# tohtsky/myFM

Hardware: AMD Instinct MI355X
Metric: Gibbs iterations/sec (rank=32) (higher is better)
Workload: dtype f64

## Files before the change

### include/myfm_hip.h

```cpp
#ifndef MYFM_HIP_H_
#define MYFM_HIP_H_

#include <stdint.h>

#ifdef __cplusplus
extern "C" {
#endif

#define MFM_OK 0
#define MFM_ERR_INVALID 1
#define MFM_ERR_RUNTIME 2
#define MFM_ERR_DEVICE 3

#define MFM_TASK_REGRESSION 0
#define MFM_TASK_CLASSIFICATION 1
#define MFM_TASK_ORDERED 2

typedef struct mfm_ctx mfm_ctx;
typedef struct mfm_design mfm_design;
typedef struct mfm_store mfm_store;

const char *mfm_version(void);
int mfm_device_count(void);
const char *mfm_global_error(void);

int mfm_create(int device, mfm_ctx **out);
void mfm_destroy(mfm_ctx *ctx);
const char *mfm_last_error(const mfm_ctx *ctx);
int mfm_get_device(const mfm_ctx *ctx);
int mfm_set_stream(mfm_ctx *ctx, void *hip_stream);
int mfm_synchronize(mfm_ctx *ctx);

int mfm_set_allreduce(mfm_ctx *ctx, int (*fn)(void *user, void *dev_buf, int64_t count), void *user);
int mfm_set_shard(mfm_ctx *ctx, int32_t rank, int32_t world);
int mfm_comm_unique_id(void *out128);
int mfm_comm_init(mfm_ctx *ctx, const void *id128, int32_t rank, int32_t world);
int mfm_comm_stats(const mfm_ctx *ctx, int64_t *calls, int64_t *doubles);
int mfm_comm_info(const mfm_ctx *ctx, int32_t *n_ranks, char *path, int64_t path_cap);
int mfm_peer_info(mfm_ctx *ctx, int32_t *pending, void **sum_buf, void **flag_buf, int64_t *sum_bytes, int64_t *flag_bytes);
int mfm_peer_set(mfm_ctx *ctx, int32_t world, int32_t rank, void *const *sum_bufs, void *const *flag_bufs);
int mfm_peer_model_info(mfm_ctx *ctx, void **w_buf, void **V_buf);
int mfm_peer_set_model(mfm_ctx *ctx, int32_t world, int32_t rank, void *const *w_bufs, void *const *V_bufs);
int mfm_peer_export(mfm_ctx *ctx, void *handles256);
int mfm_peer_import(mfm_ctx *ctx, int32_t world, int32_t rank, const void *all_handles);
int mfm_peer_drop(mfm_ctx *ctx);
int mfm_set_main_levels(mfm_ctx *ctx, const int32_t *level, int64_t D0);
int mfm_set_row_offset(mfm_ctx *ctx, int64_t first_global_row);

int mfm_set_main(mfm_ctx *ctx, int64_t N, int64_t D0, const int64_t *indptr, const int32_t *indices,
                 const double *data, const double *y);
int mfm_add_block(mfm_ctx *ctx, int64_t B, int64_t Db, const int64_t *indptr, const int32_t *indices,
                  const double *data, const int64_t *original_to_block);
int mfm_set_groups(mfm_ctx *ctx, const int32_t *group_index, int64_t D, int32_t G);
int mfm_set_residual_policy(mfm_ctx *ctx, int32_t recomputable);
int mfm_finalize(mfm_ctx *ctx, int32_t rank);

int64_t mfm_dim_all(const mfm_ctx *ctx);
int mfm_plan_info(const mfm_ctx *ctx, int64_t *n_levels_main, int64_t *n_launches_per_sweep);
int mfm_plan_flags(const mfm_ctx *ctx);
#define MFM_RES_INFO_FIELDS 16
int mfm_res_info(const mfm_ctx *ctx, int64_t *out, int n_out, char *why, int why_len);
#define MFM_CELL_INFO_FIELDS 74
int mfm_cell_info(const mfm_ctx *ctx, int64_t *out, int n_out, char *why, int why_len);
#define MFM_CHAIN_STREAM_INFO_FIELDS 30
int mfm_chain_stream_info(const mfm_ctx *ctx, int64_t *out, int max_records, int *n_records);

int mfm_set_state(mfm_ctx *ctx, double w0, const double *w, const double *V);
int mfm_get_state(mfm_ctx *ctx, double *w0, double *w, double *V);
int mfm_set_w0(mfm_ctx *ctx, double w0);
int mfm_zero_w(mfm_ctx *ctx);
int mfm_get_e(mfm_ctx *ctx, double *e);
int mfm_get_q(mfm_ctx *ctx, double *q);
int mfm_set_e(mfm_ctx *ctx, const double *e);

int mfm_reduce_e(mfm_ctx *ctx, double *sum_e, double *sum_e2);
int mfm_shift_e(mfm_ctx *ctx, double delta);
int mfm_group_stats_w(mfm_ctx *ctx, const double *mu_w, double *sum, double *ssd);
int mfm_group_stats_V(mfm_ctx *ctx, const double *mu_V, double *sum, double *ssd);
int mfm_hyper_stats(mfm_ctx *ctx, int32_t need_e, const double *mu_w, const double *mu_V, double *sum_e, double *sum_e2,
                    double *sum_w, double *ssd_w, double *sum_V, double *ssd_V);
int mfm_sweep_w(mfm_ctx *ctx, double alpha, const double *lambda_w, const double *mu_w, const double *z);
int mfm_sweep_V(mfm_ctx *ctx, int32_t f_begin, int32_t f_end, double alpha, const double *lambda_V,
                const double *mu_V, const double *z);
int mfm_sweep_wV(mfm_ctx *ctx, double alpha, double e_shift, const double *lambda_w, const double *mu_w, const double *zw,
                 int32_t f_begin, int32_t f_end, const double *lambda_V, const double *mu_V, const double *zv);

typedef struct mfm_hyper_prior {
  double alpha_0, beta_0, gamma_0, mu_0, reg_0, n_total;
  int32_t fit_w0, reserved;
} mfm_hyper_prior;
int mfm_regression_iteration_ready(mfm_ctx *ctx);
int mfm_regression_iteration(mfm_ctx *ctx, const mfm_hyper_prior *prior, const double *n_in_group, double *alpha, double *w0,
                             double *lambda_w, double *mu_w, double *lambda_V, double *mu_V);
int mfm_update_e_regression(mfm_ctx *ctx);
int mfm_update_e_classification(mfm_ctx *ctx, uint64_t seed, uint64_t draw_index);
int mfm_score_train(mfm_ctx *ctx);

int mfm_oprobit_add_group(mfm_ctx *ctx, int32_t n_class, const int64_t *rows, int64_t n_rows, int32_t *group);
int mfm_oprobit_eval(mfm_ctx *ctx, int32_t group, const double *gamma, double *ll, double *dgamma, double *H);
int mfm_oprobit_sample_z(mfm_ctx *ctx, int32_t group, const double *gamma, uint64_t seed, uint64_t draw_index);

#define MFM_RNG_NORMALS 0
#define MFM_RNG_GAMMA 1
#define MFM_RNG_LATENT 2
typedef struct mfm_rng_op {
  int32_t kind;
  int32_t dest;
  int64_t count;
  int64_t offset;
  double shape;
} mfm_rng_op;
int mfm_rng_prepare(int64_t n_features, int32_t rank, int32_t n_groups);
int mfm_rng_seed_mt19937(mfm_ctx *ctx, const uint32_t *state624, int32_t position);
int mfm_rng_set_program(mfm_ctx *ctx, const mfm_rng_op *ops, int32_t n_ops);
int mfm_rng_prefetch(mfm_ctx *ctx);
int mfm_rng_acquire(mfm_ctx *ctx, double *hyper_variates, int64_t n_hyper_variates);
int mfm_rng_get_z(mfm_ctx *ctx, double *zw, double *zv);

int mfm_update_e_classification_exact(mfm_ctx *ctx, int32_t *status);
int mfm_set_latent_order(mfm_ctx *ctx, const int64_t *rows, int64_t n);
int mfm_oprobit_sample_z_exact(mfm_ctx *ctx, int32_t group, const double *gamma, int32_t *status);
int mfm_latent_stats(mfm_ctx *ctx, int64_t *out8);
int mfm_rng_host_read(mfm_ctx *ctx, uint64_t offset, int64_t n, uint32_t *out);
int mfm_rng_host_advance(mfm_ctx *ctx, uint64_t words);

int mfm_timing_enable(mfm_ctx *ctx, int on);
int mfm_timing_select(mfm_ctx *ctx, int32_t kernel_class);
int mfm_timing_reset(mfm_ctx *ctx);
int mfm_timing_n_classes(void);
const char *mfm_timing_class_name(int cls);
int mfm_timing_get(mfm_ctx *ctx, int cls, double *ms_total, int64_t *launches, double *alg_bytes_total);

int mfm_design_create(int device, int64_t N, int64_t D0, const int64_t *indptr, const int32_t *indices,
                      const double *data, mfm_design **out);
int mfm_design_add_block(mfm_design *d, int64_t B, int64_t Db, const int64_t *indptr, const int32_t *indices,
                         const double *data, const int64_t *original_to_block);
void mfm_design_destroy(mfm_design *d);
const char *mfm_design_last_error(const mfm_design *d);
int64_t mfm_design_dim_all(const mfm_design *d);
int64_t mfm_design_n_rows(const mfm_design *d);
int mfm_design_predict(mfm_design *d, int32_t rank, int32_t n_samples, const double *w0s, const double *ws,
                       const double *Vs, int32_t mode, int32_t n_cut, const double *cutpoints, double *out);

int mfm_store_create(int device, int64_t D, int32_t rank, mfm_store **out);
void mfm_store_destroy(mfm_store *st);
const char *mfm_store_last_error(const mfm_store *st);
int32_t mfm_store_size(const mfm_store *st);
int mfm_store_reserve(mfm_store *st, int32_t n_samples);
int mfm_store_push_ctx(mfm_store *st, mfm_ctx *ctx);
int mfm_store_push_host(mfm_store *st, double w0, const double *w, const double *V);
int mfm_store_get(mfm_store *st, int32_t idx, double *w0, double *w, double *V);
int mfm_design_predict_store(mfm_design *d, mfm_store *st, int32_t first, int32_t count, int32_t mode, int32_t n_cut,
                             const double *cutpoints, double *out);

int mfm_design_summary_store(mfm_design *d, mfm_store *st, int32_t first, int32_t count, int32_t mode, int32_t n_q,
                             const double *probs, const double *precisions, const double *z, int64_t tile_rows,
                             int32_t chunk_samples, double *out_mean, double *out_std, double *out_q);
int mfm_design_summary(mfm_design *d, int32_t rank, int32_t n_samples, const double *w0s, const double *ws, const double *Vs,
                       int32_t mode, int32_t n_q, const double *probs, const double *precisions, const double *z,
                       int64_t tile_rows, int32_t chunk_samples, double *out_mean, double *out_std, double *out_q);
int mfm_design_summary_oprobit_store(mfm_design *d, mfm_store *st, int32_t first, int32_t count, int32_t expected, int32_t n_cut,
                                     const double *cutpoints, int32_t n_q, const double *probs, int64_t tile_rows,
                                     int32_t chunk_samples, double *out_mean, double *out_std, double *out_q);
int mfm_design_summary_oprobit(mfm_design *d, int32_t rank, int32_t n_samples, const double *w0s, const double *ws, const double *Vs,
                               int32_t expected, int32_t n_cut, const double *cutpoints, int32_t n_q, const double *probs,
                               int64_t tile_rows, int32_t chunk_samples, double *out_mean, double *out_std, double *out_q);

int mfm_design_logdens_store(mfm_design *d, mfm_store *st, int32_t first, int32_t count, int32_t task, const double *y,
                             const double *precisions, int32_t n_cut, const double *cutpoints, int64_t tile_rows,
                             int32_t chunk_samples, double *out_lpd, double *out_mean, double *out_var, double *out_pit,
                             double *out_ll);
int mfm_design_logdens(mfm_design *d, int32_t rank, int32_t n_samples, const double *w0s, const double *ws, const double *Vs,
                       int32_t task, const double *y, const double *precisions, int32_t n_cut, const double *cutpoints,
                       int64_t tile_rows, int32_t chunk_samples, double *out_lpd, double *out_mean, double *out_var,
                       double *out_pit, double *out_ll);
int mfm_logdens_value(int32_t task, double y, double score, double log_norm, double sqrt_alpha, int32_t n_cut,
                      const double *cutpoints_row, double *out);

int mfm_design_loo_store(mfm_design *d, mfm_store *st, int32_t first, int32_t count, int32_t task, const double *y,
                         const double *precisions, int32_t n_cut, const double *cutpoints, int64_t tile_rows,
                         int32_t chunk_samples, int32_t tail_len, double *out_elpd, double *out_k, double *out_lpd,
                         double *out_pit, double *out_lw);
int mfm_design_loo(mfm_design *d, int32_t rank, int32_t n_samples, const double *w0s, const double *ws, const double *Vs,
                   int32_t task, const double *y, const double *precisions, int32_t n_cut, const double *cutpoints,
                   int64_t tile_rows, int32_t chunk_samples, int32_t tail_len, double *out_elpd, double *out_k,
                   double *out_lpd, double *out_pit, double *out_lw);
int mfm_psis_row(int32_t S, int32_t tail_len, const double *log_lik, double *out_elpd, double *out_k, double *out_lw);

int mfm_design_ess_store(mfm_design *d, mfm_store *st, int32_t first, int32_t count, int32_t kind, int32_t mode_or_task,
                         const double *y, const double *precisions, int32_t n_cut, const double *cutpoints, int64_t tile_rows,
                         int32_t chunk_samples, double *out0, double *out1, double *out2, double *out3);
int mfm_design_ess(mfm_design *d, int32_t rank, int32_t n_samples, const double *w0s, const double *ws, const double *Vs,
                   int32_t kind, int32_t mode_or_task, const double *y, const double *precisions, int32_t n_cut,
                   const double *cutpoints, int64_t tile_rows, int32_t chunk_samples, double *out0, double *out1, double *out2,
                   double *out3);
int mfm_ess_row(int32_t S, const double *x, double *out_ess, double *out_rhat);
int mfm_design_ess_chains_store(mfm_design *d, mfm_store *st, int32_t first, int32_t count, int32_t n_chains, int32_t kind,
                                int32_t mode_or_task, const double *y, const double *precisions, int32_t n_cut,
                                const double *cutpoints, int64_t tile_rows, int32_t chunk_samples, double *out0, double *out1,
                                double *out2, double *out3);
int mfm_design_ess_chains(mfm_design *d, int32_t rank, int32_t n_samples, const double *w0s, const double *ws, const double *Vs,
                          int32_t n_chains, int32_t kind, int32_t mode_or_task, const double *y, const double *precisions,
                          int32_t n_cut, const double *cutpoints, int64_t tile_rows, int32_t chunk_samples, double *out0,
                          double *out1, double *out2, double *out3);
int mfm_ess_row_chains(int32_t S, int32_t n_chains, const double *x, double *out_ess, double *out_rhat);
int mfm_ess_check_chains(int32_t n_samples, int32_t n_chains);
int32_t mfm_ess_max_chains(void);
int mfm_rank_z_table(int32_t S, double *out);

int mfm_design_crps_store(mfm_design *d, mfm_store *st, int32_t first, int32_t count, int32_t task, const double *y,
                          const double *precisions, int32_t n_cut, const double *cutpoints, int64_t tile_rows,
                          int32_t chunk_samples, double *out_crps, double *out_accuracy, double *out_spread);
int mfm_design_crps(mfm_design *d, int32_t rank, int32_t n_samples, const double *w0s, const double *ws, const double *Vs,
                    int32_t task, const double *y, const double *precisions, int32_t n_cut, const double *cutpoints,
// ... 171 lines not shown
```

### myfm_amd/_build.py

```python
import os
import subprocess
import sys
import sysconfig

HERE = os.path.dirname(os.path.abspath(__file__))
ROOT = os.path.dirname(HERE)
CSRC = os.path.join(HERE, "csrc")
INCLUDE = os.path.join(ROOT, "include")
HIP_LIB = os.path.join(HERE, "libmyfm_hip.so")
EXT_SUFFIX = sysconfig.get_config_var("EXT_SUFFIX") or ".so"
PYMOD = os.path.join(HERE, "_myfm" + EXT_SUFFIX)

HIP_UNITS = {
    "mfm_hip.hip": ["mfm_env.hpp", "mfm_common.hpp", "mfm_wave.hpp", "mfm_policies.hpp", "mfm_kernels.hpp", "mfm_mf_kernels.hpp", "mfm_res.hpp", "mfm_res_entry.hpp", "mfm_res_plan.hpp",
                    "mfm_plan.hpp", "mfm_block_kernels.hpp", "mfm_erfcx.hpp", "mfm_tasks.hpp", "mfm_tn.hpp", "mfm_philox.hpp", "mfm_predict.hpp", "mfm_samples.hpp", "mfm_dist.hpp", "mfm_contrib.hpp", "mfm_logdens.hpp", "mfm_psis.hpp", "mfm_ess.hpp", "mfm_crps.hpp", "mfm_loo_pred.hpp", "mfm_normal_quantile.hpp", "mfm_rng.hpp", "mfm_mtjump.hpp", "mfm_cell.hpp",
                    "mfm_chain_api.hpp", "mfm_rng_state.hpp", "mfm_latent_api.hpp", "mfm_latent_host.hpp", "mfm_comm.hpp", "mfm_vbmoments.hpp", "mfm_vb_sums.hpp"],
    "mfm_latent.hip": ["mfm_env.hpp", "mfm_common.hpp", "mfm_rng_state.hpp", "mfm_latent_api.hpp"],
    "mfm_cell.hip": ["mfm_env.hpp", "mfm_common.hpp", "mfm_wave.hpp", "mfm_cell.hpp"],
    "mfm_chain.hip": ["mfm_env.hpp", "mfm_common.hpp", "mfm_wave.hpp", "mfm_policies.hpp", "mfm_chain_api.hpp", "mfm_chain_plan.hpp", "mfm_chain_stream.hpp"],
    "mfm_vb.hip": ["mfm_env.hpp", "mfm_common.hpp", "mfm_erfcx.hpp", "mfm_vb.hpp", "mfm_comm.hpp"],
    "mfm_pairs.hip": ["mfm_env.hpp", "mfm_common.hpp", "mfm_pairs.hpp", "mfm_pairs_rank.hpp", "mfm_pairs_samples.hpp", "mfm_pairs_sim.hpp", "mfm_pairs_ucb.hpp", "mfm_pairs_vb.hpp", "mfm_vb_sums.hpp", "mfm_samples.hpp"],
    "mfm_foldin.hip": ["mfm_env.hpp", "mfm_common.hpp", "mfm_foldin.hpp", "mfm_foldin_handle.hpp", "mfm_philox.hpp", "mfm_samples.hpp"],
    "mfm_foldin_gibbs.hip": ["mfm_env.hpp", "mfm_common.hpp", "mfm_foldin.hpp", "mfm_foldin_gibbs.hpp", "mfm_foldin_gibbs_plan.hpp",
                             "mfm_foldin_handle.hpp", "mfm_tn.hpp", "mfm_philox.hpp", "mfm_samples.hpp"],
}
OBJ_DIR = os.path.join(CSRC, "_obj")
PYMOD_HEADERS = ["mfm_env.hpp", "mfm_hostnormals.hpp", "mfm_mtjump.hpp", "mfm_normal_quantile.hpp"]


def _newer(target, deps):
    if not os.path.exists(target):
        return True
    t = os.path.getmtime(target)
    return any(os.path.exists(d) and os.path.getmtime(d) > t for d in deps)


def _hipcc():
    for c in ("/opt/rocm/bin/hipcc", "hipcc"):
        if os.path.exists(c) or c == "hipcc":
            return c


def build_hip(force=False, verbose=False):
    os.makedirs(OBJ_DIR, exist_ok=True)
    flags = ["--offload-arch=gfx950", "-O3", "-std=c++17", "-fPIC", "-ffp-contract=off", "-I" + INCLUDE, "-I" + CSRC] + \
        os.environ.get("MYFM_AMD_HIPCC_FLAGS", "").split()
    jobs, objs = [], []
    for src, hdrs in HIP_UNITS.items():
        obj = os.path.join(OBJ_DIR, os.path.splitext(src)[0] + ".o")
        objs.append(obj)
        deps = [os.path.join(CSRC, src)] + [os.path.join(CSRC, h) for h in hdrs] + [os.path.join(INCLUDE, "myfm_hip.h")]
        if force or _newer(obj, deps):
            cmd = [_hipcc()] + flags + ["-c", os.path.join(CSRC, src), "-o", obj]
            if verbose:
                print(" ".join(cmd))
            jobs.append((cmd, subprocess.Popen(cmd)))
    failed = [(cmd, pr.returncode) for cmd, pr in jobs if pr.wait() != 0]
    if failed:
        raise subprocess.CalledProcessError(failed[0][1], " ".join(failed[0][0]))
    if jobs or not os.path.exists(HIP_LIB) or _newer(HIP_LIB, objs):
        cmd = [_hipcc(), "--offload-arch=gfx950", "-shared", "-fPIC"] + objs + ["-o", HIP_LIB]
        if verbose:
            print(" ".join(cmd))
        subprocess.check_call(cmd)
    return HIP_LIB


def build_pymod(force=False, verbose=False):
    import pybind11

    src = os.path.join(CSRC, "_myfm.cpp")
    deps = [src, os.path.join(INCLUDE, "myfm_hip.h")] + [os.path.join(CSRC, h) for h in PYMOD_HEADERS]
    if not (force or _newer(PYMOD, deps)):
        return PYMOD
    cmd = ["g++", "-O2", "-std=c++17", "-shared", "-fPIC", "-fvisibility=hidden", "-I" + pybind11.get_include(),
           "-I" + sysconfig.get_paths()["include"], "-I" + INCLUDE, src, "-o", PYMOD, "-L" + HERE, "-lmyfm_hip",
           "-Wl,-rpath,$ORIGIN"]
    if verbose:
        print(" ".join(cmd))
    subprocess.check_call(cmd)
    return PYMOD


def build_all(force=False, verbose=False):
    build_hip(force, verbose)
    build_pymod(force, verbose)


if __name__ == "__main__":
    build_all(force="--force" in sys.argv, verbose=True)


def preload_hip_runtime():
    import ctypes
    import importlib.util

    if os.environ.get("MYFM_AMD_SYSTEM_HIP"):
        return None
    try:
        spec = importlib.util.find_spec("torch")
    except Exception:
        spec = None
    if spec is None or not spec.submodule_search_locations:
        return None
    lib = os.path.join(list(spec.submodule_search_locations)[0], "lib", "libamdhip64.so")
    if not os.path.exists(lib):
        return None
    try:
        return ctypes.CDLL(lib, mode=ctypes.RTLD_GLOBAL)
    except OSError:
        return None
```

### myfm_amd/_capi.py

```python
import ctypes as C
import os

import numpy as np
import scipy.sparse as sps

_HERE = os.path.dirname(os.path.abspath(__file__))
LIB_PATH = os.path.join(_HERE, "libmyfm_hip.so")

MFM_OK, MFM_ERR_INVALID, MFM_ERR_RUNTIME, MFM_ERR_DEVICE = 0, 1, 2, 3
TASK_REGRESSION, TASK_CLASSIFICATION, TASK_ORDERED = 0, 1, 2

SYMBOLS = [
    "mfm_version", "mfm_device_count", "mfm_global_error", "mfm_create", "mfm_destroy", "mfm_last_error",
    "mfm_set_stream", "mfm_synchronize", "mfm_set_main", "mfm_add_block", "mfm_set_groups", "mfm_finalize",
    "mfm_peer_info", "mfm_peer_set", "mfm_peer_model_info", "mfm_peer_set_model", "mfm_peer_export", "mfm_peer_import", "mfm_peer_drop", "mfm_set_residual_policy", "mfm_dim_all", "mfm_plan_info", "mfm_plan_flags", "mfm_res_info", "mfm_cell_info", "mfm_chain_stream_info", "mfm_set_state", "mfm_get_state", "mfm_set_w0", "mfm_zero_w", "mfm_get_e",
    "mfm_get_q", "mfm_set_e", "mfm_reduce_e", "mfm_shift_e", "mfm_group_stats_w", "mfm_group_stats_V",
    "mfm_sweep_w", "mfm_sweep_V", "mfm_sweep_wV", "mfm_update_e_regression", "mfm_update_e_classification", "mfm_score_train",
    "mfm_oprobit_add_group", "mfm_oprobit_eval", "mfm_oprobit_sample_z", "mfm_hyper_stats", "mfm_timing_enable", "mfm_timing_select", "mfm_timing_reset",
    "mfm_timing_n_classes", "mfm_timing_class_name", "mfm_timing_get", "mfm_design_create", "mfm_design_add_block",
    "mfm_design_destroy", "mfm_design_last_error", "mfm_design_dim_all", "mfm_design_predict",
    "mfm_host_column_levels", "mfm_rng_prepare", "mfm_rng_seed_mt19937", "mfm_rng_set_program", "mfm_rng_prefetch", "mfm_rng_acquire",
    "mfm_rng_get_z", "mfm_design_score_ctx", "mfm_design_n_rows", "mfm_set_allreduce", "mfm_set_row_offset", "mfm_set_main_levels",
    "mfm_test_erfcx", "mfm_test_truncated_normal", "mfm_get_device", "mfm_set_shard", "mfm_comm_unique_id", "mfm_comm_init",
    "mfm_comm_stats", "mfm_comm_info", "mfm_store_create", "mfm_store_destroy", "mfm_store_last_error", "mfm_store_size", "mfm_store_push_ctx",
    "mfm_store_push_host", "mfm_store_get", "mfm_design_predict_store", "mfm_store_reserve", "mfm_cs_plan_selftest", "mfm_cs_plan_probe",
    "mfm_regression_iteration_ready", "mfm_regression_iteration",
    "mfm_update_e_classification_exact", "mfm_oprobit_sample_z_exact", "mfm_latent_stats", "mfm_rng_host_read", "mfm_rng_host_advance", "mfm_set_latent_order",
    "mfm_vb_create", "mfm_vb_add_block", "mfm_vb_finalize", "mfm_vb_destroy", "mfm_vb_last_error", "mfm_vb_plan_info", "mfm_vb_set_state", "mfm_vb_get_state",
    "mfm_vb_set_w0", "mfm_vb_update_e", "mfm_vb_shift_e", "mfm_vb_get_e", "mfm_vb_get_cache", "mfm_vb_zero_w", "mfm_vb_sweep_w",
    "mfm_vb_sweep_V", "mfm_vb_group_stats", "mfm_vb_synchronize", "mfm_vb_truncated_normal",
    "mfm_vb_set_stream", "mfm_vb_set_allreduce", "mfm_vb_set_shard", "mfm_vb_comm_init", "mfm_vb_comm_stats", "mfm_vb_set_levels",
    "mfm_vb_design_levels",
    "mfm_pairs_create", "mfm_pairs_destroy", "mfm_pairs_last_error", "mfm_pairs_set_exclude", "mfm_pairs_set_scratch_bound",
    "mfm_pairs_scores_store", "mfm_pairs_topk_store", "mfm_pairs_scores", "mfm_pairs_topk", "mfm_pairs_add_block",
    "mfm_pairs_set_cutpoints", "mfm_pairs_moments_store", "mfm_pairs_moments", "mfm_pairs_topk_ucb_store", "mfm_pairs_topk_ucb",
    "mfm_pairs_set_targets", "mfm_pairs_rank_store", "mfm_pairs_rank",
    "mfm_pairs_topk_samples_store", "mfm_pairs_topk_samples", "mfm_pairs_topk_prob_store", "mfm_pairs_topk_prob",
    "mfm_pairs_create_sim", "mfm_pairs_sim_store", "mfm_pairs_sim", "mfm_pairs_topk_sim_store", "mfm_pairs_topk_sim",
    "mfm_foldin_create", "mfm_foldin_destroy", "mfm_foldin_last_error", "mfm_foldin_set_scratch_bound", "mfm_foldin_max_rank",
    "mfm_foldin_solve_store", "mfm_foldin_solve", "mfm_foldin_gibbs_solve_store", "mfm_foldin_gibbs_solve",
    "mfm_design_summary_store", "mfm_design_summary", "mfm_design_summary_oprobit_store", "mfm_design_summary_oprobit",
    "mfm_design_logdens_store", "mfm_design_logdens", "mfm_logdens_value",
    "mfm_design_loo_store", "mfm_design_loo", "mfm_psis_row",
    "mfm_design_ess_store", "mfm_design_ess", "mfm_ess_row", "mfm_rank_z_table",
    "mfm_design_ess_chains_store", "mfm_design_ess_chains", "mfm_ess_row_chains", "mfm_ess_check_chains", "mfm_ess_max_chains",
    "mfm_design_crps_store", "mfm_design_crps", "mfm_crps_row",
    "mfm_design_loo_summary_store", "mfm_design_loo_summary", "mfm_design_loo_crps_store", "mfm_design_loo_crps",
    "mfm_loo_summary_row", "mfm_loo_crps_row",
    "mfm_design_contrib_store", "mfm_design_contrib", "mfm_contrib_row",
    "mfm_design_moments_vb", "mfm_pairs_moments_vb", "mfm_pairs_topk_bound_vb",
]

SIM_METRICS = {"cosine": 0, "dot": 1}
PAIRS_VOTE_MAX = 32768

CHAIN_STREAM_INFO = ("block", "n_cols", "n_steps", "Cg", "Lw", "NB", "RD", "n_slots", "max_hot_col", "max_enter", "max_exit", "max_cold_sr",
                     "max_enter_sr", "max_exit_sr", "n_cols_no_hot")
CHAIN_STREAM_INFO_TAIL = ("lds_bytes", "n_cold", "n_hot", "launches_w", "launches_V")
CHAIN_STREAM_INFO_FIELDS = len(CHAIN_STREAM_INFO) + 10 + len(CHAIN_STREAM_INFO_TAIL)


def chain_stream_record(rec):
    n = len(CHAIN_STREAM_INFO)
    d = dict(zip(CHAIN_STREAM_INFO, (int(v) for v in rec[:n])))
    d["hot_rounds"] = [int(v) for v in rec[n:n + 10]]
    d.update(zip(CHAIN_STREAM_INFO_TAIL, (int(v) for v in rec[n + 10:])))
    return d


_lib = None


def lib():
    global _lib
    if _lib is not None:
        return _lib
    if not os.path.exists(LIB_PATH):
        raise ImportError(
            "%s is missing: build it with `python -c 'import __graft_entry__ as g; g.build()'` "
            "(hipcc --offload-arch=gfx950). There is no CPU fallback." % LIB_PATH
        )
    from ._build import preload_hip_runtime

    preload_hip_runtime()
    L = C.CDLL(LIB_PATH)
    vp, i64, i32, dbl, P = C.c_void_p, C.c_int64, C.c_int32, C.c_double, C.c_void_p
    u64 = C.c_uint64
    L.mfm_version.restype = C.c_char_p
    L.mfm_global_error.restype = C.c_char_p
    L.mfm_create.argtypes = [C.c_int, C.POINTER(vp)]
    L.mfm_destroy.argtypes = [vp]
    L.mfm_destroy.restype = None
    L.mfm_last_error.restype = C.c_char_p
    L.mfm_last_error.argtypes = [vp]
    L.mfm_set_stream.argtypes = [vp, vp]
    L.mfm_synchronize.argtypes = [vp]
    L.mfm_set_main.argtypes = [vp, i64, i64, P, P, P, P]
    L.mfm_add_block.argtypes = [vp, i64, i64, P, P, P, P]
    L.mfm_set_groups.argtypes = [vp, P, i64, i32]
    L.mfm_finalize.argtypes = [vp, i32]
    L.mfm_peer_info.argtypes = [vp, P, P, P, P, P]
    L.mfm_peer_set.argtypes = [vp, i32, i32, P, P]
    L.mfm_peer_model_info.argtypes = [vp, P, P]
    L.mfm_peer_set_model.argtypes = [vp, i32, i32, P, P]
    L.mfm_peer_export.argtypes = [vp, P]
    L.mfm_peer_import.argtypes = [vp, i32, i32, P]
    L.mfm_peer_drop.argtypes = [vp]
    L.mfm_regression_iteration_ready.argtypes = [vp]
    L.mfm_regression_iteration.argtypes = [vp, P, P, P, P, P, P, P, P]
    L.mfm_set_residual_policy.argtypes = [vp, i32]
    L.mfm_dim_all.restype = i64
    L.mfm_dim_all.argtypes = [vp]
    L.mfm_plan_info.argtypes = [vp, C.POINTER(i64), C.POINTER(i64)]
    L.mfm_plan_flags.argtypes = [vp]
    L.mfm_res_info.argtypes = [vp, P, C.c_int, C.c_char_p, C.c_int]
    L.mfm_cell_info.argtypes = [vp, P, C.c_int, C.c_char_p, C.c_int]
    L.mfm_chain_stream_info.argtypes = [vp, P, C.c_int, C.POINTER(C.c_int)]
    L.mfm_cs_plan_probe.argtypes = [i64, i32, P, P, P, i32, i32, i32, i32, P, P, C.POINTER(i32), C.POINTER(dbl)]
    L.mfm_set_state.argtypes = [vp, dbl, P, P]
    L.mfm_get_state.argtypes = [vp, C.POINTER(dbl), P, P]
    L.mfm_set_w0.argtypes = [vp, dbl]
    L.mfm_zero_w.argtypes = [vp]
    L.mfm_get_e.argtypes = [vp, P]
    L.mfm_get_q.argtypes = [vp, P]
    L.mfm_set_e.argtypes = [vp, P]
    L.mfm_reduce_e.argtypes = [vp, C.POINTER(dbl), C.POINTER(dbl)]
    L.mfm_shift_e.argtypes = [vp, dbl]
    L.mfm_group_stats_w.argtypes = [vp, P, P, P]
    L.mfm_group_stats_V.argtypes = [vp, P, P, P]
    L.mfm_hyper_stats.argtypes = [vp, C.c_int32, P, P, P, P, P, P, P, P]
    L.mfm_sweep_w.argtypes = [vp, dbl, P, P, P]
    L.mfm_sweep_V.argtypes = [vp, i32, i32, dbl, P, P, P]
    L.mfm_sweep_wV.argtypes = [vp, dbl, dbl, P, P, P, i32, i32, P, P, P]
    L.mfm_update_e_regression.argtypes = [vp]
    L.mfm_update_e_classification.argtypes = [vp, u64, u64]
    L.mfm_score_train.argtypes = [vp]
    L.mfm_oprobit_add_group.argtypes = [vp, i32, P, i64, C.POINTER(i32)]
    L.mfm_oprobit_eval.argtypes = [vp, i32, P, C.POINTER(dbl), P, P]
    L.mfm_oprobit_sample_z.argtypes = [vp, i32, P, u64, u64]
    L.mfm_timing_enable.argtypes = [vp, C.c_int]
    L.mfm_timing_select.argtypes = [vp, C.c_int32]
    L.mfm_timing_reset.argtypes = [vp]
    L.mfm_timing_class_name.restype = C.c_char_p
    L.mfm_timing_class_name.argtypes = [C.c_int]
    L.mfm_timing_get.argtypes = [vp, C.c_int, C.POINTER(dbl), C.POINTER(i64), C.POINTER(dbl)]
    L.mfm_design_create.argtypes = [C.c_int, i64, i64, P, P, P, C.POINTER(vp)]
    L.mfm_design_add_block.argtypes = [vp, i64, i64, P, P, P, P]
    L.mfm_design_destroy.argtypes = [vp]
    L.mfm_design_destroy.restype = None
    L.mfm_design_last_error.restype = C.c_char_p
    L.mfm_design_last_error.argtypes = [vp]
    L.mfm_design_dim_all.restype = i64
    L.mfm_design_dim_all.argtypes = [vp]
    L.mfm_design_predict.argtypes = [vp, i32, i32, P, P, P, i32, i32, P, P]
    L.mfm_host_column_levels.argtypes = [i64, i64, P, P, P, C.POINTER(i32)]
    L.mfm_rng_prepare.argtypes = [i64, i32, i32]
    L.mfm_rng_seed_mt19937.argtypes = [vp, P, i32]
    L.mfm_rng_set_program.argtypes = [vp, P, i32]
    L.mfm_rng_prefetch.argtypes = [vp]
    L.mfm_rng_acquire.argtypes = [vp, P, i64]
    L.mfm_rng_get_z.argtypes = [vp, P, P]
    L.mfm_update_e_classification_exact.argtypes = [vp, C.POINTER(i32)]
    L.mfm_oprobit_sample_z_exact.argtypes = [vp, i32, P, C.POINTER(i32)]
    L.mfm_latent_stats.argtypes = [vp, P]
    L.mfm_set_latent_order.argtypes = [vp, P, i64]
    L.mfm_rng_host_read.argtypes = [vp, u64, i64, P]
    L.mfm_rng_host_advance.argtypes = [vp, u64]
    L.mfm_design_score_ctx.argtypes = [vp, vp, P]
    L.mfm_design_n_rows.restype = i64
    L.mfm_design_n_rows.argtypes = [vp]
    L.mfm_set_allreduce.argtypes = [vp, vp, vp]
    L.mfm_set_row_offset.argtypes = [vp, i64]
    L.mfm_set_main_levels.argtypes = [vp, P, i64]
    L.mfm_get_device.argtypes = [vp]
    L.mfm_set_shard.argtypes = [vp, i32, i32]
    L.mfm_comm_unique_id.argtypes = [P]
    L.mfm_comm_init.argtypes = [vp, P, i32, i32]
    L.mfm_comm_stats.argtypes = [vp, C.POINTER(i64), C.POINTER(i64)]
    L.mfm_comm_info.argtypes = [vp, C.POINTER(i32), C.c_char_p, i64]
    L.mfm_store_create.argtypes = [C.c_int, i64, i32, C.POINTER(vp)]
    L.mfm_store_destroy.argtypes = [vp]
    L.mfm_store_destroy.restype = None
    L.mfm_store_last_error.restype = C.c_char_p
    L.mfm_store_last_error.argtypes = [vp]
    L.mfm_store_size.argtypes = [vp]
    L.mfm_store_reserve.argtypes = [vp, i32]
    L.mfm_store_push_ctx.argtypes = [vp, vp]
    L.mfm_store_push_host.argtypes = [vp, dbl, P, P]
    L.mfm_store_get.argtypes = [vp, i32, C.POINTER(dbl), P, P]
    L.mfm_design_predict_store.argtypes = [vp, vp, i32, i32, i32, i32, P, P]
    L.mfm_design_summary_store.argtypes = [vp, vp, i32, i32, i32, i32, P, P, P, i64, i32, P, P, P]
    L.mfm_design_summary.argtypes = [vp, i32, i32, P, P, P, i32, i32, P, P, P, i64, i32, P, P, P]
    L.mfm_design_summary_oprobit_store.argtypes = [vp, vp, i32, i32, i32, i32, P, i32, P, i64, i32, P, P, P]
    L.mfm_design_summary_oprobit.argtypes = [vp, i32, i32, P, P, P, i32, i32, P, i32, P, i64, i32, P, P, P]
    L.mfm_design_logdens_store.argtypes = [vp, vp, i32, i32, i32, P, P, i32, P, i64, i32, P, P, P, P, P]
    L.mfm_design_logdens.argtypes = [vp, i32, i32, P, P, P, i32, P, P, i32, P, i64, i32, P, P, P, P, P]
    L.mfm_logdens_value.argtypes = [i32, dbl, dbl, dbl, dbl, i32, P, P]
    L.mfm_design_loo_store.argtypes = [vp, vp, i32, i32, i32, P, P, i32, P, i64, i32, i32, P, P, P, P, P]
    L.mfm_design_loo.argtypes = [vp, i32, i32, P, P, P, i32, P, P, i32, P, i64, i32, i32, P, P, P, P, P]
    L.mfm_psis_row.argtypes = [i32, i32, P, P, P, P]
    L.mfm_design_ess_store.argtypes = [vp, vp, i32, i32, i32, i32, P, P, i32, P, i64, i32, P, P, P, P]
    L.mfm_design_ess.argtypes = [vp, i32, i32, P, P, P, i32, i32, P, P, i32, P, i64, i32, P, P, P, P]
    L.mfm_ess_row.argtypes = [i32, P, P, P]
    L.mfm_design_ess_chains_store.argtypes = [vp, vp, i32, i32, i32, i32, i32, P, P, i32, P, i64, i32, P, P, P, P]
    L.mfm_design_ess_chains.argtypes = [vp, i32, i32, P, P, P, i32, i32, i32, P, P, i32, P, i64, i32, P, P, P, P]
    L.mfm_ess_row_chains.argtypes = [i32, i32, P, P, P]
    L.mfm_ess_check_chains.argtypes = [i32, i32]
    L.mfm_ess_max_chains.argtypes = []
    L.mfm_rank_z_table.argtypes = [i32, P]
    L.mfm_design_crps_store.argtypes = [vp, vp, i32, i32, i32, P, P, i32, P, i64, i32, P, P, P]
    L.mfm_design_crps.argtypes = [vp, i32, i32, P, P, P, i32, P, P, i32, P, i64, i32, P, P, P]
    L.mfm_crps_row.argtypes = [i32, i32, dbl, P, P, i32, P, P]
    L.mfm_design_loo_summary_store.argtypes = [vp, vp, i32, i32, i32, P, P, i32, P, i64, i32, i32, i32, P, P, P, P, P, P, P]
    L.mfm_design_loo_summary.argtypes = [vp, i32, i32, P, P, P, i32, P, P, i32, P, i64, i32, i32, i32, P, P, P, P, P, P, P]
    L.mfm_design_contrib_store.argtypes = [vp, vp, i32, i32, i32, P, i64, i64, i32, P, P, P, P, P]
    L.mfm_design_contrib.argtypes = [vp, i32, i32, P, P, P, i32, P, i64, i64, i32, P, P, P, P, P]
    L.mfm_contrib_row.argtypes = [i32, P, P, i64, i32, i32, P, P, i32, P, i64, P, P]
    L.mfm_design_loo_crps_store.argtypes = [vp, vp, i32, i32, i32, P, P, i32, P, i64, i32, i32, P, P, P, P]
    L.mfm_design_loo_crps.argtypes = [vp, i32, i32, P, P, P, i32, P, P, i32, P, i64, i32, i32, P, P, P, P]
    L.mfm_loo_summary_row.argtypes = [i32, P, P, P, i32, P, P, P, P, P, P]
    L.mfm_loo_crps_row.argtypes = [i32, i32, dbl, P, P, P, i32, P, P]
    L.mfm_pairs_create.argtypes = [C.c_int, i64, i64, P, P, P, i64, P, P, P, C.POINTER(vp)]
    L.mfm_pairs_create_sim.argtypes = L.mfm_pairs_create.argtypes
    L.mfm_pairs_sim_store.argtypes = [vp, vp, i32, i32, i32, P, P]
    L.mfm_pairs_sim.argtypes = [vp, i32, i32, P, P, P, i32, P, P]
    L.mfm_pairs_topk_sim_store.argtypes = [vp, vp, i32, i32, i32, i32, C.c_double, P, P, P, P]
    L.mfm_pairs_topk_sim.argtypes = [vp, i32, i32, P, P, P, i32, i32, C.c_double, P, P, P, P]
    L.mfm_pairs_destroy.argtypes = [vp]
    L.mfm_pairs_destroy.restype = None
    L.mfm_pairs_last_error.restype = C.c_char_p
    L.mfm_pairs_last_error.argtypes = [vp]
    L.mfm_pairs_set_exclude.argtypes = [vp, P, P]
    L.mfm_pairs_set_scratch_bound.argtypes = [vp, i64]
    L.mfm_pairs_add_block.argtypes = [vp, i32, i64, i64, i64, P, P, P, P]
    L.mfm_pairs_set_cutpoints.argtypes = [vp, i32, i32, P]
    L.mfm_pairs_scores_store.argtypes = [vp, vp, i32, i32, i32, P]
    L.mfm_pairs_topk_store.argtypes = [vp, vp, i32, i32, i32, i32, P, P]
    L.mfm_pairs_scores.argtypes = [vp, i32, i32, P, P, P, i32, P]
    L.mfm_pairs_topk.argtypes = [vp, i32, i32, P, P, P, i32, i32, P, P]
    L.mfm_pairs_moments_store.argtypes = [vp, vp, i32, i32, i32, P, P]
    L.mfm_pairs_moments.argtypes = [vp, i32, i32, P, P, P, i32, P, P]
    L.mfm_pairs_topk_ucb_store.argtypes = [vp, vp, i32, i32, i32, i32, C.c_double, P, P, P, P]
    L.mfm_pairs_topk_ucb.argtypes = [vp, i32, i32, P, P, P, i32, i32, C.c_double, P, P, P, P]
    L.mfm_pairs_set_targets.argtypes = [vp, P, P]
    L.mfm_design_moments_vb.argtypes = [vp, i32, dbl, dbl, P, P, P, P, dbl, i32, i64, P, P, P]
    L.mfm_pairs_moments_vb.argtypes = [vp, i32, dbl, dbl, P, P, P, P, dbl, P, P]
    L.mfm_pairs_topk_bound_vb.argtypes = [vp, i32, dbl, dbl, P, P, P, P, dbl, i32, dbl, P, P, P, P]
    L.mfm_pairs_rank_store.argtypes = [vp, vp, i32, i32, i32, P, P]
    L.mfm_pairs_rank.argtypes = [vp, i32, i32, P, P, P, i32, P, P]
    L.mfm_pairs_topk_samples_store.argtypes = [vp, vp, i32, i32, i32, i32, P, P, P]
    L.mfm_pairs_topk_samples.argtypes = [vp, i32, i32, P, P, P, i32, i32, P, P, P]
    L.mfm_pairs_topk_prob_store.argtypes = [vp, vp, i32, i32, i32, i32, i32, P, P]
    L.mfm_pairs_topk_prob.argtypes = [vp, i32, i32, P, P, P, i32, i32, i32, P, P]
    L.mfm_foldin_create.argtypes = [C.c_int, i64, i64, P, P, P, P, i64, P, i32, C.POINTER(vp)]
    L.mfm_foldin_destroy.argtypes = [vp]
    L.mfm_foldin_destroy.restype = None
    L.mfm_foldin_last_error.restype = C.c_char_p
    L.mfm_foldin_last_error.argtypes = [vp]
    L.mfm_foldin_set_scratch_bound.argtypes = [vp, i64]
    L.mfm_foldin_max_rank.argtypes = []
    L.mfm_foldin_solve_store.argtypes = [vp, vp, i32, i32, P, P, P, i32, u64, P, P]
    L.mfm_foldin_solve.argtypes = [vp, i32, i32, P, P, P, P, P, P, i32, u64, P, P]
    L.mfm_foldin_gibbs_solve_store.argtypes = [vp, vp, i32, i32, i32, i32, P, P, P, i32, i32, i32, u64, P, P]
    L.mfm_foldin_gibbs_solve.argtypes = [vp, i32, i32, P, P, P, i32, i32, P, P, P, i32, i32, i32, u64, P, P]
    L.mfm_test_erfcx.argtypes = [C.c_int, P, i64, P]
    L.mfm_test_truncated_normal.argtypes = [C.c_int, i32, dbl, dbl, u64, u64, i64, P]
    _lib = L
    return L
# ... 124 lines not shown

    def set_e(self, e):
        e = _f64(e)
        self._ck(lib().mfm_set_e(self.h, _p(e)))

    def reduce_e(self):
        a, b = C.c_double(), C.c_double()
        self._ck(lib().mfm_reduce_e(self.h, C.byref(a), C.byref(b)))
        return a.value, b.value

    def shift_e(self, delta):
        self._ck(lib().mfm_shift_e(self.h, float(delta)))

    def group_stats_w(self, mu_w):
        mu_w = _f64(mu_w)
        s, ss = np.empty(self.G), np.empty(self.G)
        self._ck(lib().mfm_group_stats_w(self.h, _p(mu_w), _p(s), _p(ss)))
        return s, ss

    def group_stats_V(self, mu_V):
        mu = _f64(np.asarray(mu_V).T)
        s, ss = np.empty((self.K, self.G)), np.empty((self.K, self.G))
        self._ck(lib().mfm_group_stats_V(self.h, _p(mu), _p(s), _p(ss)))
        return s.T.copy(), ss.T.copy()

    def sweep_w(self, alpha, lambda_w, mu_w, z):
        lambda_w, mu_w = _f64(lambda_w), _f64(mu_w)
        if z is not None:
            z = _f64(z)
            assert z.shape[0] == self.D
        self._ck(lib().mfm_sweep_w(self.h, float(alpha), _p(lambda_w), _p(mu_w), _p(z)))

    def sweep_V(self, f_begin, f_end, alpha, lambda_V, mu_V, z):
        lam, mu = _f64(np.asarray(lambda_V).T), _f64(np.asarray(mu_V).T)
        if z is not None:
            z = _f64(z)
            assert z.size == (f_end - f_begin) * self.D
        self._ck(lib().mfm_sweep_V(self.h, f_begin, f_end, float(alpha), _p(lam), _p(mu), _p(z)))

    def sweep_wV(self, alpha, e_shift, lambda_w, mu_w, zw, f_begin, f_end, lambda_V, mu_V, zv):
        lambda_w, mu_w = _f64(lambda_w), _f64(mu_w)
        lam, mu = _f64(np.asarray(lambda_V).T), _f64(np.asarray(mu_V).T)
        if zw is not None:
            zw, zv = _f64(zw), _f64(zv)
            assert zw.shape[0] == self.D and zv.size == (f_end - f_begin) * self.D
        self._ck(lib().mfm_sweep_wV(self.h, float(alpha), float(e_shift), _p(lambda_w), _p(mu_w), _p(zw), f_begin, f_end,
                                    _p(lam), _p(mu), _p(zv)))

    def update_e_regression(self):
        self._ck(lib().mfm_update_e_regression(self.h))

    def update_e_classification(self, seed, draw_index):
        self._ck(lib().mfm_update_e_classification(self.h, seed, draw_index))

    def score_train(self):
        self._ck(lib().mfm_score_train(self.h))

    def oprobit_add_group(self, n_class, rows=None):
        g = C.c_int32()
        if rows is None:
            self._ck(lib().mfm_oprobit_add_group(self.h, n_class, None, 0, C.byref(g)))
        else:
            rows = np.ascontiguousarray(rows, dtype=np.int64)
            self._ck(lib().mfm_oprobit_add_group(self.h, n_class, _p(rows), rows.shape[0], C.byref(g)))
        return g.value

    def oprobit_eval(self, group, gamma, want_h=True):
        gamma = _f64(gamma)
        m = gamma.shape[0]
        ll = C.c_double()
        dg = np.empty(m)
        H = np.empty((m, m)) if want_h else None
        self._ck(lib().mfm_oprobit_eval(self.h, group, _p(gamma), C.byref(ll), _p(dg), _p(H)))
        return ll.value, dg, H

    def oprobit_sample_z(self, group, gamma, seed, draw_index):
        gamma = _f64(gamma)
        self._ck(lib().mfm_oprobit_sample_z(self.h, group, _p(gamma), seed, draw_index))

    def synchronize(self):
        self._ck(lib().mfm_synchronize(self.h))

    RNG_OP = np.dtype([("kind", np.int32), ("dest", np.int32), ("count", np.int64), ("offset", np.int64), ("shape", np.float64)])

    def rng_seed_mt19937(self, state624, position):
        st = np.ascontiguousarray(state624, dtype=np.uint32)
        assert st.shape[0] == 624
        self._ck(lib().mfm_rng_seed_mt19937(self.h, _p(st), int(position)))

    def rng_set_program(self, ops):
        arr = np.array([tuple(o) for o in ops], dtype=self.RNG_OP)
        self._n_hv = int(sum(o[2] for o in ops if o[1] == 0))
        self._ck(lib().mfm_rng_set_program(self.h, _p(arr), len(ops)))

    def rng_prefetch(self):
        self._ck(lib().mfm_rng_prefetch(self.h))

    def rng_acquire(self):
        hv = np.empty(max(self._n_hv, 1))
        self._ck(lib().mfm_rng_acquire(self.h, _p(hv), self._n_hv))
        return hv[: self._n_hv]

    def rng_get_z(self):
        zw, zv = np.empty(self.D), np.empty((max(self.K, 1), self.D))
        self._ck(lib().mfm_rng_get_z(self.h, _p(zw), _p(zv)))
        return zw, zv[: self.K]

    def update_e_classification_exact(self):
        st = C.c_int32()
        self._ck(lib().mfm_update_e_classification_exact(self.h, C.byref(st)))
        return st.value

    def oprobit_sample_z_exact(self, group, gamma):
        gamma = _f64(gamma)
        st = C.c_int32()
        self._ck(lib().mfm_oprobit_sample_z_exact(self.h, group, _p(gamma), C.byref(st)))
        return st.value

    def latent_stats(self):
        out = np.zeros(8, dtype=np.int64)
        self._ck(lib().mfm_latent_stats(self.h, _p(out)))
        return dict(zip(("status", "chunks", "subs", "lq", "quads", "walkers", "attempts"), (int(v) for v in out)))

    def rng_host_read(self, offset, n):
        out = np.empty(max(int(n), 1), dtype=np.uint32)
        self._ck(lib().mfm_rng_host_read(self.h, int(offset), int(n), _p(out)))
        return out[: int(n)]

    def rng_host_advance(self, words):
        self._ck(lib().mfm_rng_host_advance(self.h, int(words)))

    def set_residual_policy(self, recomputable):
        self._ck(lib().mfm_set_residual_policy(self.h, 1 if recomputable else 0))

    def plan_flags(self):
        f = lib().mfm_plan_flags(self.h)
        return {"qfree": bool(f & 1), "unit": bool(f & 2), "ell": bool(f & 4), "sharded": bool(f & 8), "soa": bool(f & 16),
                "fused_next": bool(f & 32), "sharded_fused": bool(f & 64), "mf": bool(f & 128), "resident": bool(f & 256), "cell": bool(f & 512), "streamed_chain": bool(f & 1024), "resident_overflow": bool(f & 2048)}

    RES_INFO = ("ready", "G", "RV", "RL", "RX", "umax", "n_items", "item_bits", "n_runs", "max_wg_users", "max_slice_items",
                "e_where", "n_rows", "s2_in_sweep_b", "lds_bytes", "entry_bytes")
    E_WHERE = ("rows", "slots", "slots_with_sums", "cell", "dropped")

    def res_info(self):
        out = np.zeros(len(self.RES_INFO), dtype=np.int64)
        why = C.create_string_buffer(256)
        self._ck(lib().mfm_res_info(self.h, _p(out), out.shape[0], why, len(why)))
        d = dict(zip(self.RES_INFO, (int(v) for v in out)))
        d["ready"] = bool(d["ready"])
        d["e_where"] = self.E_WHERE[d["e_where"]]
        d["why"] = why.value.decode()
        return d

    CELL_INFO = ("ready", "G", "umax", "item32", "n_streams", "n_fields", "N", "Npad", "max_steps", "chunk_max", "chunk_min",
                 "chunks_empty", "split_mask", "score_fb")
    CELL_STREAM_TYPE = ("U", "I", "C")
    CELL_MAX_STREAMS, CELL_MAX_FIELDS = 4, 16
    CELL_INFO_FIELDS = len(CELL_INFO) + 3 * CELL_MAX_STREAMS + 3 * CELL_MAX_FIELDS

    def cell_info(self):
        out = np.zeros(self.CELL_INFO_FIELDS, dtype=np.int64)
        why = C.create_string_buffer(256)
        self._ck(lib().mfm_cell_info(self.h, _p(out), out.shape[0], why, len(why)))
        n = len(self.CELL_INFO)
        nf = n + 3 * self.CELL_MAX_STREAMS
        d = dict(zip(self.CELL_INFO, (int(v) for v in out[:n])))
        d["ready"], d["item32"] = bool(d["ready"]), bool(d["item32"])
        d["streams"] = [(self.CELL_STREAM_TYPE[int(out[n + 3 * s])], int(out[n + 3 * s + 1]), int(out[n + 3 * s + 2]))
                        for s in range(d["n_streams"])]
        d["fields"] = [tuple(int(x) for x in out[nf + 3 * k:nf + 3 * k + 3]) for k in range(d["n_fields"])]
        d["why"] = why.value.decode()
        return d

    def chain_stream_info(self):
        n = C.c_int(0)
        self._ck(lib().mfm_chain_stream_info(self.h, None, 0, C.byref(n)))
        out = np.zeros((max(n.value, 1), CHAIN_STREAM_INFO_FIELDS), dtype=np.int64)
        self._ck(lib().mfm_chain_stream_info(self.h, _p(out), n.value, C.byref(n)))
        return [chain_stream_record(out[i]) for i in range(n.value)]

    def plan_info(self):
        a, b = C.c_int64(), C.c_int64()
        lib().mfm_plan_info(self.h, C.byref(a), C.byref(b))
        return a.value, b.value

    def timing_enable(self, on=True):
        self._ck(lib().mfm_timing_enable(self.h, int(on)))

    def timing_reset(self):
        self._ck(lib().mfm_timing_reset(self.h))

    def timing(self):
        L = lib()
        out = {}
        for c in range(L.mfm_timing_n_classes()):
            ms, n, by = C.c_double(), C.c_int64(), C.c_double()
            self._ck(L.mfm_timing_get(self.h, c, C.byref(ms), C.byref(n), C.byref(by)))
            if n.value:
                out[L.mfm_timing_class_name(c).decode()] = (ms.value, n.value, by.value)
        return out


class Design:

    def __init__(self, X, blocks=(), device=0):
        L = lib()
        h = C.c_void_p()
        X, ip, ix, dv = csr_parts(X)
        rc = L.mfm_design_create(device, X.shape[0], X.shape[1], _p(ip), _p(ix), _p(dv), C.byref(h))
        if rc:
            _raise(rc, L.mfm_global_error())
        self.h = h
        self.N = X.shape[0]
        for mp, B in blocks:
            B, bp, bx, bv = csr_parts(B)
            mp = np.ascontiguousarray(mp, dtype=np.int64)
            if mp.shape[0] != self.N:
                self.close()
                raise ValueError("Relation blocks have inconsistent mapper size with case_size")
            rc = L.mfm_design_add_block(h, B.shape[0], B.shape[1], _p(bp), _p(bx), _p(bv), _p(mp))
            if rc:
                msg = L.mfm_design_last_error(h)
                self.close()
                _raise(rc, msg)
        self.D = L.mfm_design_dim_all(h)

    def close(self):
        if getattr(self, "h", None):
            lib().mfm_design_destroy(self.h)
            self.h = None

    def __del__(self):
        try:
            self.close()
        except Exception:
            pass

    def score_ctx(self, ctx):
        out = np.empty(self.N)
        self._ck(lib().mfm_design_score_ctx(self.h, ctx.h, _p(out)))
        return out

    def _ck(self, rc):
        if rc:
            _raise(rc, lib().mfm_design_last_error(self.h))

    def moments_vb(self, model, extra_var=0.0, want_prob=False, tile_rows=0):
        K, head, keep = _pack_vb_model(model)
        mean, std, prob = np.empty(self.N), np.empty(self.N), np.empty(self.N if want_prob else 0)
        self._ck(lib().mfm_design_moments_vb(self.h, K, *head, float(extra_var), int(bool(want_prob)), int(tile_rows), _p(mean), _p(std),
                                             _p(prob) if want_prob else None))
        return (mean, std, prob) if want_prob else (mean, std)

    def _predict(self, src, mode, cutpoints):
        n_cut, cp = 0, None
        if mode == 2:
            cp = _f64(np.stack([np.asarray(c, dtype=np.float64) for c in cutpoints]))
            n_cut = cp.shape[1]
        out = np.empty((self.N, n_cut + 1) if mode == 2 else self.N)
        self._ck(src.call("mfm_design_predict", self.h, mode, n_cut, _p(cp), _p(out)))
        return out

    def _summary(self, src, mode, quantiles, precisions, tile_rows, chunk_samples):
        probs, prec, z, mean, std, q = _summary_args(self.N, quantiles, precisions)
        self._ck(src.call("mfm_design_summary", self.h, mode, len(probs), _p(probs), _p(prec), _p(z), int(tile_rows),
                          int(chunk_samples), _p(mean), _p(std), _p(q)))
        return mean, std, q

    def _summary_oprobit(self, src, cutpoints, expected, quantiles, tile_rows, chunk_samples):
        cp, n_cut, probs, mean, std, q = _summary_oprobit_args(self.N, cutpoints, expected, quantiles)
        self._ck(src.call("mfm_design_summary_oprobit", self.h, int(bool(expected)), n_cut, _p(cp), len(probs), _p(probs),
                          int(tile_rows), int(chunk_samples), _p(mean), _p(std), _p(q)))
        return mean, std, q

    def _log_density_args(self, y, precisions, cutpoints):
        y = _f64(y).reshape(-1)
        if y.shape[0] != self.N:
            raise ValueError("y must hold one value per design row")
        prec = None if precisions is None else _f64(precisions).reshape(-1)
        cp, n_cut = None, 0
        if cutpoints is not None:
            cp = _f64(cutpoints)
            if cp.ndim != 2:
                raise ValueError("cutpoints must be a 2-D array, one row of n_cut cutpoints per sample")
            n_cut = cp.shape[1]
        return y, prec, n_cut, cp

    def _log_density(self, src, task, y, precisions, cutpoints, pointwise, tile_rows, chunk_samples):
        y, prec, n_cut, cp = self._log_density_args(y, precisions, cutpoints)
        lpd, mean, var = np.empty(self.N), np.empty(self.N), np.empty(self.N)
        pit = np.empty(self.N) if task == TASK_REGRESSION else None
        ll = np.empty((src.S, self.N)) if pointwise else None
        self._ck(src.call("mfm_design_logdens", self.h, int(task), _p(y), _p(prec), n_cut, _p(cp), int(tile_rows), int(chunk_samples),
                          _p(lpd), _p(mean), _p(var), _p(pit), _p(ll)))
        return lpd, mean, var, pit, ll

    def log_density(self, samples, task, y, precisions=None, cutpoints=None, pointwise=False, tile_rows=0, chunk_samples=0):
        return self._log_density(_host(samples), task, y, precisions, cutpoints, pointwise, tile_rows, chunk_samples)

    def _loo(self, src, task, y, precisions, cutpoints, log_weights, r_eff, tile_rows, chunk_samples):
        y, prec, n_cut, cp = self._log_density_args(y, precisions, cutpoints)
        elpd, k, lpd = np.empty(self.N), np.empty(self.N), np.empty(self.N)
        pit = np.empty(self.N) if task == TASK_REGRESSION else None
        lw = np.empty((src.S, self.N)) if log_weights else None
        self._ck(src.call("mfm_design_loo", self.h, int(task), _p(y), _p(prec), n_cut, _p(cp), int(tile_rows), int(chunk_samples),
                          psis_tail_len(src.S, r_eff), _p(elpd), _p(k), _p(lpd), _p(pit), _p(lw)))
# ... 544 lines not shown
```

### myfm_amd/csrc/mfm_hip.hip

```cpp
#include <algorithm>
#include <cerrno>
#include <chrono>
#include <cmath>
#include <cstdio>
#include <cstring>
#include <map>
#include <memory>
#include <mutex>
#include <string>
#include <thread>
#include <type_traits>
#include <vector>

#include <fcntl.h>
#include <sys/file.h>
#include <sys/stat.h>
#include <unistd.h>

#include <hipcub/hipcub.hpp>

#include "mfm_common.hpp"
#include "mfm_kernels.hpp"
#include "mfm_plan.hpp"
#include "mfm_res_plan.hpp"
// ... 1410 lines not shown
  MFM_HIP_CHECK(hipStreamSynchronize(c->stream));
  c->res.peers_set = true;
  c->res_state = ResState::Live;
  MFM_CATCH(ctx)
}

int mfm_peer_set_model(mfm_ctx *ctx, int32_t world, int32_t rank, void *const *w_bufs, void *const *V_bufs) {
  MFM_TRY(ctx)
  ctx->need_final();
  mfm_ctx *c = ctx;
  if (!c->resident_V() || !c->res.peers_set) throw Error(MFM_ERR_RUNTIME, "mfm_peer_set_model: mfm_peer_set comes first");
  if (world != c->res.xworld || rank != c->res.xrank) throw Error(MFM_ERR_INVALID, "mfm_peer_set_model: world / rank differ from the communicator's");
  for (int r = 0; r < world; r++) {
    if (!w_bufs[r] || (c->K > 0 && !V_bufs[r])) throw Error(MFM_ERR_INVALID, "mfm_peer_set_model: null buffer");
    c->res.peer_w[r] = (double *)w_bufs[r];
    c->res.peer_V[r] = (double *)V_bufs[r];
  }
  if (c->res.peer_w[rank] != c->w.p || c->res.peer_V[rank] != c->V.p)
    throw Error(MFM_ERR_INVALID, "mfm_peer_set_model: this rank's own entry must be its own w / V (mfm_peer_model_info)");
  MFM_HIP_CHECK(hipStreamSynchronize(c->stream));
  c->res.peers_model = true;
  MFM_CATCH(ctx)
}

int mfm_peer_model_info(mfm_ctx *ctx, void **w_buf, void **V_buf) {
  MFM_TRY(ctx)
  ctx->need_final();
  if (w_buf) *w_buf = ctx->w.p;
  if (V_buf) *V_buf = ctx->V.p;
  MFM_CATCH(ctx)
}

int mfm_peer_export(mfm_ctx *ctx, void *handles256) {
  MFM_TRY(ctx)
  ctx->need_final();
  if (ctx->res_state != ResState::AwaitingPeers) throw Error(MFM_ERR_RUNTIME, "mfm_peer_export: no row-sharded persistent sweep waiting for its peers");
  static_assert(sizeof(hipIpcMemHandle_t) == 64, "IPC handle size");
  hipIpcMemHandle_t h[4];
  std::memset(h, 0, sizeof h);
  MFM_HIP_CHECK(hipIpcGetMemHandle(&h[0], ctx->res.xsum.p));
  MFM_HIP_CHECK(hipIpcGetMemHandle(&h[1], ctx->res.xflag.p));
  MFM_HIP_CHECK(hipIpcGetMemHandle(&h[2], ctx->w.p));
  if (ctx->K > 0) MFM_HIP_CHECK(hipIpcGetMemHandle(&h[3], ctx->V.p));
  std::memcpy(handles256, h, sizeof h);
  MFM_CATCH(ctx)
}

int mfm_peer_import(mfm_ctx *ctx, int32_t world, int32_t rank, const void *all_handles) {
  MFM_TRY(ctx)
  ctx->need_final();
  mfm_ctx *c = ctx;
  if (c->res_state != ResState::AwaitingPeers) throw Error(MFM_ERR_RUNTIME, "mfm_peer_import: no row-sharded persistent sweep waiting for its peers");
  if (world != c->res.xworld || rank != c->res.xrank) throw Error(MFM_ERR_INVALID, "mfm_peer_import: world / rank differ from the communicator's");
  void *sums[RES_MAX_PEERS], *flags[RES_MAX_PEERS], *ws[RES_MAX_PEERS], *Vs[RES_MAX_PEERS];
  for (int r = 0; r < world; r++) {
    if (r == rank) {
      sums[r] = c->res.xsum.p;
      flags[r] = c->res.xflag.p;
      ws[r] = c->w.p;
      Vs[r] = c->V.p;
      continue;
    }
    hipIpcMemHandle_t h[4];
    std::memcpy(h, (const char *)all_handles + (size_t)r * 256, sizeof h);
    MFM_HIP_CHECK(hipIpcOpenMemHandle(&sums[r], h[0], hipIpcMemLazyEnablePeerAccess));
    c->res.peer_mapped.push_back(sums[r]);
    MFM_HIP_CHECK(hipIpcOpenMemHandle(&flags[r], h[1], hipIpcMemLazyEnablePeerAccess));
    c->res.peer_mapped.push_back(flags[r]);
    MFM_HIP_CHECK(hipIpcOpenMemHandle(&ws[r], h[2], hipIpcMemLazyEnablePeerAccess));
    c->res.peer_mapped.push_back(ws[r]);
    Vs[r] = nullptr;
    if (c->K > 0) {
      MFM_HIP_CHECK(hipIpcOpenMemHandle(&Vs[r], h[3], hipIpcMemLazyEnablePeerAccess));
      c->res.peer_mapped.push_back(Vs[r]);
    }
  }
  int rc = mfm_peer_set(ctx, world, rank, sums, flags);
  if (rc != MFM_OK) return rc;
  if (env_int("MYFM_PEER_MODEL", 0) != 0) {
    rc = mfm_peer_set_model(ctx, world, rank, ws, Vs);
    if (rc != MFM_OK) return rc;
  }
  MFM_CATCH(ctx)
}

int mfm_peer_drop(mfm_ctx *ctx) {
  MFM_TRY(ctx)
  ctx->need_final();
  MFM_HIP_CHECK(hipStreamSynchronize(ctx->stream));
  materialize_e(ctx);
  ctx->drop_resident();
  MFM_CATCH(ctx)
}

int mfm_set_residual_policy(mfm_ctx *ctx, int32_t recomputable) {
  if (!ctx) return MFM_ERR_INVALID;
  ctx->e_recomputable = recomputable != 0;
  return MFM_OK;
}

int64_t mfm_dim_all(const mfm_ctx *ctx) { return ctx->D; }

int mfm_plan_info(const mfm_ctx *ctx, int64_t *n_levels_main, int64_t *n_launches_per_sweep) {
  if (ctx->v_path == VPath::Deferred) {
    if (n_levels_main) *n_levels_main = 2;
    if (n_launches_per_sweep) *n_launches_per_sweep = 1;
    return MFM_OK;
  }
  if (n_levels_main) *n_levels_main = (int64_t)ctx->plan_V.n_levels;
  if (n_launches_per_sweep) {
    int64_t n = ctx->plan_V.launches;
    for (auto &B : ctx->blocks) n += B->plan_V.launches + 3;
    *n_launches_per_sweep = n;
  }
  return MFM_OK;
}

int mfm_plan_flags(const mfm_ctx *ctx) {
  bool streamed = false;
  for (auto &B : ctx->blocks)
    for (const Step &st : B->plan_V.steps) streamed = streamed || (st.is_chain && st.chain.form == ChainForm::Stream);
  int form = 0;
  switch (ctx->v_path) {
    case VPath::QFree: form = 1; break;
    case VPath::Split: form = 16; break;
    case VPath::SplitFused: form = 16 | 32; break;
    case VPath::TwoField: form = 16 | 32 | 128; break;
    case VPath::ShardedSplit: form = 64; break;
    case VPath::ShardedTwoField: form = 64 | 128; break;
    case VPath::Deferred:
    case VPath::Generic:
    case VPath::Cell:
      break;
  }
  return (streamed ? 1024 : 0) | (ctx->resident_V() && ctx->res.RX > 0 ? 2048 : 0) | form | (ctx->X.unit ? 2 : 0) | (ctx->X.ell_width >= 0 ? 4 : 0) |
         (ctx->comm.active() ? 8 : 0) | (ctx->resident_V() ? 256 : 0) | (ctx->cell.ready ? 512 : 0);
}

int mfm_res_info(const mfm_ctx *ctx, int64_t *out, int n_out, char *why, int why_len) {
  if (!ctx || n_out < 0 || (n_out > 0 && !out) || why_len < 0 || (why_len > 0 && !why)) return MFM_ERR_INVALID;
  const ResPlan &rp = ctx->res;
  const int64_t v[MFM_RES_INFO_FIELDS] = {ctx->resident_V() ? 1 : 0, rp.G,       rp.RV,     rp.RL,           rp.RX,
                                          rp.umax,          rp.n_items, rp.item_bits, rp.n_runs,    rp.max_wg_users,
                                          rp.max_slice_items, (int64_t)ctx->e_where, rp.n_rows, rp.s2b, (int64_t)rp.lds_bytes,
                                          rp.ent_bytes};
  for (int i = 0; i < n_out; i++) out[i] = i < MFM_RES_INFO_FIELDS ? v[i] : 0;
  if (why_len > 0) {
    std::strncpy(why, ctx->resident_V() ? "" : rp.why.c_str(), (size_t)why_len - 1);
    why[why_len - 1] = 0;
  }
  return MFM_OK;
}

int mfm_cell_info(const mfm_ctx *ctx, int64_t *out, int n_out, char *why, int why_len) {
  if (!ctx || n_out < 0 || (n_out > 0 && !out) || why_len < 0 || (why_len > 0 && !why)) return MFM_ERR_INVALID;
  const CellPlan &cp = ctx->cell;
  int64_t v[MFM_CELL_INFO_FIELDS] = {0};
  const int m = (int)cp.fields.size(), ns = (int)cp.streams.size();
  int64_t split = 0;
  const bool typed = ns > 0 && cp.sU == 0;
  for (int k = 0; k < m && typed; k++)
    if (cp.split_pass(k == 0 ? m - 1 : k - 1, k, k == 0)) split |= (int64_t)1 << k;
  const int64_t head[14] = {cp.ready ? 1 : 0, cp.G,         cp.umax,      cp.item32 ? 1 : 0, ns,    m, cp.N, cp.Npad, cp.max_steps,
                            cp.chunk_max,     cp.chunk_min, cp.chunks_empty, split,          cp.ready ? cp.score_fb() : 0};
  for (int i = 0; i < 14; i++) v[i] = head[i];
  for (int i = 0; i < ns && i < CELL_MAX_STREAMS; i++) {
    v[14 + 3 * i] = cp.streams[i].type;
    v[15 + 3 * i] = cp.streams[i].slot;
    v[16 + 3 * i] = cp.streams[i].card;
  }
  for (int k = 0; k < m && k < CELL_MAX_FIELDS; k++) {
    v[14 + 3 * CELL_MAX_STREAMS + 3 * k] = cp.fields[k].stream;
    v[15 + 3 * CELL_MAX_STREAMS + 3 * k] = cp.fields[k].kind;
    v[16 + 3 * CELL_MAX_STREAMS + 3 * k] = cp.fields[k].n;
  }
  for (int i = 0; i < n_out; i++) out[i] = i < MFM_CELL_INFO_FIELDS ? v[i] : 0;
  if (why_len > 0) {
    std::strncpy(why, cp.ready ? "" : cp.why.c_str(), (size_t)why_len - 1);
    why[why_len - 1] = 0;
  }
  return MFM_OK;
}

int mfm_chain_stream_info(const mfm_ctx *ctx, int64_t *out, int max_records, int *n_records) {
  static_assert(MFM_CHAIN_STREAM_INFO_FIELDS == CS_INFO_FIELDS, "include/myfm_hip.h documents cs_info_record's fields");
  if (!ctx || max_records < 0 || (max_records > 0 && !out)) return MFM_ERR_INVALID;
  int n = 0;
  for (size_t b = 0; b < ctx->blocks.size(); b++) {
    std::vector<const CsStream *> of_w;
    for (const Step &st : ctx->blocks[b]->plan_W.steps)
      if (st.is_chain && st.chain.form == ChainForm::Stream) of_w.push_back(st.chain.stream.get());
    size_t k = 0;
    for (const Step &st : ctx->blocks[b]->plan_V.steps) {
      if (!st.is_chain || st.chain.form != ChainForm::Stream) continue;
      if (n < max_records) {
        int64_t *rec = out + (size_t)n * MFM_CHAIN_STREAM_INFO_FIELDS;
        cs_info_record(cs_stream_info(*st.chain.stream), rec);
        rec[0] = (int64_t)b;
        rec[28] = k < of_w.size() ? cs_stream_launches(*of_w[k], false) : 0;
        rec[29] = cs_stream_launches(*st.chain.stream, true);
      }
      n++;
      k++;
    }
  }
  if (n_records) *n_records = n;
  return MFM_OK;
}

int mfm_set_state(mfm_ctx *ctx, double w0, const double *w, const double *V) {
  MFM_TRY(ctx)
  ctx->need_final();
  ctx->w0 = w0;
  ctx->ring.upload(ctx->w.p, w, (size_t)ctx->D * sizeof(double), ctx->stream);
  if (ctx->K) ctx->ring.upload(ctx->V.p, V, (size_t)ctx->D * ctx->K * sizeof(double), ctx->stream);
  MFM_CATCH(ctx)
}

int mfm_get_state(mfm_ctx *ctx, double *w0, double *w, double *V) {
  MFM_TRY(ctx)
  ctx->need_final();
  *w0 = ctx->w0;
  if (ctx->D)
    MFM_HIP_CHECK(hipMemcpyAsync(w, ctx->w.p, (size_t)ctx->D * sizeof(double), hipMemcpyDeviceToHost, ctx->stream));
  if (ctx->K && ctx->D)
    MFM_HIP_CHECK(
        hipMemcpyAsync(V, ctx->V.p, (size_t)ctx->D * ctx->K * sizeof(double), hipMemcpyDeviceToHost, ctx->stream));
  ctx->sync_and_check();
  MFM_CATCH(ctx)
}

int mfm_set_w0(mfm_ctx *ctx, double w0) {
  MFM_TRY(ctx)
  if (w0 != ctx->w0) ensure_e(ctx);
  ctx->w0 = w0;
  MFM_CATCH(ctx)
}

int mfm_zero_w(mfm_ctx *ctx) {
  MFM_TRY(ctx)
  ctx->need_final();
  if (ctx->D) MFM_HIP_CHECK(hipMemsetAsync(ctx->w.p, 0, (size_t)ctx->D * sizeof(double), ctx->stream));
  MFM_CATCH(ctx)
}

static int get_eq(mfm_ctx *ctx, double *dst, int which) {
  MFM_TRY(ctx)
  ctx->need_final();
  materialize_e(ctx);
  if (ctx->N) {
    hipLaunchKernelGGL(k_get_eq, dim3(cdiv(ctx->N, WG)), dim3(WG), 0, ctx->stream, ctx->eq_rows(), ctx->scratch_n.p, ctx->N,
                       which);
    MFM_HIP_CHECK(
        hipMemcpyAsync(dst, ctx->scratch_n.p, (size_t)ctx->N * sizeof(double), hipMemcpyDeviceToHost, ctx->stream));
    MFM_HIP_CHECK(hipStreamSynchronize(ctx->stream));
  }
  MFM_CATCH(ctx)
}
int mfm_get_e(mfm_ctx *ctx, double *e) { return get_eq(ctx, e, 0); }
int mfm_get_q(mfm_ctx *ctx, double *q) {
  if (ctx->finalized && ctx->q_stale_factor >= 0) {
    try {
      ctx->use_device();
      for (auto &B : ctx->blocks)
        if (ctx->cell.ready) block_rowcache(ctx->stream, ctx->timing, *B, ctx->V.p + (size_t)ctx->q_stale_factor * ctx->D + B->col_off, true);
      launch_qbuild(ctx, ctx->V.p + (size_t)ctx->q_stale_factor * ctx->D);
      ctx->q_stale_factor = -1;
    } catch (const std::exception &ex) {
      ctx->err = ex.what();
      return MFM_ERR_RUNTIME;
    }
  }
  return get_eq(ctx, q, 1);
}
int mfm_set_e(mfm_ctx *ctx, const double *e) {
  MFM_TRY(ctx)
  ctx->need_final();
  if (ctx->e_where == EWhere::Dropped) ctx->e_where = EWhere::Rows;
  ctx->e_is_residual = false;
  materialize_e(ctx);
  if (ctx->N) {
    MFM_HIP_CHECK(hipStreamSynchronize(ctx->stream));
    MFM_HIP_CHECK(hipMemcpy(ctx->scratch_n.p, e, (size_t)ctx->N * sizeof(double), hipMemcpyHostToDevice));
    hipLaunchKernelGGL(k_set_eq, dim3(cdiv(ctx->N, WG)), dim3(WG), 0, ctx->stream, ctx->eq_rows(), ctx->scratch_n.p, ctx->N, 0);
    MFM_HIP_CHECK(hipStreamSynchronize(ctx->stream));
  }
  MFM_CATCH(ctx)
}

int mfm_reduce_e(mfm_ctx *ctx, double *sum_e, double *sum_e2) {
  MFM_TRY(ctx)
  ctx->need_final();
  materialize_e(ctx);
  hipStream_t s = ctx->stream;
  {
    TimedLaunch t(ctx->timing, s, KC_REDUCE_E, 8.0 * ctx->N);
    hipLaunchKernelGGL(k_reduce_e_partial, dim3(REDUCE_BLOCKS), dim3(WG), 0, s, ctx->eq_rows(), ctx->N, ctx->red_partial.p);
    hipLaunchKernelGGL(k_reduce_final, dim3(1), dim3(WG), 0, s, ctx->red_partial.p, REDUCE_BLOCKS, ctx->red_out.p);
  }
  ctx->comm.allreduce(ctx->red_out.p, 2);
  double2 *h = ctx->readback(2);
  MFM_HIP_CHECK(hipMemcpyAsync(h, ctx->red_out.p, sizeof(double2), hipMemcpyDeviceToHost, s));
  MFM_HIP_CHECK(hipMemcpyAsync(h + 1, ctx->ls.error.p, sizeof(int), hipMemcpyDeviceToHost, s));
  MFM_HIP_CHECK(hipStreamSynchronize(s));
  ctx->check_coresident(*(const int *)(h + 1));
  *sum_e = h[0].x;
// ... 802 lines not shown
```

### myfm_amd/csrc/mfm_res.hpp

```cpp
#pragma once
#include <algorithm>
#include <cstdlib>
#include <cstring>
#include <atomic>
#include <string>
#include <thread>
#include <type_traits>
#include <vector>

#include "mfm_common.hpp"
#include "mfm_mf_kernels.hpp"
#include "mfm_res_entry.hpp"

namespace mfm {

#ifndef MFM_RES_CH
#define MFM_RES_CH 4
#endif
constexpr int RES_MAX_PEERS = 8;

struct ResArgs {
  double2 *eq;
  const double *e_in;
  double *e_slots;
  const int32_t *perm;
  const uint32_t *uidw;
  const uint32_t *headw;
  const int32_t *run_item;
  const int32_t *first_run;
  const int32_t *wg_run_ptr;
  const int32_t *wg_nruns;
  const int32_t *wg_user_ptr;
  const int2 *user_desc;
  const int32_t *wg_item_ptr;
  const int32_t *ent_ptr;
  const uint32_t *entries;
  const int32_t *scols;
  const int2 *item_desc;
  double *partials;
  double *dv;
  double *V;
  int64_t D;
  int f_begin, f_end;
  int linear;
  int n_sw;
  double *w;
  const double *zw;
  const double *lam_w, *mu_w;
  double e_shift;
  const double *z;
  const double *lam, *mu;
  const int32_t *group;
  int n_groups;
  double alpha;
  const double *scal;
  int n_items, umax;
  unsigned long long *bar;
  int n_wg;
  int *error;
  unsigned long long *prof;
  int xworld, xrank;
  unsigned long long xepoch0;
  double *xsum[RES_MAX_PEERS];
  unsigned long long *xflag[RES_MAX_PEERS];
  unsigned long long *xarrive;
  int xmodel;
  double *xw[RES_MAX_PEERS], *xV[RES_MAX_PEERS];
  int ngx;
  int no_store;
  int xch_break;
  int ent4;
  const double *s2_lin;
};

__device__ __forceinline__ void res_store2(double *p, double a, double b) {
  __hip_atomic_store(p, a, __ATOMIC_RELAXED, __HIP_MEMORY_SCOPE_AGENT);
  __hip_atomic_store(p + 1, b, __ATOMIC_RELAXED, __HIP_MEMORY_SCOPE_AGENT);
}

enum { RES_BAR_START = 0, RES_BAR_TOP = 16, RES_BAR_XCNT = 32, RES_BAR_GEN = 160, RES_BAR_CENSUS = 288, RES_BAR_WORDS = 416 };
struct ResBar {
  int xcc;
  unsigned long long n_x, nx;
};

__device__ __forceinline__ bool res_spin(const ResArgs &a, const unsigned long long *w, unsigned long long target, bool &dead) {
  unsigned spins = 0;
  while (__hip_atomic_load(w, __ATOMIC_RELAXED, __HIP_MEMORY_SCOPE_AGENT) < target) {
#ifndef MFM_RES_NO_SLEEP
    __builtin_amdgcn_s_sleep(1);
#endif
    if ((++spins & 1023u) == 0u) {
      if (spins > (1u << 22) || __hip_atomic_load(a.error, __ATOMIC_RELAXED, __HIP_MEMORY_SCOPE_AGENT) != 0) {
        __hip_atomic_store(a.error, 1, __ATOMIC_RELAXED, __HIP_MEMORY_SCOPE_AGENT);
        dead = true;
        return false;
      }
    }
  }
  return true;
}

__device__ __forceinline__ bool res_spin_sys(const ResArgs &a, const unsigned long long *w, unsigned long long target, bool &dead) {
  unsigned spins = 0;
  while (__hip_atomic_load(w, __ATOMIC_RELAXED, __HIP_MEMORY_SCOPE_SYSTEM) < target) {
    __builtin_amdgcn_s_sleep(2);
    if ((++spins & 1023u) == 0u) {
      const int seen = __hip_atomic_load(a.error, __ATOMIC_RELAXED, __HIP_MEMORY_SCOPE_AGENT);
      if (spins > (1u << 23) || seen != 0) {
        if (seen == 0) __hip_atomic_store(a.error, 2, __ATOMIC_RELAXED, __HIP_MEMORY_SCOPE_AGENT);
        dead = true;
        return false;
      }
    }
  }
  return true;
}

__device__ __forceinline__ void res_bar_init(const ResArgs &a, ResBar &rb, bool &dead) {
  unsigned x;
  asm volatile("s_getreg_b32 %0, hwreg(HW_REG_XCC_ID, 0, 4)" : "=s"(x));
  rb.xcc = (int)(x & 7u);
  __hip_atomic_fetch_add(a.bar + RES_BAR_CENSUS + 16 * rb.xcc, 1ull, __ATOMIC_RELAXED, __HIP_MEMORY_SCOPE_AGENT);
  asm volatile("s_waitcnt vmcnt(0)" ::: "memory");
  __hip_atomic_fetch_add(a.bar + RES_BAR_START, 1ull, __ATOMIC_RELAXED, __HIP_MEMORY_SCOPE_AGENT);
  rb.n_x = 1;
  rb.nx = 1;
  if (!res_spin(a, a.bar + RES_BAR_START, (unsigned long long)a.n_wg, dead)) return;
  rb.nx = 0;
  for (int i = 0; i < 8; i++) {
    const unsigned long long c = __hip_atomic_load(a.bar + RES_BAR_CENSUS + 16 * i, __ATOMIC_RELAXED, __HIP_MEMORY_SCOPE_AGENT);
    rb.nx += c > 0 ? 1 : 0;
    if (i == rb.xcc) rb.n_x = c;
  }
}

__device__ __forceinline__ void res_grid_barrier(const ResArgs &a, const ResBar &rb, unsigned long long k, int tid, bool &dead) {
  asm volatile("s_waitcnt vmcnt(0)" ::: "memory");
  __syncthreads();
  if (tid == 0 && !dead) {
    const unsigned long long old =
        __hip_atomic_fetch_add(a.bar + RES_BAR_XCNT + 16 * rb.xcc, 1ull, __ATOMIC_RELAXED, __HIP_MEMORY_SCOPE_AGENT);
    if (old + 1 == k * rb.n_x) {
      __builtin_amdgcn_fence(__ATOMIC_RELEASE, "agent");
      asm volatile("s_waitcnt vmcnt(0)" ::: "memory");
      __hip_atomic_fetch_add(a.bar + RES_BAR_TOP, 1ull, __ATOMIC_RELAXED, __HIP_MEMORY_SCOPE_AGENT);
      if (res_spin(a, a.bar + RES_BAR_TOP, k * rb.nx, dead))
        __hip_atomic_store(a.bar + RES_BAR_GEN + 16 * rb.xcc, k, __ATOMIC_RELAXED, __HIP_MEMORY_SCOPE_AGENT);
    } else {
      res_spin(a, a.bar + RES_BAR_GEN + 16 * rb.xcc, k, dead);
    }
    __builtin_amdgcn_fence(__ATOMIC_ACQUIRE, "agent");
  }
  __syncthreads();
}

constexpr int res_dv_shift(bool s2b) { return s2b ? 5 : 4; }
typedef double res_d16_t __attribute__((ext_vector_type(16)));
typedef unsigned res_u4_t __attribute__((ext_vector_type(4)));
typedef double res_d2u_t __attribute__((ext_vector_type(2), aligned(8)));
__device__ __forceinline__ double res_cc0(double x) { return x; }
__device__ __forceinline__ double res_cc1(double) { return 0.0; }
__device__ __forceinline__ double res_cc0(res_d2u_t x) { return x[0]; }
__device__ __forceinline__ double res_cc1(res_d2u_t x) { return x[1]; }

#define RES_UID(lo, hi, bb, k) \
  ((k) < 3 ? (int)(((lo) >> (10 * (k))) & 0x3ffu) : (int)(((lo) >> 30) | ((((hi) >> (8 * (bb))) & 0xffu) << 2)))
#define RES_UIDS(lo, hi, bb, uid)        \
  {                                      \
    const unsigned lo_ = lo;             \
    uid[0] = RES_UID(lo_, hi, bb, 0);    \
    uid[1] = RES_UID(lo_, hi, bb, 1);    \
    uid[2] = RES_UID(lo_, hi, bb, 2);    \
    uid[3] = RES_UID(lo_, hi, bb, 3);    \
  }
#define RES_USER_WORDS(p_, row_, off_, uw_, ux_)                                                      \
  _Pragma("unroll") for (int w_ = 0; w_ < 4; w_++) uw_[w_] = (p_)[((row_) + w_) * NT + (off_)];       \
  ux_ = (p_)[((row_) + 4) * NT + (off_)]
#define RES_GROUP_WORDS(a_, ngt_, j_, uw_, ux_, hb_)                                           \
  RES_USER_WORDS((a_).uidw, (int64_t)g * (5 * (ngt_)) + 5 * (j_), tid, uw_, ux_);              \
  hb_ = (a_).headw[((int64_t)g * (ngt_) + (j_)) * NT + tid]

template <int NT, int NGV, int NGL, bool XCH = false, bool OVF = false, bool S2B = false>
__global__ __launch_bounds__(NT) void k_mf_resident(ResArgs a) {
  extern __shared__ __attribute__((aligned(16))) char res_smem[];
  constexpr int NW = NT / WAVE, NG = NGV + NGL, R = 16 * NG, RL = 16 * NGL;
  constexpr int B = 4;
  const int g = (int)blockIdx.x, tid = threadIdx.x, lane = tid & 63;
  const int wv = __builtin_amdgcn_readfirstlane(tid >> 6);
  const int U = a.umax;
  const double alpha_k = a.scal ? a.scal[0] : a.alpha, e_shift_k = a.scal ? a.scal[2] : a.e_shift;
  const int ngx = OVF ? a.ngx : 0, NGt = NG + ngx, Rt = 16 * NGt;
  d2_t *utab = (d2_t *)res_smem;
  double *elds = (double *)(utab + U);
  double *acc1 = elds + (size_t)RL * NT;
  double *acc2 = acc1 + NW * U;
  double *acc3 = acc2 + NW * U;
  d2_t *wcarry = (d2_t *)(acc2 + (S2B ? 2 : 1) * NW * U);
  int *wflag = (int *)(wcarry + NW);
  const int32_t *perm_g = a.perm + (int64_t)g * Rt * NT;
  const int u0 = a.wg_user_ptr[g], nu = a.wg_user_ptr[g + 1] - u0;
  const int rb0 = a.wg_run_ptr[g];
  const int pad_item = a.n_items;
  constexpr int DSH = res_dv_shift(S2B);
  const unsigned rb0b = 4u * (unsigned)rb0, padb = (unsigned)pad_item << DSH;
  const char *run_item_b = (const char *)a.run_item, *dv_b = (const char *)a.dv;
  double *acc1w = acc1 + wv * U, *acc2w = acc2 + wv * U, *acc3w = acc3 + wv * U;
  bool dead = false;
  unsigned long long nbar = 0;
  ResBar rbar;
  rbar.xcc = 0;
  rbar.n_x = rbar.nx = 1;
#define RES_STAMP0(k) \
  if (a.prof && tid == 0) a.prof[(int64_t)g * a.n_sw * 64 + 56 + (k)] = __builtin_amdgcn_s_memrealtime()
  RES_STAMP0(0);
  if (tid == 0) res_bar_init(a, rbar, dead);
  RES_STAMP0(1);
  const int wv_hi = wv >> 2;
#define RES_PRIO(j)                  \
  if ((((j) & 1) ^ wv_hi) != 0)      \
    __builtin_amdgcn_s_setprio(1);   \
  else                               \
    __builtin_amdgcn_s_setprio(0)
  const int trash_run = a.wg_run_ptr[g] + a.wg_nruns[g];
#define RES_STAMP(k)                                                                                      \
  if (a.prof && tid == 0) a.prof[((int64_t)g * a.n_sw + (f - f_first)) * 64 + (k)] = __builtin_amdgcn_s_memrealtime()

  const bool s2_tab = S2B && a.s2_lin != nullptr;
  for (int i = tid; i < (S2B && !s2_tab ? 3 : 2) * NW * U; i += NT) acc1[i] = 0.0;
  if (s2_tab)
    for (int i = tid; i < NW * U; i += NT) acc3[i] = a.s2_lin[(int64_t)g * (NW * U) + i];
  for (int i = tid; i < U; i += NT) utab[i] = d2_t{0.0, 0.0};

  res_u4_t uw[NG];
  unsigned ux[NG];
  unsigned hbv[NG], nbv[NG];
#pragma unroll
  for (int j = 0; j < NG; j++) {
    RES_GROUP_WORDS(a, NGt, j, uw[j], ux[j], hbv[j]);
    nbv[j] = hbv[j] | (j == 0 ? 1u : 0u);
  }
  const unsigned nbx0 = OVF && ngx > 0 ? a.headw[((int64_t)g * NGt + NG) * NT + tid] : 0u;
  double *eog = OVF ? a.e_slots + ((int64_t)g * Rt + 16 * NG) * NT + tid : nullptr;
  const uint32_t *uidw_x = a.uidw + ((int64_t)g * (5 * NGt) + 5 * NG) * NT + tid;
  const uint32_t *headw_x = a.headw + ((int64_t)g * NGt + NG) * NT + tid;
  const int run0 = a.first_run[g * NT + tid];
  const bool head0 = (hbv[0] & 1u) != 0u;
#define RES_NIB(j, q) ((((nbv[j]) | ((j) + 1 < NG ? nbv[(j) + 1 < NG ? (j) + 1 : (j)] << 16 : nbx0 << 16)) >> (4 * (q))) & 15u)
#define RES_ON_NIB(q) RES_NIB(j, q)
#define RES_ON_HEADS hbv[j]
#define RES_ON_UIDS(bb, uid) RES_UIDS(uw[j][bb], ux[j], bb, uid)
#define RES_ON_LD(bb, k) (j < NGV ? ev[j < NGV ? j : 0][4 * (bb) + k] : elds[(16 * (j - NGV) + 4 * (bb) + k) * NT + tid])
#define RES_ON_ST(bb, k, x)                \
  if (j < NGV)                             \
    ev[j < NGV ? j : 0][4 * (bb) + k] = x; \
  else                                     \
    elds[(16 * (j - NGV) + 4 * (bb) + k) * NT + tid] = x
#define RES_OV_NIB(q) ((nbw >> (4 * (q))) & 15u)
#define RES_OV_HEADS hb_c
#define RES_OV_UIDS(bb, uid) RES_UIDS(uwx[bb], uxx, bb, uid)
#define RES_OV_LD(bb, k) eo[4 * (bb) + k]
#define RES_OV_ST(bb, k, x) eo[4 * (bb) + k] = x
#define RES_OVERFLOW_GROUPS(STEP, gA, gB)                                                   \
  if (OVF) {                                                                                \
    unsigned hb_c = nbx0;                                                                   \
    for (int jx = 0; jx < ngx; jx++) {                                                      \
      res_u4_t uwx;                                                                         \
      unsigned uxx;                                                                         \
      RES_USER_WORDS(uidw_x, 5 * jx, 0, uwx, uxx);                                          \
      const unsigned hb_n = jx + 1 < ngx ? headw_x[(jx + 1) * NT] : 0u;                     \
      const unsigned nbw = hb_c | (hb_n << 16);                                             \
      res_d16_t eo;                                                                         \
      _Pragma("unroll") for (int i = 0; i < 16; i++) eo[i] = eog[(16 * jx + i) * NT];       \
      _Pragma("unroll 1") for (int bp = 0; bp < 2; bp++) {                                  \
        STEP(RES_OV, 2 * bp, itA, itB, gA, gB);                                             \
        STEP(RES_OV, 2 * bp + 1, itB, itA, gB, gA);                                         \
      }                                                                                     \
      _Pragma("unroll") for (int i = 0; i < 16; i++) eog[(16 * jx + i) * NT] = eo[i];       \
      hb_c = hb_n;                                                                          \
    }                                                                                       \
  }
#define RES_PRIME(T, OFF, gA)                                                                                         \
  {                                                                                                                   \
    int it0[B];                                                                                                       \
    const unsigned n0 = RES_NIB(0, 0), n1 = RES_NIB(0, 1);                                                            \
    _Pragma("unroll") for (int k = 0; k < B; k++) {                                                                   \
      rcb += ((n0 >> k) & 1u) << 2;                                                                                   \
      it0[k] = *(const int *)(run_item_b + ((n0 >> k) & 1u ? rcb : rb0b));                                            \
    }                                                                                                                 \
    _Pragma("unroll") for (int k = 0; k < B; k++) {                                                                   \
      rcb += ((n1 >> k) & 1u) << 2;                                                                                   \
      itA[k] = *(const int *)(run_item_b + ((n1 >> k) & 1u ? rcb : rb0b));                                            \
    }                                                                                                                 \
    _Pragma("unroll") for (int k = 0; k < B; k++)                                                                     \
      gA[k] = *(const T *)(dv_b + (OFF) + ((n0 >> k) & 1u ? (unsigned)it0[k] << DSH : padb));                         \
  }

#define RES_OPAQUE()                                                                            \
  _Pragma("unroll") for (int j_ = 0; j_ < NG; j_++) {                                           \
    asm volatile("" : "+v"(uw[j_]), "+v"(ux[j_]), "+v"(hbv[j_]), "+v"(nbv[j_]));                \
  }
  res_d16_t ev[NGV > 0 ? NGV : 1];
#pragma unroll
  for (int j = 0; j < NG; j++) {
#pragma unroll 1
    for (int bb = 0; bb < 4; bb++) {
      int row[B];
#pragma unroll
      for (int k = 0; k < B; k++) row[k] = a.e_in ? 0 : perm_g[(16 * j + 4 * bb + k) * NT + tid];
#pragma unroll
      for (int k = 0; k < B; k++) {
        const double x = (a.e_in ? a.e_in[((int64_t)g * Rt + 16 * j + 4 * bb + k) * NT + tid] : a.eq[row[k] < 0 ? 0 : row[k]].x) + e_shift_k;
        RES_ON_ST(bb, k, x);
      }
    }
  }
  if (OVF) {
    for (int jx = 0; jx < ngx; jx++) {
#pragma unroll 4
      for (int i = 0; i < 16; i++) {
        const int64_t sl = 16 * (NG + jx) + i;
        const int row = a.e_in ? 0 : perm_g[sl * NT + tid];
        const double x = (a.e_in ? a.e_in[((int64_t)g * Rt + sl) * NT + tid] : a.eq[row < 0 ? 0 : row].x) + e_shift_k;
        eog[(16 * jx + i) * NT] = x;
      }
    }
  }
  __syncthreads();
  if (S2B && !s2_tab) {
    const uint32_t *uidw_p = a.uidw + (int64_t)g * (5 * NGt) * NT + tid;
    const uint32_t *headw_p = a.headw + (int64_t)g * NGt * NT + tid;
    int run = run0 - 1;
    double c = 0.0;
#pragma unroll 1
    for (int jp = 0; jp < NGt; jp++) {
      const unsigned nb = headw_p[jp * NT] | (jp == 0 ? 1u : 0u);
      const unsigned uxp = uidw_p[(5 * jp + 4) * NT];
#pragma unroll 1
      for (int bb = 0; bb < 4; bb++) {
        const unsigned lo_ = uidw_p[(5 * jp + bb) * NT];
#pragma unroll 1
        for (int k = 0; k < B; k++) {
          if ((nb >> (4 * bb + k)) & 1u) {
            run++;
            c = a.dv[((int64_t)a.run_item[run] << (DSH - 3)) + 1];
          }
          const int uid = RES_UID(lo_, uxp, bb, k);
          __hip_atomic_fetch_add(&acc3w[uid], c * c, __ATOMIC_RELAXED, __HIP_MEMORY_SCOPE_WORKGROUP);
        }
      }
    }
    __syncthreads();
  }

  RES_STAMP0(2);
  const int f_first = a.f_begin - a.linear;
  for (int f = f_first; f < a.f_end; f++) {
    const bool lin = f < a.f_begin;
    double *Vf = lin ? a.w : a.V + (int64_t)f * a.D;
    const double *zf = lin ? a.zw : a.z + (int64_t)(f - a.f_begin) * a.D;
    const double *lamf = lin ? a.lam_w : a.lam + (int64_t)f * a.n_groups;
    const double *muf = lin ? a.mu_w : a.mu + (int64_t)f * a.n_groups;
    int uj = 0;
    double uold = 0.0, uz = 0.0, ulam = 0.0, umu = 0.0;
    if (tid < nu) {
      const int2 d = a.user_desc[u0 + tid];
      uj = d.x;
      uold = Vf[uj];
      uz = zf[uj];
      ulam = lamf[d.y];
      umu = muf[d.y];
    }
    RES_STAMP(0);
    {
      RES_OPAQUE();
      asm volatile(";; res sweep A");
      unsigned rcb = 4u * (unsigned)(run0 - 1);
      int itA[B];
      d2_t ddA[B];
      RES_PRIME(d2_t, 0, ddA);
      d2_t ddc = d2_t{0.0, 0.0};
      int itB[B];
      d2_t ddB[B];
#define RES_STEP_A(F, bb, iti, ito, ddi, ddo)                                                                              \
  {                                                                                                                        \
    const unsigned n4 = F##_NIB(bb), n4a = F##_NIB((bb) + 1), n4b = F##_NIB((bb) + 2);                                     \
    _Pragma("unroll") for (int k = 0; k < B; k++) {                                                                        \
      rcb += ((n4b >> k) & 1u) << 2;                                                                                       \
      ito[k] = *(const int *)(run_item_b + ((n4b >> k) & 1u ? rcb : rb0b));                                                \
    }                                                                                                                      \
    _Pragma("unroll") for (int k = 0; k < B; k++)                                                                          \
      ddo[k] = *(const d2_t *)(dv_b + ((n4a >> k) & 1u ? (unsigned)iti[k] << DSH : padb));                                 \
    int uid[B];                                                                                                            \
    F##_UIDS(bb, uid);                                                                                                     \
    double up[B], ex[B];                                                                                                   \
    _Pragma("unroll") for (int k = 0; k < B; k++) {                                                                        \
      up[k] = utab[uid[k]][0];                                                                                             \
      ex[k] = F##_LD(bb, k);                                                                                               \
    }                                                                                                                      \
    _Pragma("unroll") for (int k = 0; k < B; k++) {                                                                        \
      const bool need = ((n4 >> k) & 1u) != 0u;                                                                            \
      ddc[0] = need ? ddi[k][0] : ddc[0];                                                                                  \
      ddc[1] = need ? ddi[k][1] : ddc[1];                                                                                  \
      const double er = ex[k] + up[k] * ddc[0];                                                                            \
      F##_ST(bb, k, er);                                                                                                   \
      const double c = ddc[1];                                                                                             \
      __hip_atomic_fetch_add(&acc1w[uid[k]], (-er) * c, __ATOMIC_RELAXED, __HIP_MEMORY_SCOPE_WORKGROUP);                   \
      if (!S2B) __hip_atomic_fetch_add(&acc2w[uid[k]], c * c, __ATOMIC_RELAXED, __HIP_MEMORY_SCOPE_WORKGROUP);             \
    }                                                                                                                      \
  }
#pragma unroll
      for (int j = 0; j < NG; j++) {
        RES_PRIO(j);
#pragma unroll
        for (int bp = 0; bp < 2; bp++) {
          RES_STEP_A(RES_ON, 2 * bp, itA, itB, ddA, ddB);
          RES_STEP_A(RES_ON, 2 * bp + 1, itB, itA, ddB, ddA);
        }
      }
      asm volatile(";; res sweep end");
      RES_OVERFLOW_GROUPS(RES_STEP_A, ddA, ddB);
#undef RES_STEP_A
    }
    __syncthreads();
    RES_STAMP(1);
    if (tid < nu) {
      double S1 = 0.0, S2 = 0.0;
#pragma unroll
      for (int w = 0; w < NW; w++) {
        double *accS = S2B ? acc3 : acc2;
        S1 += acc1[w * U + tid];
        S2 += accS[w * U + tid];
        acc1[w * U + tid] = 0.0;
        accS[w * U + tid] = 0.0;
      }
      const double fresh = PMainV::draw(S1, S2, uold, alpha_k, ulam, umu, uz);
      Vf[uj] = fresh;
      if (XCH && a.xmodel) {
        for (int r = 0; r < a.xworld; r++)
          if (r != a.xrank)
            __hip_atomic_store((lin ? a.xw[r] : a.xV[r] + (int64_t)f * a.D) + uj, fresh, __ATOMIC_RELAXED, __HIP_MEMORY_SCOPE_SYSTEM);
      }
      utab[tid] = d2_t{lin ? 1.0 : fresh, fresh - uold};
    }
    __syncthreads();
    RES_STAMP(2);
    {
      typedef typename std::conditional<S2B, res_d2u_t, double>::type cc_t;
#define RES_CC0(x) res_cc0(x)
#define RES_CC1(x) res_cc1(x)
      bool have_head = false;
      double f1 = 0.0, f2 = 0.0, s1 = 0.0, s2 = 0.0;
      d2_t *part2 = (d2_t *)a.partials;
      char *part_b = (char *)a.partials - 16;
      const unsigned trashb = 16u * (unsigned)(trash_run + 1);
      {
        RES_OPAQUE();
        asm volatile(";; res sweep B");
        unsigned rcb = 4u * (unsigned)(run0 - 1);
        unsigned rcCb = 16u * (unsigned)(run0 - 1);
        int itA[B];
        cc_t ccA[B];
        RES_PRIME(cc_t, 8, ccA);
        double ccc = 0.0, cqc = 0.0;
        int itB[B];
        cc_t ccB[B];
#define RES_PARTIAL_STORE() *(d2_t *)(part_b + (head && have_head ? rcCb : trashb)) = d2_t{s1, s2}
#define RES_STEP_B(F, bb, iti, ito, cci, cco)                                                                              \
  {                                                                                                                        \
    const unsigned n4 = F##_NIB(bb), n4a = F##_NIB((bb) + 1), n4b = F##_NIB((bb) + 2);                                     \
    const unsigned h4 = (F##_HEADS >> (4 * (bb))) & 15u;                                                                   \
    _Pragma("unroll") for (int k = 0; k < B; k++) {                                                                        \
      rcb += ((n4b >> k) & 1u) << 2;                                                                                       \
      ito[k] = *(const int *)(run_item_b + ((n4b >> k) & 1u ? rcb : rb0b));                                                \
    }                                                                                                                      \
    _Pragma("unroll") for (int k = 0; k < B; k++)                                                                          \
      cco[k] = *(const cc_t *)(dv_b + 8 + ((n4a >> k) & 1u ? (unsigned)iti[k] << DSH : padb));                             \
    int uid[B];                                                                                                            \
    F##_UIDS(bb, uid);                                                                                                     \
    d2_t ut[B];                                                                                                            \
    double ex[B];                                                                                                          \
    _Pragma("unroll") for (int k = 0; k < B; k++) {                                                                        \
      ut[k] = utab[uid[k]];                                                                                                \
      ex[k] = F##_LD(bb, k);                                                                                               \
    }                                                                                                                      \
    _Pragma("unroll") for (int k = 0; k < B; k++) {                                                                        \
      const bool need = ((n4 >> k) & 1u) != 0u;                                                                            \
      const bool head = ((h4 >> k) & 1u) != 0u;                                                                            \
      ccc = need ? RES_CC0(cci[k]) : ccc;                                                                                  \
      if (S2B) {                                                                                                           \
        cqc = need ? RES_CC1(cci[k]) : cqc;                                                                                \
        __hip_atomic_fetch_add(&acc3w[uid[k]], cqc, __ATOMIC_RELAXED, __HIP_MEMORY_SCOPE_WORKGROUP);                       \
      }                                                                                                                    \
      rcCb += need ? 16u : 0u;                                                         \
                        \
      RES_PARTIAL_STORE();                                                                                                 \
      f1 = head && !have_head ? s1 : f1;                                                                                   \
      f2 = head && !have_head ? s2 : f2;                                                                                   \
      have_head = have_head || head;                                                                                       \
      const double er = ex[k] + ccc * ut[k][1];                                                                            \
      F##_ST(bb, k, er);                                                                                                   \
      s1 = (head ? 0.0 : s1) + (-er) * ut[k][0];                                                                           \
      s2 = (head ? 0.0 : s2) + ut[k][0] * ut[k][0];                                                                        \
    }                                                                                                                      \
  }
#pragma unroll
        for (int j = 0; j < NG; j++) {
          RES_PRIO(j);
#pragma unroll 1
          for (int bp = 0; bp < 2; bp++) {
            RES_STEP_B(RES_ON, 2 * bp, itA, itB, ccA, ccB);
            RES_STEP_B(RES_ON, 2 * bp + 1, itB, itA, ccB, ccA);
          }
          if (a.prof && lane == 0 && (wv == 4 || wv == 7))
            a.prof[((int64_t)g * a.n_sw + (f - f_first)) * 64 + 16 + (wv == 4 ? 0 : 20) + j] = __builtin_amdgcn_s_memrealtime();
        }
        asm volatile(";; res sweep end");
        RES_OVERFLOW_GROUPS(RES_STEP_B, ccA, ccB);
#undef RES_STEP_B
#undef RES_CC0
#undef RES_CC1
#undef RES_PARTIAL_STORE
      }
      if (a.prof && lane == 0)
        a.prof[((int64_t)g * a.n_sw + (f - f_first)) * 64 + 8 + wv] = __builtin_amdgcn_s_memrealtime();
      double v1 = s1, v2 = s2;
      int fl = have_head ? 1 : 0;
      wave_segscan2(v1, v2, fl);
      if (lane == 63) {
        wcarry[wv] = d2_t{v1, v2};
        wflag[wv] = fl;
      }
      double x1 = dpp_f64<0x138, 0xf>(v1), x2 = dpp_f64<0x138, 0xf>(v2);
      int xf = dpp_i32<0x138, 0xf>(fl, 0);
      if (lane == 0) {
        x1 = 0.0;
        x2 = 0.0;
        xf = 0;
      }
      lds_barrier();
      if (have_head && tid > 0) {
        if (!xf) {
          double c1 = 0.0, c2 = 0.0;
          for (int w = 0; w < wv; w++) {
            const d2_t cw = wcarry[w];
            const bool fw = wflag[w] != 0;
            c1 = (fw ? 0.0 : c1) + cw[0];
            c2 = (fw ? 0.0 : c2) + cw[1];
          }
          x1 = c1 + x1;
          x2 = c2 + x2;
        }
        const int closing = head0 ? run0 - 1 : run0;
        part2[closing] = d2_t{x1 + f1, x2 + f2};
      }
    }
    RES_STAMP(3);
    constexpr int CH = MFM_RES_CH;
    const int c0 = a.ent_ptr[g] >> 6, c1 = a.ent_ptr[g + 1] >> 6;
    const int per = (c1 - c0 + NW - 1) / NW;
    const int wb = c0 + wv * per, we = wb + per < c1 ? wb + per : c1;
    const int i0 = a.wg_item_ptr[g], ni = a.wg_item_ptr[g + 1] - i0;
    const bool more = f + 1 < a.f_end;
    int ij = 0;
    double iold = 0.0, iz = 0.0, ivn = 0.0, ivq = 0.0, ilam = 0.0, imu = 0.0;
    if (tid < ni) {
      const int2 d = a.item_desc[i0 + tid];
      ij = d.x;
      iold = Vf[ij];
      iz = zf[ij];
      ivn = more ? a.V[(int64_t)(f + 1) * a.D + ij] : 0.0;
      if (S2B) ivq = f + 2 < a.f_end ? a.V[(int64_t)(f + 2) * a.D + ij] : 0.0;
      ilam = lamf[d.y];
      imu = muf[d.y];
    }
    const bool ent4 = a.ent4 != 0;
#define RES_ENTRIES(c_)                                                                                                    \
  if (ent4) {                                                                                                              \
    _Pragma("unroll") for (int k = 0; k < CH; k++)                                                                         \
      en[k] = make_int2((int)a.entries[(int64_t)((c_) + k < we ? (c_) + k : (c_)) * WAVE + lane], 0);                      \
  } else {                                                                                                                 \
    _Pragma("unroll") for (int k = 0; k < CH; k++)                                                                         \
      en[k] = ((const int2 *)a.entries)[(int64_t)((c_) + k < we ? (c_) + k : (c_)) * WAVE + lane];                         \
  }
#define RES_ENT_RUN(e_) (ent4 ? res_entry_run((uint32_t)(e_).x) : (e_).x)
#define RES_ENT_ITEM(e_) (ent4 ? res_entry_item((uint32_t)(e_).x) : (e_).y)
    int2 en[CH];
#pragma unroll
    for (int k = 0; k < CH; k++) en[k] = make_int2(0, 0);
    if (wb < we) {
      RES_ENTRIES(wb);
    }
    res_grid_barrier(a, rbar, ++nbar, tid, dead);
    RES_STAMP(4);
    {
      const d2_t *part2 = (const d2_t *)a.partials;
      for (int cb = wb; cb < we; cb += CH) {
        d2_t sv[CH];
#pragma unroll
        for (int k = 0; k < CH; k++) sv[k] = part2[RES_ENT_RUN(en[k])];
        int il[CH];
#pragma unroll
        for (int k = 0; k < CH; k++) il[k] = RES_ENT_ITEM(en[k]);
        if (cb + CH < we) {
          RES_ENTRIES(cb + CH);
        }
#pragma unroll
        for (int k = 0; k < CH; k++) {
          if (cb + k >= we) break;
          __hip_atomic_fetch_add(&acc1[wv * U + il[k]], sv[k][0], __ATOMIC_RELAXED, __HIP_MEMORY_SCOPE_WORKGROUP);
          __hip_atomic_fetch_add(&acc2[wv * U + il[k]], sv[k][1], __ATOMIC_RELAXED, __HIP_MEMORY_SCOPE_WORKGROUP);
        }
      }
      __syncthreads();
      double S1 = 0.0, S2 = 0.0;
      if (tid < ni) {
#pragma unroll
        for (int w = 0; w < NW; w++) {
          S1 += acc1[w * U + tid];
          S2 += acc2[w * U + tid];
          acc1[w * U + tid] = 0.0;
          acc2[w * U + tid] = 0.0;
        }
      }
      if (XCH) {
        const unsigned long long E = a.xepoch0 + (unsigned long long)(f - f_first) + 1ull;
        const int64_t stride = 2 * ((int64_t)a.n_items + 1), par = (int64_t)(E & 1ull);
        if (tid < ni) {
          const int64_t off = ((int64_t)a.xrank * 2 + par) * stride + 2 * (int64_t)(i0 + tid);
          for (int r = 0; r < a.xworld; r++) {
            __hip_atomic_store(a.xsum[r] + off, S1, __ATOMIC_RELAXED, __HIP_MEMORY_SCOPE_SYSTEM);
            __hip_atomic_store(a.xsum[r] + off + 1, S2, __ATOMIC_RELAXED, __HIP_MEMORY_SCOPE_SYSTEM);
          }
        }
        asm volatile("s_waitcnt vmcnt(0)" ::: "memory");
        __syncthreads();
        if (tid == 0 && !dead) {
          const unsigned long long old = __hip_atomic_fetch_add(a.xarrive, 1ull, __ATOMIC_RELAXED, __HIP_MEMORY_SCOPE_AGENT);
          if (old + 1 == (unsigned long long)a.n_wg * E) {
            for (int r = 0; r < a.xworld && !a.xch_break; r++)
              __hip_atomic_store(a.xflag[r] + 16 * a.xrank, E, __ATOMIC_RELEASE, __HIP_MEMORY_SCOPE_SYSTEM);
          }
          for (int r = 0; r < a.xworld && !dead; r++) res_spin_sys(a, a.xflag[a.xrank] + 16 * r, E, dead);
        }
        __syncthreads();
        if (tid < ni) {
          S1 = S2 = 0.0;
          for (int r = 0; r < a.xworld; r++) {
            const int64_t off = ((int64_t)r * 2 + par) * stride + 2 * (int64_t)(i0 + tid);
            S1 += __hip_atomic_load(a.xsum[a.xrank] + off, __ATOMIC_RELAXED, __HIP_MEMORY_SCOPE_SYSTEM);
            S2 += __hip_atomic_load(a.xsum[a.xrank] + off + 1, __ATOMIC_RELAXED, __HIP_MEMORY_SCOPE_SYSTEM);
          }
        }
      }
      if (tid < ni) {
        const double fresh = PMainV::draw(S1, S2, iold, alpha_k, ilam, imu, iz);
        Vf[ij] = fresh;
        res_store2(a.dv + ((int64_t)(i0 + tid) << (DSH - 3)), fresh - iold, ivn);
        if (S2B) __hip_atomic_store(a.dv + 4 * (int64_t)(i0 + tid) + 2, ivq * ivq, __ATOMIC_RELAXED, __HIP_MEMORY_SCOPE_AGENT);
      }
    }
    RES_STAMP(5);
    res_grid_barrier(a, rbar, ++nbar, tid, dead);
    RES_STAMP(6);
  }
#undef RES_STAMP
#undef RES_ENTRIES
#undef RES_ENT_RUN
#undef RES_ENT_ITEM
  RES_STAMP0(3);
  if (!a.no_store) {
    int run_last = run0;
#pragma unroll
    for (int j = 0; j < NG; j++) {
#pragma unroll 1
      for (int bb = 0; bb < 4; bb++) {
        const unsigned h4 = (hbv[j] >> (4 * bb)) & 15u;
        int row[B], it[B];
#pragma unroll
        for (int k = 0; k < B; k++) {
          if (16 * j + 4 * bb + k > 0) run_last += (int)((h4 >> k) & 1u);
          it[k] = a.run_item[run_last];
          row[k] = perm_g[(16 * j + 4 * bb + k) * NT + tid];
        }
        int uid[B];
        RES_ON_UIDS(bb, uid);
#pragma unroll
        for (int k = 0; k < B; k++) {
          const double dl = a.dv[(int64_t)it[k] << (DSH - 3)];
          const double ex = RES_ON_LD(bb, k);
          const double ef = ex + utab[uid[k]][0] * dl;
          if (a.e_slots)
            a.e_slots[((int64_t)g * Rt + 16 * j + 4 * bb + k) * NT + tid] = ef;
          else if (row[k] >= 0)
            a.eq[row[k]].x = ef;
        }
      }
    }
    if (OVF) {
      for (int jx = 0; jx < ngx; jx++) {
        res_u4_t uwx;
        unsigned uxx;
        RES_USER_WORDS(uidw_x, 5 * jx, 0, uwx, uxx);
        const unsigned hbx = headw_x[jx * NT];
#pragma unroll 1
        for (int bb = 0; bb < 4; bb++) {
          const unsigned h4 = (hbx >> (4 * bb)) & 15u;
          int it[B], uid[B];
#pragma unroll
          for (int k = 0; k < B; k++) {
            run_last += (int)((h4 >> k) & 1u);
            it[k] = a.run_item[run_last];
          }
          RES_OV_UIDS(bb, uid);
#pragma unroll
          for (int k = 0; k < B; k++) {
            const double dl = a.dv[(int64_t)it[k] << (DSH - 3)];
            double *ep = eog + (16 * jx + 4 * bb + k) * NT;
            *ep = *ep + utab[uid[k]][0] * dl;
          }
        }
      }
    }
  }
#undef RES_PRIO
#undef RES_NIB
#undef RES_ON_NIB
#undef RES_ON_HEADS
#undef RES_ON_UIDS
#undef RES_ON_LD
#undef RES_ON_ST
#undef RES_OV_NIB
#undef RES_OV_HEADS
#undef RES_OV_UIDS
#undef RES_OV_LD
#undef RES_OV_ST
#undef RES_OVERFLOW_GROUPS
#undef RES_PRIME
#undef RES_OPAQUE
  asm volatile("s_waitcnt vmcnt(0)" ::: "memory");
  RES_STAMP0(4);
#undef RES_STAMP0
}

__global__ void k_res_init_dv(const double *__restrict__ theta, const int32_t *__restrict__ scols, int n_items,
                              double *__restrict__ dv, unsigned long long *__restrict__ bar, int wd,
                              const double *__restrict__ theta2) {
  const int i = blockIdx.x * blockDim.x + threadIdx.x;
  if (blockIdx.x == 0)
    for (int k = threadIdx.x; k < RES_BAR_WORDS; k += blockDim.x) bar[k] = 0ull;
  if (i > n_items) return;
  const bool pad = i == n_items;
  dv[wd * i] = 0.0;
  dv[wd * i + 1] = pad ? 0.0 : theta ? theta[scols[i]] : 1.0;
  if (wd == 4) {
    const double c2 = !pad && theta2 ? theta2[scols[i]] : 0.0;
    dv[wd * i + 2] = c2 * c2;
    dv[wd * i + 3] = 0.0;
  }
}

__global__ __launch_bounds__(512) void k_res_s2_lin(const uint32_t *__restrict__ uidw, const uint32_t *__restrict__ headw,
                                                    const int32_t *__restrict__ run_item, const int32_t *__restrict__ first_run,
                                                    int NGt, int umax, int n_items, double *__restrict__ s2_lin) {
  extern __shared__ unsigned res_s2_cnt[];
  constexpr int NT = 512, NW = NT / WAVE;
  const int g = (int)blockIdx.x, tid = threadIdx.x, wv = tid >> 6;
  for (int i = tid; i < NW * umax; i += NT) res_s2_cnt[i] = 0u;
  __syncthreads();
  const uint32_t *uidw_p = uidw + (int64_t)g * (5 * NGt) * NT + tid;
  const uint32_t *headw_p = headw + (int64_t)g * NGt * NT + tid;
  int run = first_run[g * NT + tid] - 1;
  bool real = false;
  for (int jp = 0; jp < NGt; jp++) {
    const unsigned nb = headw_p[jp * NT] | (jp == 0 ? 1u : 0u);
    const unsigned uxp = uidw_p[(5 * jp + 4) * NT];
    for (int bb = 0; bb < 4; bb++) {
      const unsigned lo_ = uidw_p[(5 * jp + bb) * NT];
      for (int k = 0; k < 4; k++) {
        if ((nb >> (4 * bb + k)) & 1u) {
          run++;
          real = run_item[run] < n_items;
        }
        if (real) atomicAdd(&res_s2_cnt[wv * umax + RES_UID(lo_, uxp, bb, k)], 1u);
      }
    }
  }
  __syncthreads();
  for (int i = tid; i < NW * umax; i += NT) s2_lin[(int64_t)g * (NW * umax) + i] = (double)res_s2_cnt[i];
}

__global__ void k_res_unpermute(const double *__restrict__ e_slots, const int32_t *__restrict__ perm, int64_t n_slots,
                                double2 *__restrict__ eq) {
  const int64_t i = (int64_t)blockIdx.x * blockDim.x + threadIdx.x;
  if (i >= n_slots) return;
  const int32_t row = perm[i];
  if (row >= 0) eq[row].x = e_slots[i];
}

struct ResScoreArgs {
  const uint32_t *uidw, *headw;
  const int32_t *first_run, *run_feat, *wg_user_ptr, *wg_fill;
  const int2 *user_desc;
  int umax, KS;
  const double *Vt, *w;
  double w0;
  const double *w0p;
  const double *y_slots;
  double *e_slots;
  double2 *sums;
  unsigned long long *prof;
};

template <int NT, int NG, int KPT>
__global__ __launch_bounds__(NT) void k_res_score(ResScoreArgs a) {
  extern __shared__ __attribute__((aligned(16))) char res_smem[];
  constexpr int R = 16 * NG, NW = NT / WAVE;
  constexpr int US = 2 * KPT + 2;
  const int g = blockIdx.x, tid = threadIdx.x, lane = tid & 63, wv = tid >> 6;
  const int KP = a.KS >> 1;
  const double w0_k = a.w0p ? *a.w0p : a.w0;
  double *uV = (double *)res_smem;
  double *uW = uV + (size_t)a.umax * US;
  double2 *wsum = (double2 *)(uW + ((a.umax + 1) & ~1));
  if (a.prof && tid == 0) a.prof[4 * g] = __builtin_amdgcn_s_memrealtime();
  int *ucol = (int *)(wsum + NW);
  const int u0 = a.wg_user_ptr[g], nu = a.wg_user_ptr[g + 1] - u0;
  for (int ul = tid; ul < a.umax; ul += NT) {
    const int ju = ul < nu ? a.user_desc[u0 + ul].x : -1;
    ucol[ul] = ju;
    uW[ul] = ju >= 0 ? a.w[ju] : 0.0;
  }
  __syncthreads();
#pragma unroll 4
  for (int i = tid; i < a.umax * KPT; i += NT) {
    const int ul = i / KPT, pr = i - ul * KPT;
    const int ju = ucol[ul];
    double2 v = make_double2(0.0, 0.0);
    if (ju >= 0 && pr < KP) v = ((const double2 *)(a.Vt + (int64_t)ju * a.KS))[pr];
    ((double2 *)(uV + (size_t)ul * US))[pr] = v;
  }
  res_u4_t uw[NG];
  unsigned ux[NG], hbv[NG];
#pragma unroll
  for (int j = 0; j < NG; j++) {
    RES_GROUP_WORDS(a, NG, j, uw[j], ux[j], hbv[j]);
  }
  int run = a.first_run[g * NT + tid];
  const int64_t fill = a.wg_fill[g];
  __syncthreads();
  if (a.prof && tid == 0) a.prof[4 * g + 1] = __builtin_amdgcn_s_memrealtime();
  double2 vi[KPT];
  double wi = 0.0, s1 = 0.0, s2 = 0.0;
#pragma unroll
  for (int p = 0; p < KPT; p++) vi[p] = make_double2(0.0, 0.0);
  int jc[4], jn[4];
  double yn[4];
#pragma unroll
  for (int k = 0; k < 4; k++) yn[k] = a.y_slots[((int64_t)g * R + k) * NT + tid];
  {
    const unsigned h0 = hbv[0] & 15u;
    int r = run;
#pragma unroll
    for (int k = 0; k < 4; k++) {
      if (k > 0) r += (int)((h0 >> k) & 1u);
      jc[k] = a.run_feat[r];
    }
    run = r;
  }
#pragma unroll
  for (int j = 0; j < NG; j++) {
    const unsigned hb2 = hbv[j] | (j + 1 < NG ? hbv[j + 1 < NG ? j + 1 : j] << 16 : 0u);
#pragma unroll 1
    for (int bb = 0; bb < 4; bb++) {
      {
        const unsigned hn = (hb2 >> (4 * (bb + 1))) & 15u;
        int r = run;
#pragma unroll
        for (int k = 0; k < 4; k++) {
          r += (int)((hn >> k) & 1u);
          jn[k] = a.run_feat[r];
        }
        run = r;
      }
      int uid[4];
      RES_UIDS(uw[j][bb], ux[j], bb, uid);
      const unsigned h4 = (hbv[j] >> (4 * bb)) & 15u;
      double yv[4], eb[4];
#pragma unroll
      for (int k = 0; k < 4; k++) yv[k] = yn[k];
      {
        const int nb = 16 * j + 4 * bb + 4 < R ? 16 * j + 4 * bb + 4 : 0;
#pragma unroll
        for (int k = 0; k < 4; k++) yn[k] = a.y_slots[((int64_t)g * R + nb + k) * NT + tid];
      }
#pragma unroll
      for (int k = 0; k < 4; k++) {
        const int slot = 16 * j + 4 * bb + k;
        const bool head = slot == 0 || ((h4 >> k) & 1u);
        if (head) {
          const int ji = jc[k];
          wi = 0.0;
          if (ji >= 0) {
            const double2 *src = (const double2 *)(a.Vt + (int64_t)ji * a.KS);
#pragma unroll
            for (int p = 0; p < KPT; p++) vi[p] = p < KP ? src[p] : make_double2(0.0, 0.0);
            wi = a.w[ji];
          } else {
#pragma unroll
            for (int p = 0; p < KPT; p++) vi[p] = make_double2(0.0, 0.0);
          }
        }
        const double2 *vu = (const double2 *)(uV + (size_t)uid[k] * US);
        double d0 = 0.0, d1 = 0.0;
#pragma unroll
        for (int p = 0; p < KPT; p += 2) {
          const double2 x0 = vu[p], x1 = vu[p + 1];
          d0 += x0.x * vi[p].x + x0.y * vi[p].y;
          d1 += x1.x * vi[p + 1].x + x1.y * vi[p + 1].y;
        }
        const double pred = w0_k + (uW[uid[k]] + wi) + (d0 + d1);
        const bool real = (int64_t)tid * R + slot < fill;
        const double e = real ? pred - yv[k] : 0.0;
        eb[k] = e;
        s1 += e;
        s2 += e * e;
      }
#pragma unroll
      for (int k = 0; k < 4; k++) a.e_slots[((int64_t)g * R + 16 * j + 4 * bb + k) * NT + tid] = eb[k];
#pragma unroll
      for (int k = 0; k < 4; k++) jc[k] = jn[k];
    }
  }
  if (a.prof && lane == 0) a.prof[4 * g + 2] = __builtin_amdgcn_s_memrealtime();
  wave_allreduce_sum2(s1, s2);
  if (lane == 0) wsum[wv] = make_double2(s1, s2);
  __syncthreads();
  if (a.prof && tid == 0) a.prof[4 * g + 3] = __builtin_amdgcn_s_memrealtime();
  if (tid == 0) {
    double t1 = 0.0, t2 = 0.0;
    for (int w = 0; w < NW; w++) {
      t1 += wsum[w].x;
      t2 += wsum[w].y;
    }
    a.sums[g] = make_double2(t1, t2);
  }
}

#undef RES_UID
#undef RES_UIDS
#undef RES_USER_WORDS
#undef RES_GROUP_WORDS

__global__ void k_res_permute_y(const double *__restrict__ y, const int32_t *__restrict__ perm, int64_t n_slots,
                                double *__restrict__ y_slots) {
  const int64_t i = (int64_t)blockIdx.x * blockDim.x + threadIdx.x;
  if (i >= n_slots) return;
  const int32_t row = perm[i];
  y_slots[i] = row >= 0 ? y[row] : 0.0;
}

template <class F>
static inline void res_parallel_for(int n, F f) {
  const int hw = (int)std::thread::hardware_concurrency();
  const int T = std::max(1, std::min({n, 16, hw > 0 ? hw : 1}));
  if (T == 1) {
    for (int i = 0; i < n; i++) f(i);
    return;
  }
  std::atomic<int> next(0);
  auto work = [&]() {
    for (;;) {
      const int i = next.fetch_add(1);
      if (i >= n) return;
      f(i);
    }
  };
  std::vector<std::thread> pool;
  for (int t = 1; t < T; t++) pool.emplace_back(work);
  work();
  for (auto &t : pool) t.join();
}

struct ResForm {
  int rv, rl;
  bool xch, ovf, s2b;
  const void *fn;
  DeviceOnce raised;
};
static inline auto &res_forms() {
#define MFM_RES_FORM(NGV, NGL, ...) {16 * NGV, 16 * NGL, __VA_ARGS__, (const void *)k_mf_resident<512, NGV, NGL, __VA_ARGS__>, {}}
  static ResForm forms[] = {
      MFM_RES_FORM(1, 0, false, false, false), MFM_RES_FORM(2, 0, false, false, false), MFM_RES_FORM(4, 1, false, false, false),
      MFM_RES_FORM(1, 0, true, false, false),  MFM_RES_FORM(2, 0, true, false, false),  MFM_RES_FORM(4, 1, true, false, false),
      MFM_RES_FORM(4, 1, false, true, false),  MFM_RES_FORM(4, 1, false, false, true),  MFM_RES_FORM(4, 1, false, true, true)};
#undef MFM_RES_FORM
  return forms;
}
static inline ResForm *res_form(int rv, int rl, bool xch, bool ovf, bool s2b) {
  for (ResForm &f : res_forms())
    if (f.rv == rv && f.rl == rl && f.xch == xch && f.ovf == ovf && f.s2b == s2b) return &f;
  return nullptr;
}
struct ResScoreForm {
  int ng;
  const void *fn;
  DeviceOnce raised;
};
static inline auto &res_score_forms() {
#define MFM_RES_SCORE_FORM(NG) {NG, (const void *)k_res_score<512, NG, 16>, {}}
  static ResScoreForm forms[] = {MFM_RES_SCORE_FORM(1), MFM_RES_SCORE_FORM(2), MFM_RES_SCORE_FORM(5), MFM_RES_SCORE_FORM(6),
                                 MFM_RES_SCORE_FORM(7), MFM_RES_SCORE_FORM(8), MFM_RES_SCORE_FORM(9), MFM_RES_SCORE_FORM(10)};
#undef MFM_RES_SCORE_FORM
  return forms;
}
template <class Form, class Args>
static inline void res_launch(Form &f, int G, size_t lds, hipStream_t s, Args &a) {
  if (f.raised.need()) {
    MFM_HIP_CHECK(hipFuncSetAttribute(f.fn, hipFuncAttributeMaxDynamicSharedMemorySize, 160 * 1024));
    f.raised.mark();
  }
  void *args[] = {&a};
  MFM_HIP_CHECK(hipLaunchKernel(f.fn, dim3(G), dim3(512), args, lds, s));
}

struct ResPlan {
  bool ready = false;
  int G = 0, NT = 512, RV = 0, RL = 0, umax = 0, item_bits = 0, n_items = 0;
  int RX = 0;
  int R() const { return RV + RL + RX; }
  bool allow_overflow = true;
  int64_t n_rows = 0, n_runs = 0;
  size_t lds_bytes = 0;
  int s2b = 0;
  int dv_doubles() const { return 1 << (res_dv_shift(s2b != 0) - 3); }
  bool plan_lds() {
    const size_t nw = (size_t)(NT / WAVE), lim = 160 * 1024 - 512;
    lds_bytes = (size_t)RL * NT * 8 + 2 * nw * umax * 8 + (size_t)umax * 16 + nw * 16 + nw * 4 + 64;
    if (lds_bytes > lim) return false;
    s2b = res_form(RV, RL, !allow_overflow, RX > 0, true) && lds_bytes + nw * umax * 8 <= lim ? 1 : 0;
    if (s2b) lds_bytes += nw * umax * 8;
    return true;
  }
  DevBuf<int32_t> perm, first_run, wg_run_ptr, wg_nruns, wg_user_ptr, wg_item_ptr, ent_ptr, scols;
  DevBuf<uint32_t> entries;
  int ent_bytes = 8;
  void choose_entry_width(int64_t zero_run) { ent_bytes = res_entry_bytes(zero_run, !allow_overflow); }
  DevBuf<double> s2_lin;
  void fill_s2_lin(hipStream_t s) {
    s2_lin = DevBuf<double>();
    if (!s2b) return;
    const size_t nw = (size_t)(NT / WAVE);
    s2_lin.alloc((size_t)G * nw * umax);
    hipLaunchKernelGGL(k_res_s2_lin, dim3(G), dim3(NT), nw * umax * sizeof(unsigned), s, uidw.p, headw.p, run_item.p, first_run.p,
                       R() / 16, umax, n_items, s2_lin.p);
    MFM_HIP_CHECK(hipGetLastError());
    MFM_HIP_CHECK(hipStreamSynchronize(s));
  }
  DevBuf<uint32_t> uidw, headw;
  DevBuf<int32_t> run_item;
  DevBuf<int2> user_desc, item_desc;
  DevBuf<double> partials, dv, e_slots;
  DevBuf<unsigned long long> bar;
  DevBuf<int32_t> run_feat, wg_fill;
  DevBuf<double> y_slots;
  DevBuf<double2> sums;
  int max_wg_users = 0, max_slice_items = 0;
  int xworld = 1, xrank = 0;
  bool peers_set = false;
  DevBuf<double> xsum;
  DevBuf<unsigned long long> xflag, xarrive;
  double *peer_sum[RES_MAX_PEERS] = {nullptr, nullptr, nullptr, nullptr, nullptr, nullptr, nullptr, nullptr};
  unsigned long long *peer_flag[RES_MAX_PEERS] = {nullptr, nullptr, nullptr, nullptr, nullptr, nullptr, nullptr, nullptr};
  unsigned long long xepoch = 0;
  bool peers_model = false;
  double *peer_w[RES_MAX_PEERS] = {nullptr, nullptr, nullptr, nullptr, nullptr, nullptr, nullptr, nullptr};
  double *peer_V[RES_MAX_PEERS] = {nullptr, nullptr, nullptr, nullptr, nullptr, nullptr, nullptr, nullptr};
  std::vector<void *> peer_mapped;
  size_t xsum_bytes(int world) const { return (size_t)world * 2 * 2 * ((size_t)n_items + 1) * sizeof(double); }
  void alloc_exchange(int world, int rank, hipStream_t s) {
    xworld = world;
    xrank = rank;
    peers_set = false;
    peers_model = false;
    xepoch = 0;
    auto alloc_shared = [&](auto &buf, size_t count) {
      buf.release();
      void *p = nullptr;
      const size_t bytes = count * sizeof(*buf.p);
      if (hipExtMallocWithFlags(&p, bytes, hipDeviceMallocUncached) != hipSuccess) {
        (void)hipGetLastError();
        throw Error(MFM_ERR_DEVICE, "no uncached device memory for the ranks' exchange buffers (hipExtMallocWithFlags(hipDeviceMallocUncached))");
      }
      buf.p = (decltype(buf.p))p;
      buf.n = count;
      buf.owned = true;
      MFM_HIP_CHECK(hipMemsetAsync(p, 0, bytes, s));
    };
    alloc_shared(xsum, xsum_bytes(world) / sizeof(double));
    alloc_shared(xflag, (size_t)16 * RES_MAX_PEERS);
    xarrive.alloc_zero(16, s);
  }
  std::string why;
  std::vector<int32_t> h_nruns;
  std::vector<std::string> h_diag;

  static int bits_for(int64_t n) {
    int b = 1;
    while (((int64_t)1 << b) < n) b++;
    return b;
  }
  struct Variant {
    int rv, rl;
  };
  static std::vector<Variant> variants() {
    std::vector<Variant> v;
    for (const ResForm &f : res_forms())
      if (!f.xch && !f.ovf && !f.s2b) v.push_back({f.rv, f.rl});
    return v;
  }

  bool choose_layout(int64_t N, const std::vector<int64_t> &ustart, int64_t max_user, int n_cu, std::vector<int64_t> &ucut) {
    const int64_t n_users = (int64_t)ustart.size() - 1;
    const std::vector<Variant> vs = variants();
    const int nv = (int)vs.size();
    bool found = false;
    for (int vi = 0; vi < nv && !found; vi++) {
      const int64_t cap = (int64_t)NT * (vs[vi].rv + vs[vi].rl) - 1;
      if (max_user > cap) continue;
      const int64_t slack = std::min<int64_t>(cap / 8, max_user);
      int64_t Gw = (N + (cap - slack) - 1) / (cap - slack);
      if (Gw > n_cu && N <= (int64_t)n_cu * cap) Gw = n_cu;
      if (Gw > n_cu) continue;
      if (env_flag("MFM_RES_WGS")) Gw = std::min<int64_t>(n_cu, std::max<int64_t>(Gw, env_i64("MFM_RES_WGS", 0)));
      Gw = std::min<int64_t>(Gw, n_users);
      ucut.assign(1, 0);
      bool ok = true;
      for (int64_t g = 1; g <= Gw && ok; g++) {
        const int64_t lo_u = ucut.back();
        int64_t hi_u;
        if (g == Gw) {
          hi_u = n_users;
        } else {
          const int64_t want = (N * g) / Gw;
          hi_u = std::upper_bound(ustart.begin(), ustart.end(), want) - ustart.begin() - 1;
          if (hi_u + 1 <= n_users && ustart[hi_u + 1] - want < want - ustart[hi_u]) hi_u++;
          hi_u = std::max(hi_u, lo_u + 1);
          hi_u = std::min<int64_t>(hi_u, n_users - (Gw - g));
          hi_u = std::max<int64_t>(hi_u, n_users - (Gw - g) * NT);
          while (hi_u > lo_u + 1 && ustart[hi_u] - ustart[lo_u] > cap) hi_u--;
        }
        if (hi_u <= lo_u || ustart[hi_u] - ustart[lo_u] > cap) ok = false;
        ucut.push_back(hi_u);
      }
      if (!ok) continue;
      G = (int)Gw;
      RV = vs[vi].rv;
      RL = vs[vi].rl;
      found = true;
    }
    RX = 0;
    if (!found && allow_overflow) {
      const Variant big = vs[nv - 1];
      for (int rx = 16; rx <= 80 && !found; rx += 16) {
        const int64_t cap = (int64_t)NT * (big.rv + big.rl + rx) - 1;
        if (max_user > cap || N > (int64_t)n_cu * cap) continue;
        int64_t Gw = std::min<int64_t>(n_cu, n_users);
        ucut.assign(1, 0);
        bool ok = true;
        for (int64_t g = 1; g <= Gw && ok; g++) {
          const int64_t lo_u = ucut.back();
          int64_t hi_u;
          if (g == Gw) {
            hi_u = n_users;
          } else {
            const int64_t want = (N * g) / Gw;
            hi_u = std::upper_bound(ustart.begin(), ustart.end(), want) - ustart.begin() - 1;
            if (hi_u + 1 <= n_users && ustart[hi_u + 1] - want < want - ustart[hi_u]) hi_u++;
            hi_u = std::max(hi_u, lo_u + 1);
            hi_u = std::min<int64_t>(hi_u, n_users - (Gw - g));
            hi_u = std::max<int64_t>(hi_u, n_users - (Gw - g) * NT);
            while (hi_u > lo_u + 1 && ustart[hi_u] - ustart[lo_u] > cap) hi_u--;
          }
          if (hi_u <= lo_u || ustart[hi_u] - ustart[lo_u] > cap) ok = false;
          ucut.push_back(hi_u);
        }
        if (!ok) continue;
        G = (int)Gw;
        RV = big.rv;
        RL = big.rl;
        RX = rx;
        found = true;
      }
    }
    if (!found) return fail("no variant fits (rows per CU, or a first-level column longer than a workgroup's capacity)");
    return true;
  }
  bool choose_item_slices(const std::vector<int32_t> &slot_ptr, int64_t counter, std::vector<int32_t> &iptr) {
    iptr.assign((size_t)G + 1, 0);
    bool ok = false;
    for (double scale = 1.0; scale < 3.0 && !ok; scale *= 1.1) {
      const double target = scale * ((double)counter + 16.0 * n_items) / G;
      double acc = 0.0;
      int gq = 0, cnt = 0;
      for (int c = 0; c < n_items; c++) {
        acc += (double)(slot_ptr[c + 1] - slot_ptr[c]) + 16.0;
        cnt++;
        if ((acc >= target || cnt == NT) && gq + 1 < G) {
          iptr[++gq] = c + 1;
          acc = 0.0;
          cnt = 0;
        }
// ... 75 lines not shown
    max_wg_users = maxu;
    if (maxu > NT) return fail("more first-level columns in a workgroup than threads");
    item_bits = bits_for((int64_t)n_items + 1);
    const int UW = 5 * (R / 16), HW = R / 16;
    std::vector<uint16_t> h_uid((size_t)G * cap_slots, 0xffffu);
    std::vector<uint32_t> h_headw((size_t)G * HW * NT, 0);
    std::vector<int32_t> h_perm((size_t)G * cap_slots, -1), h_first((size_t)G * NT, 0);
    std::vector<std::vector<int32_t>> wg_run_item((size_t)G);
    std::vector<int64_t> fill((size_t)G, 0);
    std::vector<int32_t> nruns((size_t)G, 0);
    res_parallel_for(G, [&](int g) {
      const int64_t row0 = ustart[ucut[g]], row1 = ustart[ucut[g + 1]];
      const int64_t n = row1 - row0;
      std::vector<int32_t> cnt((size_t)n_items + 1, 0), uloc((size_t)n);
      for (int64_t u = ucut[g]; u < ucut[g + 1]; u++)
        for (int64_t r = ustart[u]; r < ustart[u + 1]; r++) uloc[(size_t)(r - row0)] = (int32_t)(u - ucut[g]);
      for (int64_t r = row0; r < row1; r++) cnt[(size_t)item_of_row[r] + 1]++;
      std::vector<int32_t> &runs = wg_run_item[g];
      for (int c = 0; c < n_items; c++) {
        if (cnt[c + 1]) {
          const int64_t sidx = cnt[c];
          const int th = (int)(sidx / R), rh = (int)(sidx % R);
          h_headw[((size_t)g * HW + rh / 16) * NT + th] |= 1u << (rh % 16);
          runs.push_back(c);
        }
        cnt[c + 1] += cnt[c];
      }
      {
        size_t ri = 0;
        std::vector<int32_t> run_start(runs.size());
        for (size_t k = 0; k < runs.size(); k++) run_start[k] = cnt[runs[k]];
        for (int t = 0; t < NT; t++) {
          const int64_t s0 = (int64_t)t * R;
          if (s0 >= n) break;
          while (ri + 1 < runs.size() && run_start[ri + 1] <= s0) ri++;
          h_first[(size_t)g * NT + t] = (int32_t)ri;
        }
      }
      for (int64_t r = row0; r < row1; r++) {
        const int64_t sidx = cnt[(size_t)item_of_row[r]]++;
        const int t = (int)(sidx / R), rr = (int)(sidx % R);
        h_perm[(size_t)g * cap_slots + (size_t)rr * NT + t] = (int32_t)r;
        h_uid[(size_t)g * cap_slots + (size_t)sidx] = (uint16_t)uloc[(size_t)(r - row0)];
      }
      fill[g] = n;
      nruns[g] = (int32_t)runs.size();
    });
    std::vector<int32_t> h_slot_ptr((size_t)n_items + 1, 0);
    int64_t counter = 0;
    for (int g = 0; g < G; g++) {
      counter += nruns[g];
      for (int32_t c : wg_run_item[g]) h_slot_ptr[(size_t)c + 1]++;
    }
    for (int c = 0; c < n_items; c++) h_slot_ptr[(size_t)c + 1] += h_slot_ptr[c];
    h_slot_ptr[n_items] = (int32_t)counter;
    n_runs = counter;
    if (counter >= ((int64_t)1 << 31) - 2) return fail("too many runs");
    std::vector<int32_t> run_base = run_bases(nruns);
    const int32_t zero_run = run_base[G];
    std::vector<int32_t> h_run_item((size_t)zero_run + 1, n_items);
    for (int g = 0; g < G; g++) {
      std::copy(wg_run_item[g].begin(), wg_run_item[g].end(), h_run_item.begin() + run_base[g]);
      if (fill[g] < cap_slots) {
        const int th = (int)(fill[g] / R), rh = (int)(fill[g] % R);
        h_headw[((size_t)g * HW + rh / 16) * NT + th] |= 1u << (rh % 16);
      }
      h_headw[((size_t)g * HW) * NT] |= 1u;
      for (int t = 0; t < NT; t++) {
        const int64_t s0 = (int64_t)t * R;
        int32_t &fr = h_first[(size_t)g * NT + t];
        fr = (s0 >= fill[g] ? nruns[g] : fr) + run_base[g];
      }
    }
    std::vector<int32_t> h_uptr((size_t)G + 1, 0);
    std::vector<int2> h_udesc;
    for (int g = 0; g < G; g++) {
      for (int32_t j : wg_users[g]) h_udesc.push_back(make_int2(j, group_of && (size_t)j < group_of->size() ? (*group_of)[j] : 0));
      h_uptr[g + 1] = (int32_t)h_udesc.size();
    }
    std::vector<int32_t> h_iptr;
    if (!choose_item_slices(h_slot_ptr, counter, h_iptr)) return false;
    int imax = 0;
    for (int g = 0; g < G; g++) imax = std::max(imax, h_iptr[g + 1] - h_iptr[g]);
    max_slice_items = imax;
    umax = std::max(maxu, imax) + 1;
    if (umax > 1024) return fail("internal: user field");
    std::vector<uint32_t> h_uidw((size_t)G * UW * NT, 0);
    res_parallel_for(G, [&](int g) {
      for (int64_t sl = 0; sl < cap_slots; sl++) {
        const uint16_t u16 = h_uid[(size_t)g * cap_slots + (size_t)sl];
        const uint32_t u = u16 == 0xffffu ? (uint32_t)(umax - 1) : u16;
        const int t = (int)(sl / R), r = (int)(sl % R);
        const int w0 = 5 * (r / 16), bb = (r % 16) / 4, k = r % 4;
        if (k < 3) {
          h_uidw[((size_t)g * UW + w0 + bb) * NT + t] |= u << (10 * k);
        } else {
          h_uidw[((size_t)g * UW + w0 + bb) * NT + t] |= (u & 3u) << 30;
          h_uidw[((size_t)g * UW + w0 + 4) * NT + t] |= (u >> 2) << (8 * bb);
        }
      }
    });
    h_uid = std::vector<uint16_t>();
    std::vector<int32_t> slice_of((size_t)n_items);
    for (int g = 0; g < G; g++)
      for (int c = h_iptr[g]; c < h_iptr[g + 1]; c++) slice_of[c] = g;
    std::vector<int32_t> h_eptr((size_t)G + 1, 0);
    {
      std::vector<int64_t> cnt((size_t)G, 0);
      for (int g = 0; g < G; g++)
        for (int32_t c : wg_run_item[g]) cnt[slice_of[c]]++;
      for (int g = 0; g < G; g++) {
        const int64_t e = h_eptr[g] + ((cnt[g] + WAVE - 1) / WAVE) * WAVE;
        if (e >= ((int64_t)1 << 31)) return fail("too many entries");
        h_eptr[g + 1] = (int32_t)e;
      }
    }
    choose_entry_width(zero_run);
    const size_t ew = (size_t)ent_bytes / 4;
    std::vector<uint32_t> h_entries(ew * (size_t)h_eptr[G]);
    auto put_entry = [&](size_t i, int32_t run, int32_t item) {
      if (ew == 1) {
        h_entries[i] = res_entry_pack(run, item);
      } else {
        h_entries[2 * i] = (uint32_t)run;
        h_entries[2 * i + 1] = (uint32_t)item;
      }
    };
    for (size_t i = 0; i < (size_t)h_eptr[G]; i++) put_entry(i, zero_run, 0);
    {
      std::vector<int64_t> pos((size_t)G);
      for (int g = 0; g < G; g++) pos[g] = h_eptr[g];
      for (int g = 0; g < G; g++)
        for (size_t l = 0; l < wg_run_item[g].size(); l++) {
          const int32_t c = wg_run_item[g][l];
          const int sgl = slice_of[c];
          put_entry((size_t)pos[sgl]++, run_base[g] + (int32_t)l, c - h_iptr[sgl]);
        }
    }
    if ((size_t)h_eptr[G] >= ((size_t)1 << 31)) return fail("too many entries");
    if (!plan_lds()) return fail("LDS");
    uidw.upload(h_uidw);
    headw.upload(h_headw);
    run_item.upload(h_run_item);
    perm.upload(h_perm);
    first_run.upload(h_first);
    wg_user_ptr.upload(h_uptr);
    user_desc.upload(h_udesc.data(), h_udesc.size());
    wg_item_ptr.upload(h_iptr);
    ent_ptr.upload(h_eptr);
    entries.upload(h_entries);
    wg_run_ptr.upload(run_base);
    wg_nruns.upload(nruns);
    fill_s2_lin(nullptr);
    e_slots.alloc((size_t)G * cap_slots);
    {
      std::vector<int32_t> h_run_feat(h_run_item.size() + 8, -1);
      for (size_t r = 0; r < h_run_item.size(); r++) h_run_feat[r] = h_run_item[r] < n_items ? items[(size_t)h_run_item[r]] : -1;
      run_feat.upload(h_run_feat);
      std::vector<int32_t> h_fill((size_t)G);
      for (int g = 0; g < G; g++) h_fill[g] = (int32_t)fill[g];
      wg_fill.upload(h_fill);
      sums.alloc((size_t)G);
      y_slots = DevBuf<double>();
    }
    h_nruns = nruns;
    if (env_flag("MFM_RES_PROF")) {
      h_diag.assign((size_t)G, "");
      for (int g = 0; g < G; g++) {
        int64_t maxlen = 0;
        for (int64_t u = ucut[g]; u < ucut[g + 1]; u++) maxlen = std::max(maxlen, ustart[u + 1] - ustart[u]);
        int64_t sinstr = 0, maxst = 0, nthr_head = 0;
        for (int w = 0; w < NT / WAVE; w++) {
          std::vector<char> hh(WAVE, 0);
          std::vector<int> st(WAVE, 0);
          for (int r = 0; r < R; r++) {
            bool any = false;
            for (int l = 0; l < WAVE; l++) {
              const int t = w * WAVE + l;
              const bool head = (h_headw[((size_t)g * HW + r / 16) * NT + t] >> (r % 16)) & 1u;
              if (head && hh[l]) {
                any = true;
                st[l]++;
              }
              hh[l] = hh[l] || head;
            }
            sinstr += any;
          }
          for (int l = 0; l < WAVE; l++) {
            maxst = std::max<int64_t>(maxst, st[l]);
            nthr_head += hh[l];
          }
        }
        char buf[160];
        std::snprintf(buf, sizeof buf, "users %d maxlen %lld rows %lld store-instr %lld max-stores/thread %lld threads-with-head %lld",
                      (int)(ucut[g + 1] - ucut[g]), (long long)maxlen, (long long)fill[g], (long long)sinstr, (long long)maxst,
                      (long long)nthr_head);
        h_diag[g] = buf;
      }
    }
    scols.upload(items);
    {
      std::vector<int2> h_idesc(items.size());
      for (size_t i = 0; i < items.size(); i++) {
        const int32_t j = items[i];
        h_idesc[i] = make_int2(j, group_of && (size_t)j < group_of->size() ? (*group_of)[j] : 0);
      }
      item_desc.upload(h_idesc.data(), h_idesc.size());
    }
    partials.alloc((size_t)2 * ((size_t)zero_run + 1));
    MFM_HIP_CHECK(hipMemset(partials.p, 0, (size_t)16 * ((size_t)zero_run + 1)));
    dv.alloc((size_t)dv_doubles() * (n_items + 1));
    bar.alloc(RES_BAR_WORDS);
    ready = true;
    why.clear();
    return true;
  }
  bool fail(const char *w) {
    why = w;
    ready = false;
    return false;
  }
};

static inline ResForm &res_kernel(const ResPlan &rp, bool xch) {
  const bool ovf = rp.RX > 0 && res_form(rp.RV, rp.RL, false, true, false);
  ResForm *f = res_form(rp.RV, rp.RL, xch, ovf, rp.s2b != 0);
  if (!f) throw Error(MFM_ERR_RUNTIME, "internal: no resident kernel variant for this plan");
  return *f;
}

static inline hipError_t res_occupancy(const ResPlan &rp, int *per_cu) {
  *per_cu = 0;
  const void *fn = res_kernel(rp, false).fn;
  hipError_t e = hipFuncSetAttribute(fn, hipFuncAttributeMaxDynamicSharedMemorySize, 160 * 1024);
  if (e != hipSuccess) return e;
  return hipOccupancyMaxActiveBlocksPerMultiprocessor(per_cu, fn, 512, rp.lds_bytes);
}

static inline void run_sweep_resident(hipStream_t s, Timing &tm, ResPlan &rp, int kernel_class, double2 *eq, double *V, int64_t D,
                                      int f_begin, int f_end, const double *zbase, const double *lam, const double *mu,
                                      const int32_t *group, int n_groups, double alpha, int *error,
                                      double *w = nullptr, const double *zw = nullptr, const double *lam_w = nullptr,
                                      const double *mu_w = nullptr, double e_shift = 0.0, bool load_slots = false,
                                      bool no_store = false, const double *scal = nullptr) {
  ResArgs a;
  std::memset(&a, 0, sizeof(a));
  a.scal = scal;
  a.eq = eq;
  a.e_slots = rp.e_slots.p;
  a.ngx = rp.RX / 16;
  a.no_store = no_store ? 1 : 0;
  a.e_in = load_slots ? rp.e_slots.p : nullptr;
  a.linear = w ? 1 : 0;
  a.n_sw = f_end - f_begin + a.linear;
  a.w = w;
  a.zw = zw;
  a.lam_w = lam_w;
  a.mu_w = mu_w;
  a.e_shift = e_shift;
  a.perm = rp.perm.p;
  a.uidw = rp.uidw.p;
  a.headw = rp.headw.p;
  a.run_item = rp.run_item.p;
  a.first_run = rp.first_run.p;
  a.wg_user_ptr = rp.wg_user_ptr.p;
  a.user_desc = rp.user_desc.p;
  a.wg_item_ptr = rp.wg_item_ptr.p;
  a.ent_ptr = rp.ent_ptr.p;
  a.entries = rp.entries.p;
  a.ent4 = rp.ent_bytes == 4 ? 1 : 0;
  a.s2_lin = rp.s2b && w ? rp.s2_lin.p : nullptr;
  a.wg_run_ptr = rp.wg_run_ptr.p;
  a.wg_nruns = rp.wg_nruns.p;
  a.scols = rp.scols.p;
  a.item_desc = rp.item_desc.p;
  a.partials = rp.partials.p;
  a.dv = rp.dv.p;
  a.V = V;
  a.D = D;
  a.f_begin = f_begin;
  a.f_end = f_end;
  a.z = zbase;
  a.lam = lam;
  a.mu = mu;
  a.group = group;
  a.n_groups = n_groups;
  a.alpha = alpha;
  a.n_items = rp.n_items;
  a.umax = rp.umax;
  a.bar = rp.bar.p;
  a.n_wg = rp.G;
  a.error = error;
  const bool xch = rp.xworld > 1;
  a.xch_break = xch && rp.xrank == 1 && env_flag("MFM_RES_XCH_BREAK");
  a.xworld = rp.xworld;
  a.xrank = rp.xrank;
  a.xepoch0 = rp.xepoch;
  a.xarrive = rp.xarrive.p;
  a.xmodel = xch && rp.peers_model ? 1 : 0;
  for (int r = 0; r < RES_MAX_PEERS; r++) {
    a.xsum[r] = rp.peer_sum[r];
    a.xflag[r] = rp.peer_flag[r];
    a.xw[r] = rp.peer_w[r];
    a.xV[r] = rp.peer_V[r];
  }
  if (xch && !rp.peers_set) throw Error(MFM_ERR_RUNTIME, "row-sharded persistent sweep: the peers' exchange buffers are not set (mfm_peer_set)");
  static int prof_launch = 0;
  const bool prof = env_flag("MFM_RES_PROF") && ++prof_launch == env_int("MFM_RES_PROF", 0);
  DevBuf<unsigned long long> prof_buf;
  if (prof) {
    prof_buf.alloc((size_t)rp.G * a.n_sw * 64);
    MFM_HIP_CHECK(hipMemsetAsync(prof_buf.p, 0, (size_t)rp.G * a.n_sw * 512, s));
    a.prof = prof_buf.p;
  }
  const int K = a.n_sw;
  double bytes = (8.0 + (load_slots ? 0.0 : 4.0) + 1.4 + (no_store ? 0.0 : 8.0)) * rp.n_rows + K * (40.0 + rp.ent_bytes) * rp.n_runs;
  if (rp.RX) bytes += (double)K * (16.0 + 1.75) * (double)rp.G * rp.NT * rp.RX;
  {
    const int f_second = f_begin + (w ? 0 : 1);
    hipLaunchKernelGGL(k_res_init_dv, dim3((rp.n_items + 256) / 256), dim3(256), 0, s,
                       w ? (const double *)nullptr : V + (int64_t)f_begin * D, rp.scols.p, rp.n_items,
                       rp.dv.p, rp.bar.p, rp.dv_doubles(), rp.s2b && f_second < f_end ? V + (int64_t)f_second * D : (const double *)nullptr);
  }
  TimedLaunch t(tm, s, kernel_class, bytes);
  res_launch(res_kernel(rp, xch), rp.G, rp.lds_bytes, s, a);
  MFM_HIP_CHECK(hipGetLastError());
  if (xch) rp.xepoch += (unsigned long long)a.n_sw;
  if (prof) {
    MFM_HIP_CHECK(hipStreamSynchronize(s));
    const int K2 = a.n_sw;
    std::vector<unsigned long long> h((size_t)rp.G * K2 * 64);
    MFM_HIP_CHECK(hipMemcpy(h.data(), prof_buf.p, h.size() * 8, hipMemcpyDeviceToHost));
    const char *names[6] = {"sweep A", "user draw", "sweep B", "barrier 1 (wait)", "item draw", "barrier 2 (wait)"};
    std::fprintf(stderr, "[resident profile] G=%d factors=%d; us per factor: mean | mean of max over workgroups | mean of min\n", rp.G, K2);
    for (int ph = 0; ph < 6; ph++) {
      double sm = 0, smax = 0, smin = 0;
      for (int f = 0; f < K2; f++) {
        double mx = 0, mn = 1e30;
        for (int g = 0; g < rp.G; g++) {
          const unsigned long long *t = &h[((size_t)g * K2 + f) * 64];
          const double d = (double)(t[ph + 1] - t[ph]) * 0.01;
          sm += d;
          mx = std::max(mx, d);
          mn = std::min(mn, d);
        }
        smax += mx;
        smin += mn;
      }
      std::fprintf(stderr, "  %-18s %8.2f | %8.2f | %8.2f\n", names[ph], sm / ((double)rp.G * K2), smax / K2, smin / K2);
    }
    {
      std::vector<std::pair<double, int>> tb;
      for (int g = 0; g < rp.G; g++) {
        double d = 0;
        for (int f = 0; f < K2; f++) d += (double)(h[((size_t)g * K2 + f) * 64 + 3] - h[((size_t)g * K2 + f) * 64 + 2]) * 0.01;
        tb.push_back({d / K2, g});
      }
      std::sort(tb.begin(), tb.end());
      std::fprintf(stderr, "  sweep B by workgroup: fastest");
      for (int k = 0; k < 4; k++) std::fprintf(stderr, " wg %d %.1f (%d runs)", tb[k].second, tb[k].first, rp.h_nruns[tb[k].second]);
      std::fprintf(stderr, "; median wg %d %.1f (%d runs); slowest", tb[rp.G / 2].second, tb[rp.G / 2].first, rp.h_nruns[tb[rp.G / 2].second]);
      for (int k = rp.G - 4; k < rp.G; k++) std::fprintf(stderr, " wg %d %.1f (%d runs)", tb[k].second, tb[k].first, rp.h_nruns[tb[k].second]);
      std::fprintf(stderr, "\n");
      if (!rp.h_diag.empty())
        for (int k : {0, 1, rp.G / 2, rp.G - 3, rp.G - 2, rp.G - 1})
        {
          const int g = tb[k].second;
          std::fprintf(stderr, "    wg %d %.1f us: %s; waves:", g, tb[k].first, rp.h_diag[g].c_str());
          for (int w = 0; w < 8; w++) {
            double d = 0;
            for (int f = 0; f < K2; f++) d += (double)(h[((size_t)g * K2 + f) * 64 + 8 + w] - h[((size_t)g * K2 + f) * 64 + 2]) * 0.01;
            std::fprintf(stderr, " %.1f", d / K2);
          }
          std::fprintf(stderr, "\n      groups of 16 slots of waves 4 and 7 (factor 3 alone):");
          for (int w : {0, 20}) {
            std::fprintf(stderr, " |");
            for (int b = 0; b < (rp.RV + rp.RL) / 16; b++)
              std::fprintf(stderr, " %.1f", (double)(h[((size_t)g * K2 + 3) * 64 + 16 + w + b] - h[((size_t)g * K2 + 3) * 64 + 2]) * 0.01);
          }
          std::fprintf(stderr, "\n");
        }
    }
    if (const char *dump = env_str("MFM_RES_PROF_DUMP")) {
      if (FILE *fp = std::fopen(dump, "w")) {
        for (int g = 0; g < rp.G; g++) {
          std::fprintf(fp, "%d", g);
          for (int ph = 0; ph < 6; ph++) {
            double d = 0;
            for (int f = 0; f < K2; f++) d += (double)(h[((size_t)g * K2 + f) * 64 + ph + 1] - h[((size_t)g * K2 + f) * 64 + ph]) * 0.01;
            std::fprintf(fp, " %.2f", d / K2);
          }
          std::fprintf(fp, " | %s\n", rp.h_diag.empty() ? "" : rp.h_diag[g].c_str());
        }
        std::fclose(fp);
      }
    }
    {
      const char *nm[4] = {"census barrier", "residual load", "factor loop", "residual store"};
      for (int ph = 0; ph < 4; ph++) {
        double sm = 0, mx = 0;
        for (int g = 0; g < rp.G; g++) {
          const double d = (double)(h[(size_t)g * K2 * 64 + 56 + ph + 1] - h[(size_t)g * K2 * 64 + 56 + ph]) * 0.01;
          sm += d;
          mx = std::max(mx, d);
        }
        std::fprintf(stderr, "  %-18s %8.2f mean | %8.2f max (us, whole launch)\n", nm[ph], sm / rp.G, mx);
      }
      unsigned long long t0 = ~0ull, t1 = 0;
      for (int g = 0; g < rp.G; g++) {
        t0 = std::min(t0, h[(size_t)g * K2 * 64 + 56]);
        t1 = std::max(t1, h[(size_t)g * K2 * 64 + 60]);
      }
      std::fprintf(stderr, "  first workgroup in to last workgroup out: %.1f us\n", (double)(t1 - t0) * 0.01);
    }
    double tot = 0;
// ... 75 lines not shown
```

### myfm_amd/csrc/mfm_res_plan.hpp

```cpp
#pragma once
#include <chrono>

#include <hipcub/hipcub.hpp>

#include "mfm_res.hpp"

namespace mfm {

namespace rp {

constexpr int TB = 256;

__global__ void k_rows(const int32_t *__restrict__ colidx, int64_t N, int32_t *__restrict__ bflag, int32_t *__restrict__ ucnt,
                       int32_t *__restrict__ icnt, int32_t *__restrict__ red) {
  const int64_t r = (int64_t)blockIdx.x * blockDim.x + threadIdx.x;
  int32_t mu = -1, mi = 0x7fffffff;
  if (r < N) {
    const int2 c = ((const int2 *)colidx)[r];
    const bool b = r == 0 || c.x != colidx[2 * (r - 1)];
    bflag[r] = b ? 1 : 0;
    if (b) atomicAdd(&ucnt[c.x], 1);
    atomicAdd(&icnt[c.y], 1);
    mu = c.x;
    mi = c.y;
// ... 314 lines not shown
  inclusive_sum(bflag.p, uord1.p, N, tmp, s);
  lap("rows, columns, scans (enqueued + run)");
  int32_t h_red[4], n_items = 0, n_emp = 0, n_users = 0;
  MFM_HIP_CHECK(hipMemcpyAsync(h_red, red.p, sizeof h_red, hipMemcpyDeviceToHost, s));
  MFM_HIP_CHECK(hipMemcpyAsync(&n_items, iord.p + D0, sizeof(int32_t), hipMemcpyDeviceToHost, s));
  MFM_HIP_CHECK(hipMemcpyAsync(&n_emp, eord.p + D0, sizeof(int32_t), hipMemcpyDeviceToHost, s));
  MFM_HIP_CHECK(hipMemcpyAsync(&n_users, uord1.p + (N - 1), sizeof(int32_t), hipMemcpyDeviceToHost, s));
  MFM_HIP_CHECK(hipStreamSynchronize(s));
  if (!given && h_red[0] >= h_red[1]) return rpn.fail("the two fields' column ranges overlap");
  if (h_red[2] != 0) return rpn.fail("first level not contiguous");
  if (n_users < 1 || n_items < 1) return rpn.fail("empty level");
  rpn.n_items = n_items;
  DevBuf<int32_t> empties, d_ustart, d_users;
  rpn.scols.alloc((size_t)n_items);
  empties.alloc((size_t)std::max(n_emp, 1));
  d_ustart.alloc((size_t)n_users + 1);
  d_users.alloc((size_t)n_users);
  hipLaunchKernelGGL(k_col_lists, grid(D0), dim3(TB), 0, s, iflag.p, eflag.p, iord.p, eord.p, D0, rpn.scols.p, empties.p);
  hipLaunchKernelGGL(k_users, grid(N), dim3(TB), 0, s, X.colidx.p, bflag.p, uord1.p, N, d_ustart.p, d_users.p);
  std::vector<int64_t> ustart((size_t)n_users + 1), ucut;
  int64_t max_user = 0;
  {
    const std::vector<int32_t> u32 = download(d_ustart.p, (size_t)n_users + 1, s);
    for (size_t u = 0; u < u32.size(); u++) ustart[u] = u32[u];
    for (int32_t u = 0; u < n_users; u++) max_user = std::max(max_user, ustart[u + 1] - ustart[u]);
  }
  if (!rpn.choose_layout(N, ustart, max_user, n_cu, ucut)) return false;
  const int G = rpn.G, R = rpn.R();
  const int64_t cap_slots = (int64_t)NT * R;
  if (G > 1024) return rpn.fail("more than 1024 workgroups");
  std::vector<int32_t> h_rowcut((size_t)G + 1), h_ucut((size_t)G + 1), h_uptr((size_t)G + 1, 0);
  int maxu = 0;
  for (int g = 0; g <= G; g++) {
    h_rowcut[g] = (int32_t)ustart[ucut[g]];
    h_ucut[g] = (int32_t)ucut[g];
  }
  for (int g = 0; g < G; g++) {
    const int nu = (int)(ucut[g + 1] - ucut[g]) + n_emp / G + (g < n_emp % G ? 1 : 0);
    maxu = std::max(maxu, nu);
    h_uptr[g + 1] = h_uptr[g] + nu;
  }
  rpn.max_wg_users = maxu;
  if (maxu > NT) return rpn.fail("more first-level columns in a workgroup than threads");
  rpn.item_bits = ResPlan::bits_for((int64_t)n_items + 1);
  const int gbits = ResPlan::bits_for(G);
  if (rpn.item_bits + gbits > 32) return rpn.fail("sort key width");
  DevBuf<int32_t> rowcut, d_ucut, hrun0, hs, headf;
  rowcut.upload(h_rowcut);
  d_ucut.upload(h_ucut);
  rpn.wg_user_ptr.upload(h_uptr);
  DevBuf<uint32_t> key, key2;
  DevBuf<int32_t> val, val2;
  key.alloc((size_t)N);
  key2.alloc((size_t)N);
  val.alloc((size_t)N);
  val2.alloc((size_t)N);
  hipLaunchKernelGGL(k_keys, grid(N), dim3(TB), 0, s, X.colidx.p, iord.p, rowcut.p, G, rpn.item_bits, N, key.p, val.p);
  sort_pairs(key, key2, val, val2, N, rpn.item_bits + gbits, tmp, s);
  lap("users, cuts, keys, sort");
  DevBuf<uint16_t> uid;
  uid.alloc((size_t)G * cap_slots);
  MFM_HIP_CHECK(hipMemsetAsync(uid.p, 0xff, (size_t)G * cap_slots * sizeof(uint16_t), s));
  rpn.perm.alloc((size_t)G * cap_slots);
  MFM_HIP_CHECK(hipMemsetAsync(rpn.perm.p, 0xff, (size_t)G * cap_slots * sizeof(int32_t), s));
  headf.alloc((size_t)N);
  hs.alloc((size_t)N);
  hipLaunchKernelGGL(k_slots, grid(N), dim3(TB), 0, s, key2.p, val2.p, uord1.p, rowcut.p, d_ucut.p, rpn.item_bits, R, NT, N, rpn.perm.p, uid.p,
                     headf.p);
  inclusive_sum(headf.p, hs.p, N, tmp, s);
  hrun0.alloc((size_t)G + 1);
  hipLaunchKernelGGL(k_wg_runs, dim3((G + 1 + TB - 1) / TB), dim3(TB), 0, s, hs.p, rowcut.p, G, hrun0.p);
  const std::vector<int32_t> h_hrun0 = download(hrun0.p, (size_t)G + 1, s);
  std::vector<int32_t> nruns((size_t)G);
  for (int g = 0; g < G; g++) nruns[g] = h_hrun0[g + 1] - h_hrun0[g];
  const int64_t counter = h_hrun0[G];
  rpn.n_runs = counter;
  if (counter >= ((int64_t)1 << 31) - 2) return rpn.fail("too many runs");
  const std::vector<int32_t> run_base = ResPlan::run_bases(nruns);
  const int32_t zero_run = run_base[G];
  rpn.wg_run_ptr.upload(run_base);
  rpn.wg_nruns.upload(nruns);
  rpn.run_item.alloc((size_t)zero_run + 1);
  hipLaunchKernelGGL(k_fill32, grid(zero_run + 1), dim3(TB), 0, s, rpn.run_item.p, (int64_t)zero_run + 1, n_items);
  DevBuf<int32_t> run_item_c, runs_per_item;
  run_item_c.alloc((size_t)std::max<int64_t>(counter, 1));
  runs_per_item.alloc_zero((size_t)n_items, s);
  hipLaunchKernelGGL(k_runs, grid(N), dim3(TB), 0, s, key2.p, headf.p, hs.p, hrun0.p, rpn.wg_run_ptr.p, rpn.item_bits, N, run_item_c.p,
                     rpn.run_item.p, runs_per_item.p);
  rpn.first_run.alloc((size_t)G * NT);
  hipLaunchKernelGGL(k_first, grid((int64_t)G * NT), dim3(TB), 0, s, hs.p, rowcut.p, hrun0.p, rpn.wg_run_ptr.p, G, R, NT, rpn.first_run.p);
  lap("slots, heads, runs, first");
  std::vector<int32_t> h_slot_ptr((size_t)n_items + 1, 0), h_iptr;
  {
    const std::vector<int32_t> rpi = download(runs_per_item.p, (size_t)n_items, s);
    for (int c = 0; c < n_items; c++) h_slot_ptr[(size_t)c + 1] = h_slot_ptr[c] + rpi[c];
  }
  if (!rpn.choose_item_slices(h_slot_ptr, counter, h_iptr)) return false;
  int imax = 0;
  for (int g = 0; g < G; g++) imax = std::max(imax, h_iptr[g + 1] - h_iptr[g]);
  rpn.max_slice_items = imax;
  rpn.umax = std::max(maxu, imax) + 1;
  if (rpn.umax > 1024) return rpn.fail("internal: user field");
  const int UW = 5 * (R / 16), HW = R / 16;
  rpn.uidw.alloc((size_t)G * UW * NT);
  rpn.headw.alloc((size_t)G * HW * NT);
  hipLaunchKernelGGL(k_pack, grid((int64_t)G * HW * NT), dim3(TB), 0, s, uid.p, headf.p, rowcut.p, G, R, NT, rpn.umax, rpn.uidw.p, rpn.headw.p);
  std::vector<int32_t> h_eptr((size_t)G + 1, 0), h_sstart((size_t)G + 1, 0);
  for (int g = 0; g < G; g++) {
    const int64_t cnt = h_slot_ptr[h_iptr[g + 1]] - h_slot_ptr[h_iptr[g]];
    const int64_t e = h_eptr[g] + ((cnt + WAVE - 1) / WAVE) * WAVE;
    if (e >= ((int64_t)1 << 31)) return rpn.fail("too many entries");
    h_eptr[g + 1] = (int32_t)e;
    h_sstart[g + 1] = h_sstart[g] + (int32_t)cnt;
  }
  rpn.wg_item_ptr.upload(h_iptr);
  rpn.ent_ptr.upload(h_eptr);
  rpn.choose_entry_width(zero_run);
  const bool ent4 = rpn.ent_bytes == 4;
  rpn.entries.alloc((size_t)(rpn.ent_bytes / 4) * (size_t)h_eptr[G]);
  if (h_eptr[G]) hipLaunchKernelGGL(k_fill_entries, grid(h_eptr[G]), dim3(TB), 0, s, rpn.entries.p, (int64_t)h_eptr[G], zero_run, 0, ent4);
  if (counter > 0) {
    DevBuf<int32_t> sstart;
    sstart.upload(h_sstart);
    DevBuf<uint32_t> sk, sk2;
    DevBuf<int32_t> sv, sv2;
    sk.alloc((size_t)counter);
    sk2.alloc((size_t)counter);
    sv.alloc((size_t)counter);
    sv2.alloc((size_t)counter);
    hipLaunchKernelGGL(k_slice_keys, grid(counter), dim3(TB), 0, s, run_item_c.p, rpn.wg_item_ptr.p, G, counter, sk.p, sv.p);
    sort_pairs(sk, sk2, sv, sv2, counter, gbits, tmp, s);
    hipLaunchKernelGGL(k_entries, grid(counter), dim3(TB), 0, s, sk2.p, sv2.p, run_item_c.p, hrun0.p, rpn.wg_run_ptr.p, rpn.wg_item_ptr.p,
                       rpn.ent_ptr.p, sstart.p, G, counter, rpn.entries.p, ent4);
    MFM_HIP_CHECK(hipStreamSynchronize(s));
  }
  lap("slices, pack, entries");
  DevBuf<int32_t> d_group;
  if (group_of && (int64_t)group_of->size() >= D0) d_group.upload(group_of->data(), (size_t)D0);
  rpn.user_desc.alloc((size_t)h_uptr[G]);
  hipLaunchKernelGGL(k_user_desc, grid((int64_t)n_users + n_emp), dim3(TB), 0, s, d_users.p, empties.p, d_ucut.p, rpn.wg_user_ptr.p, d_group.p, G,
                     n_users, n_emp, rpn.user_desc.p);
  rpn.item_desc.alloc((size_t)n_items);
  hipLaunchKernelGGL(k_item_desc, grid(n_items), dim3(TB), 0, s, rpn.scols.p, d_group.p, n_items, rpn.item_desc.p);
  rpn.run_feat.alloc((size_t)zero_run + 1 + 8);
  hipLaunchKernelGGL(k_run_feat, grid((int64_t)zero_run + 9), dim3(TB), 0, s, rpn.run_item.p, rpn.scols.p, n_items, (int64_t)zero_run + 1,
                     (int64_t)zero_run + 9, rpn.run_feat.p);
  {
    std::vector<int32_t> h_fill((size_t)G);
    for (int g = 0; g < G; g++) h_fill[g] = h_rowcut[g + 1] - h_rowcut[g];
    rpn.wg_fill.upload(h_fill);
  }
  if (!rpn.plan_lds()) return rpn.fail("LDS");
  rpn.fill_s2_lin(s);
  rpn.e_slots.alloc((size_t)G * cap_slots);
  rpn.sums.alloc((size_t)G);
  rpn.y_slots = DevBuf<double>();
  rpn.h_nruns = nruns;
  rpn.h_diag.clear();
  rpn.partials.alloc((size_t)2 * ((size_t)zero_run + 1));
  MFM_HIP_CHECK(hipMemsetAsync(rpn.partials.p, 0, (size_t)16 * ((size_t)zero_run + 1), s));
  rpn.dv.alloc((size_t)rpn.dv_doubles() * (n_items + 1));
  rpn.bar.alloc(RES_BAR_WORDS);
  MFM_HIP_CHECK(hipStreamSynchronize(s));
  MFM_HIP_CHECK(hipGetLastError());
  lap("descriptors, buffers");
  rpn.ready = true;
  rpn.why.clear();
  return true;
}

static inline std::string res_plan_compare(const ResPlan &a, const ResPlan &b, hipStream_t s) {
  if (a.G != b.G || a.RV != b.RV || a.RL != b.RL || a.RX != b.RX || a.umax != b.umax || a.item_bits != b.item_bits || a.n_items != b.n_items ||
      a.n_rows != b.n_rows || a.n_runs != b.n_runs || a.lds_bytes != b.lds_bytes || a.s2b != b.s2b || a.max_wg_users != b.max_wg_users ||
      a.max_slice_items != b.max_slice_items || a.ent_bytes != b.ent_bytes)
    return "scalars";
  auto same = [&](const void *p, size_t np, const void *q, size_t nq, size_t elem) {
    if (np != nq) return false;
    std::vector<char> x(np * elem), y(nq * elem);
    if (np) {
      MFM_HIP_CHECK(hipMemcpyAsync(x.data(), p, np * elem, hipMemcpyDeviceToHost, s));
      MFM_HIP_CHECK(hipMemcpyAsync(y.data(), q, nq * elem, hipMemcpyDeviceToHost, s));
    }
    MFM_HIP_CHECK(hipStreamSynchronize(s));
    return x == y;
  };
#define MFM_RP_CMP(f) \
  if (!same(a.f.p, a.f.n, b.f.p, b.f.n, sizeof(*a.f.p))) return #f;
  MFM_RP_CMP(perm)
  MFM_RP_CMP(first_run)
  MFM_RP_CMP(wg_run_ptr)
  MFM_RP_CMP(wg_nruns)
  MFM_RP_CMP(wg_user_ptr)
  MFM_RP_CMP(wg_item_ptr)
  MFM_RP_CMP(ent_ptr)
  MFM_RP_CMP(scols)
  MFM_RP_CMP(entries)
  MFM_RP_CMP(uidw)
  MFM_RP_CMP(headw)
  MFM_RP_CMP(run_item)
  MFM_RP_CMP(user_desc)
  MFM_RP_CMP(item_desc)
  MFM_RP_CMP(run_feat)
  MFM_RP_CMP(wg_fill)
  MFM_RP_CMP(s2_lin)
#undef MFM_RP_CMP
  return "";
}

}
```

Baseline: 384.1.

## Precompute per-wave head masks as scalar ballots for the persistent residual sweep

Adds a transposed head-bit layout: a setup kernel ballots each row's per-lane head bit into a 64-bit wave mask. The sweep kernel then reads these masks through a constant-address-space pointer and expands them with inverse_ballot, replacing the per-thread nibble registers (hbv/nbv). This frees VGPRs and removes the padded-item branch on dv loads, since masked-off lanes now point at a trash run. It adds sched barriers between steps. The cost is extra scalar loads per step and a new device buffer built at plan time.

After: 388.4 (median of 5 runs). No clear change (+1.1%).

```diff
diff --git a/include/myfm_hip.h b/include/myfm_hip.h
--- a/include/myfm_hip.h
+++ b/include/myfm_hip.h
@@ -60,6 +60,7 @@
 int mfm_plan_flags(const mfm_ctx *ctx);
 #define MFM_RES_INFO_FIELDS 16
 int mfm_res_info(const mfm_ctx *ctx, int64_t *out, int n_out, char *why, int why_len);
+int mfm_res_masks(mfm_ctx *ctx, int g, uint64_t *out, int64_t n);
 #define MFM_CELL_INFO_FIELDS 74
 int mfm_cell_info(const mfm_ctx *ctx, int64_t *out, int n_out, char *why, int why_len);
 #define MFM_CHAIN_STREAM_INFO_FIELDS 30
diff --git a/myfm_amd/_build.py b/myfm_amd/_build.py
--- a/myfm_amd/_build.py
+++ b/myfm_amd/_build.py
@@ -12,7 +12,7 @@
 PYMOD = os.path.join(HERE, "_myfm" + EXT_SUFFIX)
 
 HIP_UNITS = {
-    "mfm_hip.hip": ["mfm_env.hpp", "mfm_common.hpp", "mfm_wave.hpp", "mfm_policies.hpp", "mfm_kernels.hpp", "mfm_mf_kernels.hpp", "mfm_res.hpp", "mfm_res_entry.hpp", "mfm_res_plan.hpp",
+    "mfm_hip.hip": ["mfm_env.hpp", "mfm_common.hpp", "mfm_wave.hpp", "mfm_policies.hpp", "mfm_kernels.hpp", "mfm_mf_kernels.hpp", "mfm_res.hpp", "mfm_res_entry.hpp", "mfm_res_masks.hpp", "mfm_res_plan.hpp",
                     "mfm_plan.hpp", "mfm_block_kernels.hpp", "mfm_erfcx.hpp", "mfm_tasks.hpp", "mfm_tn.hpp", "mfm_philox.hpp", "mfm_predict.hpp", "mfm_samples.hpp", "mfm_dist.hpp", "mfm_contrib.hpp", "mfm_logdens.hpp", "mfm_psis.hpp", "mfm_ess.hpp", "mfm_crps.hpp", "mfm_loo_pred.hpp", "mfm_normal_quantile.hpp", "mfm_rng.hpp", "mfm_mtjump.hpp", "mfm_cell.hpp",
                     "mfm_chain_api.hpp", "mfm_rng_state.hpp", "mfm_latent_api.hpp", "mfm_latent_host.hpp", "mfm_comm.hpp", "mfm_vbmoments.hpp", "mfm_vb_sums.hpp"],
     "mfm_latent.hip": ["mfm_env.hpp", "mfm_common.hpp", "mfm_rng_state.hpp", "mfm_latent_api.hpp"],
diff --git a/myfm_amd/_capi.py b/myfm_amd/_capi.py
--- a/myfm_amd/_capi.py
+++ b/myfm_amd/_capi.py
@@ -13,7 +13,7 @@
 SYMBOLS = [
     "mfm_version", "mfm_device_count", "mfm_global_error", "mfm_create", "mfm_destroy", "mfm_last_error",
     "mfm_set_stream", "mfm_synchronize", "mfm_set_main", "mfm_add_block", "mfm_set_groups", "mfm_finalize",
-    "mfm_peer_info", "mfm_peer_set", "mfm_peer_model_info", "mfm_peer_set_model", "mfm_peer_export", "mfm_peer_import", "mfm_peer_drop", "mfm_set_residual_policy", "mfm_dim_all", "mfm_plan_info", "mfm_plan_flags", "mfm_res_info", "mfm_cell_info", "mfm_chain_stream_info", "mfm_set_state", "mfm_get_state", "mfm_set_w0", "mfm_zero_w", "mfm_get_e",
+    "mfm_peer_info", "mfm_peer_set", "mfm_peer_model_info", "mfm_peer_set_model", "mfm_peer_export", "mfm_peer_import", "mfm_peer_drop", "mfm_set_residual_policy", "mfm_dim_all", "mfm_plan_info", "mfm_plan_flags", "mfm_res_info", "mfm_res_masks", "mfm_cell_info", "mfm_chain_stream_info", "mfm_set_state", "mfm_get_state", "mfm_set_w0", "mfm_zero_w", "mfm_get_e",
     "mfm_get_q", "mfm_set_e", "mfm_reduce_e", "mfm_shift_e", "mfm_group_stats_w", "mfm_group_stats_V",
     "mfm_sweep_w", "mfm_sweep_V", "mfm_sweep_wV", "mfm_update_e_regression", "mfm_update_e_classification", "mfm_score_train",
     "mfm_oprobit_add_group", "mfm_oprobit_eval", "mfm_oprobit_sample_z", "mfm_hyper_stats", "mfm_timing_enable", "mfm_timing_select", "mfm_timing_reset",
@@ -114,6 +114,7 @@
     L.mfm_plan_info.argtypes = [vp, C.POINTER(i64), C.POINTER(i64)]
     L.mfm_plan_flags.argtypes = [vp]
     L.mfm_res_info.argtypes = [vp, P, C.c_int, C.c_char_p, C.c_int]
+    L.mfm_res_masks.argtypes = [vp, C.c_int, P, i64]
     L.mfm_cell_info.argtypes = [vp, P, C.c_int, C.c_char_p, C.c_int]
     L.mfm_chain_stream_info.argtypes = [vp, P, C.c_int, C.POINTER(C.c_int)]
     L.mfm_cs_plan_probe.argtypes = [i64, i32, P, P, P, i32, i32, i32, i32, P, P, C.POINTER(i32), C.POINTER(dbl)]
@@ -544,6 +545,13 @@
         d["why"] = why.value.decode()
         return d
 
+    def res_masks(self, g):
+        info = self.res_info()
+        per = info["RV"] + info["RL"] + info["RX"] + 8
+        out = np.zeros((8, per), dtype=np.uint64)
+        self._ck(lib().mfm_res_masks(self.h, int(g), _p(out), out.size))
+        return out
+
     CELL_INFO = ("ready", "G", "umax", "item32", "n_streams", "n_fields", "N", "Npad", "max_steps", "chunk_max", "chunk_min",
                  "chunks_empty", "split_mask", "score_fb")
     CELL_STREAM_TYPE = ("U", "I", "C")
diff --git a/myfm_amd/csrc/mfm_hip.hip b/myfm_amd/csrc/mfm_hip.hip
--- a/myfm_amd/csrc/mfm_hip.hip
+++ b/myfm_amd/csrc/mfm_hip.hip
@@ -1586,6 +1586,19 @@
   return MFM_OK;
 }
 
+int mfm_res_masks(mfm_ctx *ctx, int g, uint64_t *out, int64_t n) {
+  if (!ctx || n < 0 || (n > 0 && !out)) return MFM_ERR_INVALID;
+  MFM_TRY(ctx)
+  const ResPlan &rp = ctx->res;
+  if (!ctx->resident_V() || !rp.headm.p) throw Error(MFM_ERR_RUNTIME, "mfm_res_masks: no persistent-sweep layout");
+  const int64_t per = res_masks_per_wg(rp.NT / WAVE, rp.R());
+  if (g < 0 || g >= rp.G) throw Error(MFM_ERR_INVALID, "mfm_res_masks: workgroup out of range");
+  if (n != per) throw Error(MFM_ERR_INVALID, "mfm_res_masks: n must be (NT / 64) * (RV + RL + RX + 8) = " + std::to_string(per));
+  MFM_HIP_CHECK(hipMemcpyAsync(out, rp.headm.p + (int64_t)g * per, (size_t)per * sizeof(uint64_t), hipMemcpyDeviceToHost, ctx->stream));
+  MFM_HIP_CHECK(hipStreamSynchronize(ctx->stream));
+  MFM_CATCH(ctx)
+}
+
 int mfm_cell_info(const mfm_ctx *ctx, int64_t *out, int n_out, char *why, int why_len) {
   if (!ctx || n_out < 0 || (n_out > 0 && !out) || why_len < 0 || (why_len > 0 && !why)) return MFM_ERR_INVALID;
   const CellPlan &cp = ctx->cell;
diff --git a/myfm_amd/csrc/mfm_res.hpp b/myfm_amd/csrc/mfm_res.hpp
--- a/myfm_amd/csrc/mfm_res.hpp
+++ b/myfm_amd/csrc/mfm_res.hpp
@@ -11,6 +11,7 @@
 #include "mfm_common.hpp"
 #include "mfm_mf_kernels.hpp"
 #include "mfm_res_entry.hpp"
+#include "mfm_res_masks.hpp"
 
 namespace mfm {
 
@@ -26,6 +27,7 @@
   const int32_t *perm;
   const uint32_t *uidw;
   const uint32_t *headw;
+  const uint64_t *headm;
   const int32_t *run_item;
   const int32_t *first_run;
   const int32_t *wg_run_ptr;
@@ -158,6 +160,7 @@
 constexpr int res_dv_shift(bool s2b) { return s2b ? 5 : 4; }
 typedef double res_d16_t __attribute__((ext_vector_type(16)));
 typedef unsigned res_u4_t __attribute__((ext_vector_type(4)));
+typedef const uint64_t __attribute__((address_space(4))) *res_masks_p;
 typedef double res_d2u_t __attribute__((ext_vector_type(2), aligned(8)));
 __device__ __forceinline__ double res_cc0(double x) { return x; }
 __device__ __forceinline__ double res_cc1(double) { return 0.0; }
@@ -200,10 +203,7 @@
   int *wflag = (int *)(wcarry + NW);
   const int32_t *perm_g = a.perm + (int64_t)g * Rt * NT;
   const int u0 = a.wg_user_ptr[g], nu = a.wg_user_ptr[g + 1] - u0;
-  const int rb0 = a.wg_run_ptr[g];
-  const int pad_item = a.n_items;
   constexpr int DSH = res_dv_shift(S2B);
-  const unsigned rb0b = 4u * (unsigned)rb0, padb = (unsigned)pad_item << DSH;
   const char *run_item_b = (const char *)a.run_item, *dv_b = (const char *)a.dv;
   double *acc1w = acc1 + wv * U, *acc2w = acc2 + wv * U, *acc3w = acc3 + wv * U;
   bool dead = false;
@@ -223,6 +223,7 @@
   else                               \
     __builtin_amdgcn_s_setprio(0)
   const int trash_run = a.wg_run_ptr[g] + a.wg_nruns[g];
+  const unsigned padrb = 4u * (unsigned)trash_run;
 #define RES_STAMP(k)                                                                                      \
   if (a.prof && tid == 0) a.prof[((int64_t)g * a.n_sw + (f - f_first)) * 64 + (k)] = __builtin_amdgcn_s_memrealtime()
 
@@ -234,21 +235,20 @@
 
   res_u4_t uw[NG];
   unsigned ux[NG];
-  unsigned hbv[NG], nbv[NG];
 #pragma unroll
   for (int j = 0; j < NG; j++) {
-    RES_GROUP_WORDS(a, NGt, j, uw[j], ux[j], hbv[j]);
-    nbv[j] = hbv[j] | (j == 0 ? 1u : 0u);
-  }
-  const unsigned nbx0 = OVF && ngx > 0 ? a.headw[((int64_t)g * NGt + NG) * NT + tid] : 0u;
+    RES_USER_WORDS(a.uidw, (int64_t)g * (5 * NGt) + 5 * j, tid, uw[j], ux[j]);
+  }
+  res_masks_p hm = (res_masks_p)(uintptr_t)(a.headm + res_masks_wave_at(g, NW, wv, Rt));
   double *eog = OVF ? a.e_slots + ((int64_t)g * Rt + 16 * NG) * NT + tid : nullptr;
   const uint32_t *uidw_x = a.uidw + ((int64_t)g * (5 * NGt) + 5 * NG) * NT + tid;
   const uint32_t *headw_x = a.headw + ((int64_t)g * NGt + NG) * NT + tid;
   const int run0 = a.first_run[g * NT + tid];
-  const bool head0 = (hbv[0] & 1u) != 0u;
-#define RES_NIB(j, q) ((((nbv[j]) | ((j) + 1 < NG ? nbv[(j) + 1 < NG ? (j) + 1 : (j)] << 16 : nbx0 << 16)) >> (4 * (q))) & 15u)
-#define RES_ON_NIB(q) RES_NIB(j, q)
-#define RES_ON_HEADS hbv[j]
+  const bool head0 = res_head_bit(a.headw[res_head_word_at(g, NT, Rt, 0, tid)], 0) != 0u;
+#define RES_MASKS4(s_, m_) _Pragma("unroll") for (int k_ = 0; k_ < B; k_++) m_[k_] = hm[(s_) + k_]
+#define RES_LANE(m_) __builtin_amdgcn_inverse_ballot_w64(m_)
+#define RES_STEP_FENCE() __builtin_amdgcn_sched_barrier(0)
+#define RES_ON_SLOT(bb) (16 * j + 4 * (bb))
 #define RES_ON_UIDS(bb, uid) RES_UIDS(uw[j][bb], ux[j], bb, uid)
 #define RES_ON_LD(bb, k) (j < NGV ? ev[j < NGV ? j : 0][4 * (bb) + k] : elds[(16 * (j - NGV) + 4 * (bb) + k) * NT + tid])
 #define RES_ON_ST(bb, k, x)                \
@@ -256,20 +256,16 @@
     ev[j < NGV ? j : 0][4 * (bb) + k] = x; \
   else                                     \
     elds[(16 * (j - NGV) + 4 * (bb) + k) * NT + tid] = x
-#define RES_OV_NIB(q) ((nbw >> (4 * (q))) & 15u)
-#define RES_OV_HEADS hb_c
+#define RES_OV_SLOT(bb) (16 * (NG + jx) + 4 * (bb))
 #define RES_OV_UIDS(bb, uid) RES_UIDS(uwx[bb], uxx, bb, uid)
 #define RES_OV_LD(bb, k) eo[4 * (bb) + k]
 #define RES_OV_ST(bb, k, x) eo[4 * (bb) + k] = x
 #define RES_OVERFLOW_GROUPS(STEP, gA, gB)                                                   \
   if (OVF) {                                                                                \
-    unsigned hb_c = nbx0;                                                                   \
     for (int jx = 0; jx < ngx; jx++) {                                                      \
       res_u4_t uwx;                                                                         \
       unsigned uxx;                                                                         \
       RES_USER_WORDS(uidw_x, 5 * jx, 0, uwx, uxx);                                          \
-      const unsigned hb_n = jx + 1 < ngx ? headw_x[(jx + 1) * NT] : 0u;                     \
-      const unsigned nbw = hb_c | (hb_n << 16);                                             \
       res_d16_t eo;                                                                         \
       _Pragma("unroll") for (int i = 0; i < 16; i++) eo[i] = eog[(16 * jx + i) * NT];       \
       _Pragma("unroll 1") for (int bp = 0; bp < 2; bp++) {                                  \
@@ -277,29 +273,32 @@
         STEP(RES_OV, 2 * bp + 1, itB, itA, gB, gA);                                         \
       }                                                                                     \
       _Pragma("unroll") for (int i = 0; i < 16; i++) eog[(16 * jx + i) * NT] = eo[i];       \
-      hb_c = hb_n;                                                                          \
     }                                                                                       \
   }
 #define RES_PRIME(T, OFF, gA)                                                                                         \
   {                                                                                                                   \
     int it0[B];                                                                                                       \
-    const unsigned n0 = RES_NIB(0, 0), n1 = RES_NIB(0, 1);                                                            \
-    _Pragma("unroll") for (int k = 0; k < B; k++) {                                                                   \
-      rcb += ((n0 >> k) & 1u) << 2;                                                                                   \
-      it0[k] = *(const int *)(run_item_b + ((n0 >> k) & 1u ? rcb : rb0b));                                            \
+    uint64_t n0[B], n1[B];                                                                                            \
+    RES_MASKS4(0, n0);                                                                                                \
+    RES_MASKS4(4, n1);                                                                                                \
+    rcb += 4u;                                        \
+    it0[0] = *(const int *)(run_item_b + rcb);                                                                        \
+    _Pragma("unroll") for (int k = 1; k < B; k++) {                                                                   \
+      rcb += RES_LANE(n0[k]) ? 4u : 0u;                                                                               \
+      it0[k] = *(const int *)(run_item_b + (RES_LANE(n0[k]) ? rcb : padrb));                                          \
     }                                                                                                                 \
     _Pragma("unroll") for (int k = 0; k < B; k++) {                                                                   \
-      rcb += ((n1 >> k) & 1u) << 2;                                                                                   \
-      itA[k] = *(const int *)(run_item_b + ((n1 >> k) & 1u ? rcb : rb0b));                                            \
+      rcb += RES_LANE(n1[k]) ? 4u : 0u;                                                                               \
+      itA[k] = *(const int *)(run_item_b + (RES_LANE(n1[k]) ? rcb : padrb));                                          \
     }                                                                                                                 \
-    _Pragma("unroll") for (int k = 0; k < B; k++)                                                                     \
-      gA[k] = *(const T *)(dv_b + (OFF) + ((n0 >> k) & 1u ? (unsigned)it0[k] << DSH : padb));                         \
+    _Pragma("unroll") for (int k = 0; k < B; k++) gA[k] = *(const T *)(dv_b + (OFF) + ((unsigned)it0[k] << DSH));     \
   }
 
 #define RES_OPAQUE()                                                                            \
   _Pragma("unroll") for (int j_ = 0; j_ < NG; j_++) {                                           \
-    asm volatile("" : "+v"(uw[j_]), "+v"(ux[j_]), "+v"(hbv[j_]), "+v"(nbv[j_]));                \
-  }
+    asm volatile("" : "+v"(uw[j_]), "+v"(ux[j_]));                                              \
+  }                                                                                             \
+  asm volatile("" : "+s"(hm));
   res_d16_t ev[NGV > 0 ? NGV : 1];
 #pragma unroll
   for (int j = 0; j < NG; j++) {
@@ -379,18 +378,20 @@
       int itA[B];
       d2_t ddA[B];
       RES_PRIME(d2_t, 0, ddA);
-      d2_t ddc = d2_t{0.0, 0.0};
+      d2_t ddc = ddA[0];
       int itB[B];
       d2_t ddB[B];
 #define RES_STEP_A(F, bb, iti, ito, ddi, ddo)                                                                              \
   {                                                                                                                        \
-    const unsigned n4 = F##_NIB(bb), n4a = F##_NIB((bb) + 1), n4b = F##_NIB((bb) + 2);                                     \
+    const int s_ = F##_SLOT(bb);                                                                                           \
+    uint64_t n4[B], n4b[B];                                          \
+    RES_MASKS4(s_, n4);                                                                                                    \
+    RES_MASKS4(s_ + 8, n4b);                                                                                               \
     _Pragma("unroll") for (int k = 0; k < B; k++) {                                                                        \
-      rcb += ((n4b >> k) & 1u) << 2;                                                                                       \
-      ito[k] = *(const int *)(run_item_b + ((n4b >> k) & 1u ? rcb : rb0b));                                                \
+      rcb += RES_LANE(n4b[k]) ? 4u : 0u;                                                                                   \
+      ito[k] = *(const int *)(run_item_b + (RES_LANE(n4b[k]) ? rcb : padrb));                                              \
     }                                                                                                                      \
-    _Pragma("unroll") for (int k = 0; k < B; k++)                                                                          \
-      ddo[k] = *(const d2_t *)(dv_b + ((n4a >> k) & 1u ? (unsigned)iti[k] << DSH : padb));                                 \
+    _Pragma("unroll") for (int k = 0; k < B; k++) ddo[k] = *(const d2_t *)(dv_b + ((unsigned)iti[k] << DSH));                                \
     int uid[B];                                                                                                            \
     F##_UIDS(bb, uid);                                                                                                     \
     double up[B], ex[B];                                                                                                   \
@@ -399,7 +400,7 @@
       ex[k] = F##_LD(bb, k);                                                                                               \
     }                                                                                                                      \
     _Pragma("unroll") for (int k = 0; k < B; k++) {                                                                        \
-      const bool need = ((n4 >> k) & 1u) != 0u;                                                                            \
+      const bool need = RES_LANE(n4[k]);                                                                                   \
       ddc[0] = need ? ddi[k][0] : ddc[0];                                                                                  \
       ddc[1] = need ? ddi[k][1] : ddc[1];                                                                                  \
       const double er = ex[k] + up[k] * ddc[0];                                                                            \
@@ -415,7 +416,9 @@
 #pragma unroll
         for (int bp = 0; bp < 2; bp++) {
           RES_STEP_A(RES_ON, 2 * bp, itA, itB, ddA, ddB);
+          RES_STEP_FENCE();
           RES_STEP_A(RES_ON, 2 * bp + 1, itB, itA, ddB, ddA);
+          RES_STEP_FENCE();
         }
       }
       asm volatile(";; res sweep end");
@@ -458,24 +461,25 @@
         RES_OPAQUE();
         asm volatile(";; res sweep B");
         unsigned rcb = 4u * (unsigned)(run0 - 1);
-        unsigned rcCb = 16u * (unsigned)(run0 - 1);
+        unsigned rcCb = 16u * (unsigned)(run0 - (head0 ? 1 : 0));
         int itA[B];
         cc_t ccA[B];
         RES_PRIME(cc_t, 8, ccA);
-        double ccc = 0.0, cqc = 0.0;
+        double ccc = RES_CC0(ccA[0]), cqc = RES_CC1(ccA[0]);
         int itB[B];
         cc_t ccB[B];
 #define RES_PARTIAL_STORE() *(d2_t *)(part_b + (head && have_head ? rcCb : trashb)) = d2_t{s1, s2}
 #define RES_STEP_B(F, bb, iti, ito, cci, cco)                                                                              \
   {                                                                                                                        \
-    const unsigned n4 = F##_NIB(bb), n4a = F##_NIB((bb) + 1), n4b = F##_NIB((bb) + 2);                                     \
-    const unsigned h4 = (F##_HEADS >> (4 * (bb))) & 15u;                                                                   \
+    const int s_ = F##_SLOT(bb);                                                                                           \
+    uint64_t n4[B], n4b[B];                                          \
+    RES_MASKS4(s_, n4);                                                                                                    \
+    RES_MASKS4(s_ + 8, n4b);                                                                                               \
     _Pragma("unroll") for (int k = 0; k < B; k++) {                                                                        \
-      rcb += ((n4b >> k) & 1u) << 2;                                                                                       \
-      ito[k] = *(const int *)(run_item_b + ((n4b >> k) & 1u ? rcb : rb0b));                                                \
+      rcb += RES_LANE(n4b[k]) ? 4u : 0u;                                                                                   \
+      ito[k] = *(const int *)(run_item_b + (RES_LANE(n4b[k]) ? rcb : padrb));                                              \
     }                                                                                                                      \
-    _Pragma("unroll") for (int k = 0; k < B; k++)                                                                          \
-      cco[k] = *(const cc_t *)(dv_b + 8 + ((n4a >> k) & 1u ? (unsigned)iti[k] << DSH : padb));                             \
+    _Pragma("unroll") for (int k = 0; k < B; k++) cco[k] = *(const cc_t *)(dv_b + 8 + ((unsigned)iti[k] << DSH));                            \
     int uid[B];                                                                                                            \
     F##_UIDS(bb, uid);                                                                                                     \
     d2_t ut[B];                                                                                                            \
@@ -485,14 +489,14 @@
       ex[k] = F##_LD(bb, k);                                                                                               \
     }                                                                                                                      \
     _Pragma("unroll") for (int k = 0; k < B; k++) {                                                                        \
-      const bool need = ((n4 >> k) & 1u) != 0u;                                                                            \
-      const bool head = ((h4 >> k) & 1u) != 0u;                                                                            \
-      ccc = need ? RES_CC0(cci[k]) : ccc;                                                                                  \
+      const bool head = RES_LANE(n4[k]);                                                                                   \
+      const double c0_ = RES_CC0(cci[k]), c1_ = RES_CC1(cci[k]);                                                           \
+      ccc = head ? c0_ : ccc;                                                                                              \
       if (S2B) {                                                                                                           \
-        cqc = need ? RES_CC1(cci[k]) : cqc;                                                                                \
+        cqc = head ? c1_ : cqc;                                                                                            \
         __hip_atomic_fetch_add(&acc3w[uid[k]], cqc, __ATOMIC_RELAXED, __HIP_MEMORY_SCOPE_WORKGROUP);                       \
       }                                                                                                                    \
-      rcCb += need ? 16u : 0u;                                                         \
+      rcCb += head ? 16u : 0u;                                                         \
                         \
       RES_PARTIAL_STORE();                                                                                                 \
       f1 = head && !have_head ? s1 : f1;                                                                                   \
@@ -510,7 +514,9 @@
 #pragma unroll 1
           for (int bp = 0; bp < 2; bp++) {
             RES_STEP_B(RES_ON, 2 * bp, itA, itB, ccA, ccB);
+            RES_STEP_FENCE();
             RES_STEP_B(RES_ON, 2 * bp + 1, itB, itA, ccB, ccA);
+            RES_STEP_FENCE();
           }
           if (a.prof && lane == 0 && (wv == 4 || wv == 7))
             a.prof[((int64_t)g * a.n_sw + (f - f_first)) * 64 + 16 + (wv == 4 ? 0 : 20) + j] = __builtin_amdgcn_s_memrealtime();
@@ -675,7 +681,7 @@
     for (int j = 0; j < NG; j++) {
 #pragma unroll 1
       for (int bb = 0; bb < 4; bb++) {
-        const unsigned h4 = (hbv[j] >> (4 * bb)) & 15u;
+        const unsigned h4 = (a.headw[res_head_word_at(g, NT, Rt, 16 * j, tid)] >> (4 * bb)) & 15u;
         int row[B], it[B];
 #pragma unroll
         for (int k = 0; k < B; k++) {
@@ -724,14 +730,14 @@
     }
   }
 #undef RES_PRIO
-#undef RES_NIB
-#undef RES_ON_NIB
-#undef RES_ON_HEADS
+#undef RES_MASKS4
+#undef RES_LANE
+#undef RES_STEP_FENCE
+#undef RES_ON_SLOT
 #undef RES_ON_UIDS
 #undef RES_ON_LD
 #undef RES_ON_ST
-#undef RES_OV_NIB
-#undef RES_OV_HEADS
+#undef RES_OV_SLOT
 #undef RES_OV_UIDS
 #undef RES_OV_LD
 #undef RES_OV_ST
@@ -790,6 +796,17 @@
   for (int i = tid; i < NW * umax; i += NT) s2_lin[(int64_t)g * (NW * umax) + i] = (double)res_s2_cnt[i];
 }
 
+__global__ __launch_bounds__(512) void k_res_headm(const uint32_t *__restrict__ headw, int Rt, uint64_t *__restrict__ headm) {
+  constexpr int NT = 512, NW = NT / WAVE;
+  const int g = (int)blockIdx.x, tid = threadIdx.x, wv = tid >> 6;
+  uint64_t *out = headm + res_masks_wave_at(g, NW, wv, Rt);
+  for (int r = 0; r < Rt + RES_MASK_PAD; r++) {
+    const unsigned bit = r < Rt ? res_head_bit(headw[res_head_word_at(g, NT, Rt, r, tid)], r) : 0u;
+    const uint64_t m = __ballot(bit != 0u);
+    if ((tid & 63) == 0) out[r] = m;
+  }
+}
+
 __global__ void k_res_unpermute(const double *__restrict__ e_slots, const int32_t *__restrict__ perm, int64_t n_slots,
                                 double2 *__restrict__ eq) {
   const int64_t i = (int64_t)blockIdx.x * blockDim.x + threadIdx.x;
@@ -1058,6 +1075,13 @@
     MFM_HIP_CHECK(hipStreamSynchronize(s));
   }
   DevBuf<uint32_t> uidw, headw;
+  DevBuf<uint64_t> headm;
+  void fill_headm(hipStream_t s) {
+    headm.alloc((size_t)res_masks_words(G, NT / WAVE, R()));
+    hipLaunchKernelGGL(k_res_headm, dim3(G), dim3(NT), 0, s, headw.p, R(), headm.p);
+    MFM_HIP_CHECK(hipGetLastError());
+    MFM_HIP_CHECK(hipStreamSynchronize(s));
+  }
   DevBuf<int32_t> run_item;
   DevBuf<int2> user_desc, item_desc;
   DevBuf<double> partials, dv, e_slots;
@@ -1439,6 +1463,7 @@
     wg_run_ptr.upload(run_base);
     wg_nruns.upload(nruns);
     fill_s2_lin(nullptr);
+    fill_headm(nullptr);
     e_slots.alloc((size_t)G * cap_slots);
     {
       std::vector<int32_t> h_run_feat(h_run_item.size() + 8, -1);
@@ -1548,6 +1573,7 @@
   a.perm = rp.perm.p;
   a.uidw = rp.uidw.p;
   a.headw = rp.headw.p;
+  a.headm = rp.headm.p;
   a.run_item = rp.run_item.p;
   a.first_run = rp.first_run.p;
   a.wg_user_ptr = rp.wg_user_ptr.p;
diff --git a/myfm_amd/csrc/mfm_res_masks.hpp b/myfm_amd/csrc/mfm_res_masks.hpp
--- /dev/null
+++ b/myfm_amd/csrc/mfm_res_masks.hpp
@@ -0,0 +1,37 @@
+#pragma once
+#include <cstdint>
+
+#if defined(__HIPCC__)
+#define MFM_RES_MASKS_FN __host__ __device__ inline
+#else
+#define MFM_RES_MASKS_FN inline
+#endif
+
+namespace mfm {
+
+constexpr int RES_MASK_PAD = 8;
+constexpr int RES_MASK_LANES = 64;
+
+MFM_RES_MASKS_FN int64_t res_masks_per_wave(int rt) { return (int64_t)rt + RES_MASK_PAD; }
+MFM_RES_MASKS_FN int64_t res_masks_per_wg(int nw, int rt) { return (int64_t)nw * res_masks_per_wave(rt); }
+MFM_RES_MASKS_FN int64_t res_masks_words(int n_wg, int nw, int rt) { return (int64_t)n_wg * res_masks_per_wg(nw, rt); }
+MFM_RES_MASKS_FN int64_t res_masks_wave_at(int g, int nw, int w, int rt) { return ((int64_t)g * nw + w) * res_masks_per_wave(rt); }
+
+MFM_RES_MASKS_FN int64_t res_head_word_at(int g, int nt, int rt, int r, int t) { return ((int64_t)g * (rt / 16) + r / 16) * nt + t; }
+MFM_RES_MASKS_FN unsigned res_head_bit(uint32_t word, int r) { return (word >> (r & 15)) & 1u; }
+
+MFM_RES_MASKS_FN uint64_t res_mask_of(const uint32_t *headw, int g, int nt, int rt, int w, int r) {
+  if (r >= rt) return 0;
+  uint64_t m = 0;
+  for (int l = 0; l < RES_MASK_LANES; l++)
+    m |= (uint64_t)res_head_bit(headw[res_head_word_at(g, nt, rt, r, w * RES_MASK_LANES + l)], r) << l;
+  return m;
+}
+MFM_RES_MASKS_FN void res_masks_transpose(const uint32_t *headw, int n_wg, int nt, int rt, uint64_t *out) {
+  const int nw = nt / RES_MASK_LANES;
+  for (int g = 0; g < n_wg; g++)
+    for (int w = 0; w < nw; w++)
+      for (int r = 0; r < rt + RES_MASK_PAD; r++) out[res_masks_wave_at(g, nw, w, rt) + r] = res_mask_of(headw, g, nt, rt, w, r);
+}
+
+}
diff --git a/myfm_amd/csrc/mfm_res_plan.hpp b/myfm_amd/csrc/mfm_res_plan.hpp
--- a/myfm_amd/csrc/mfm_res_plan.hpp
+++ b/myfm_amd/csrc/mfm_res_plan.hpp
@@ -490,6 +490,7 @@
   }
   if (!rpn.plan_lds()) return rpn.fail("LDS");
   rpn.fill_s2_lin(s);
+  rpn.fill_headm(s);
   rpn.e_slots.alloc((size_t)G * cap_slots);
   rpn.sums.alloc((size_t)G);
   rpn.y_slots = DevBuf<double>();
@@ -541,7 +542,16 @@
   MFM_RP_CMP(run_feat)
   MFM_RP_CMP(wg_fill)
   MFM_RP_CMP(s2_lin)
+  MFM_RP_CMP(headm)
 #undef MFM_RP_CMP
+  {
+    const std::vector<uint32_t> hw = rp::download(a.headw.p, a.headw.n, s);
+    const std::vector<uint64_t> hm = rp::download(a.headm.p, a.headm.n, s);
+    std::vector<uint64_t> want((size_t)res_masks_words(a.G, a.NT / WAVE, a.R()));
+    if (hw.size() != (size_t)a.G * (a.R() / 16) * a.NT || hm.size() != want.size()) return "headm (size)";
+    res_masks_transpose(hw.data(), a.G, a.NT, a.R(), want.data());
+    if (hm != want) return "headm (transposition)";
+  }
   return "";
 }
 
```
